# mandanasmi/lane-slam

Hardware: AMD Instinct MI355X
Metric: frames/sec (640x480) detect->descript->project->sanity->associate (higher is better)
Workload: dtype u8/f64 (FP4 e2m1 MFMA with exact f32 accumulation for association)

## Files before the change

### include/lanefront.h

```cpp
#ifndef LANEFRONT_H
#define LANEFRONT_H

#include <stddef.h>
#include <stdint.h>

#define LF_API __attribute__((visibility("default")))

#ifdef __cplusplus
extern "C" {
#endif

#define LF_ABI_VERSION 5

typedef enum lf_status {
    LF_OK = 0,
    LF_ERR_BAD_ARG = -1,
    LF_ERR_CAPACITY = -2,
    LF_ERR_HIP = -3,
    LF_ERR_NOT_INITIALISED = -4,
    LF_ERR_UNSUPPORTED = -5,
    LF_ERR_DECODE = -6
} lf_status;

#define LF_WHITE 0
// ... 427 lines not shown
LF_API int lf_deserialize_segments(lf_handle* h, const uint8_t* bodies, int bodies_on_device, const int64_t* frame_byte_offset,
                            int n_frames, lf_segments* out, int out_on_device, int* n_segments);

LF_API int lf_draw_lines(lf_handle* h, int n_frames, const lf_segments* seg, int seg_on_device, uint8_t* out_bgr, int out_on_device);
LF_API int lf_draw_lines_image(lf_handle* h, const uint8_t* bgr, int n_frames, int rows, int cols, const lf_segments* seg, int seg_on_device,
                               uint8_t* out_bgr, int images_on_device);

#define LF_JPEG_ENCODE_STAGES 8
LF_API size_t lf_jpeg_encode_bound(int rows, int cols);
LF_API int lf_jpeg_encode_batch(lf_handle* h, const uint8_t* bgr, int bgr_on_device, int n_frames, int rows, int cols, int quality, uint8_t* out,
                                size_t out_stride, uint32_t* out_size, int out_on_device);
LF_API int lf_jpeg_encode_timing(lf_handle* h, double* ms_per_stage, int n);
LF_API const char* lf_jpeg_encode_stage_name(int stage);

#define LF_RECTIFY_STAGES 1
LF_API int lf_set_camera(lf_handle* h, const double* K, const double* D, const double* R, const double* P, int cam_w, int cam_h);
LF_API int lf_set_rectified_input(lf_handle* h, int flag);
LF_API int lf_get_rectified_input(lf_handle* h, int* flag);
LF_API int lf_rectify_map(lf_handle* h, float* mapx, float* mapy);
LF_API int lf_rectify_batch(lf_handle* h, const uint8_t* src, int src_on_device, int n_frames, int rows, int cols, int channels, uint8_t* dst,
                            int dst_on_device);
LF_API int lf_rectify_timing(lf_handle* h, double* ms_per_stage, int n);
LF_API const char* lf_rectify_stage_name(int stage);

typedef enum lf_buffer_id {
    LF_BUF_BGR = 0,
    LF_BUF_MASKS = 1,
    LF_BUF_EDGES = 2,
    LF_BUF_LSD_ANGLE = 3,
    LF_BUF_LSD_MODGRAD = 4,
    LF_BUF_LSD_ORDER = 5,
    LF_BUF_LSD_NORDER = 6,
    LF_BUF_LBD_DX = 7,
    LF_BUF_LBD_DY = 8,
    LF_BUF_LSD_COUNTS = 9,
    LF_BUF_LSD_SCRATCH = 10,
    LF_BUF_LSD_NLOW = 11
} lf_buffer_id;
LF_API int lf_debug_fetch(lf_handle* h, int buffer_id, void* dst, size_t bytes);
LF_API int lf_debug_detmath(lf_handle* h, int which, const double* a, const double* b_or_null, double* y, int n);
enum { LF_WAVE_INT = 0, LF_WAVE_UINT = 1, LF_WAVE_FLOAT = 2, LF_WAVE_DOUBLE = 3, LF_WAVE_LONG = 4, LF_WAVE_ULONG = 5 };
enum {
    LF_WAVE_READLANE = 0, LF_WAVE_DPP = 1, LF_WAVE_SUM = 2, LF_WAVE_MAX = 3, LF_WAVE_MIN = 4, LF_WAVE_INCL_SCAN_DPP = 5,
    LF_WAVE_INCL_MIN_DPP = 6, LF_WAVE_SUM_BCAST = 7, LF_WAVE_MIN_BCAST = 8, LF_WAVE_INCL_SCAN = 9, LF_WAVE_REDUCE = 10,
    LF_WAVE_BALLOT = 11, LF_WAVE_LANE_MASK_LT = 12, LF_WAVE_LANES_BELOW = 13, LF_WAVE_BALLOT_BRANCH = 14, LF_WAVE_UNI = 15,
    LF_WAVE_WG_EXCL_SCAN = 16, LF_WAVE_WG_SCAN_TURNS = 17
};
LF_API int lf_debug_wave(lf_handle* h, int op, int type, int arg, int diverge, const uint64_t* in, uint64_t* out, int n_threads, int block);
LF_API int lf_debug_probe(lf_handle* h, int width, int write, size_t bytes, int reps);
LF_API int lf_debug_lsd_binary(lf_handle* h, const uint8_t* img, int rows, int cols, float* lines4, int cap, int* n_out);
LF_API int lf_debug_segments(lf_handle* h, int mode, int n_frames, const int32_t* counts, const float* lines4, const uint8_t* masks,
                             lf_segments* out, int* n_segments);
LF_API int lf_debug_std_sort(lf_handle* h, const int32_t* keys, int n, int32_t* order);
LF_API int lf_lsd_size(const lf_handle* h, int* rows, int* cols);
LF_API int lf_suggested_depth(const lf_handle* h);

LF_API int lf_lsd_list_capacity(const lf_handle* h, int* entries, int* grown);
LF_API int lf_lsd_scratch_stride(const lf_handle* h);

#define LF_N_STAGES 16
LF_API int lf_set_profiling(lf_handle* h, int enabled);
LF_API int lf_get_timing(lf_handle* h, double* ms_per_stage, int32_t* launches_per_stage, int n);
LF_API int lf_reset_timing(lf_handle* h);
LF_API const char* lf_stage_name(int stage);

#ifdef __cplusplus
}
#endif
#endif
```

### lane_slam_amd/_lib.py

```python
import ctypes
import os

from .config import LfConfig

_HERE = os.path.dirname(os.path.abspath(__file__))
SO_PATH = os.environ.get("LANEFRONT_LIBRARY") or os.path.join(_HERE, "liblanefront.so")

LF_N_STAGES = 16
LF_MAP_N_STAGES = 4
LF_MSG_DETECTOR, LF_MSG_GROUND, LF_MSG_FILTERED = 0, 1, 2
(LF_BUF_BGR, LF_BUF_MASKS, LF_BUF_EDGES, LF_BUF_LSD_ANGLE, LF_BUF_LSD_MODGRAD, LF_BUF_LSD_ORDER,
 LF_BUF_LSD_NORDER, LF_BUF_LBD_DX, LF_BUF_LBD_DY, LF_BUF_LSD_COUNTS, LF_BUF_LSD_SCRATCH, LF_BUF_LSD_NLOW) = range(12)

EXPORTS = (
    "lf_abi_version", "lf_create", "lf_destroy", "lf_last_error", "lf_synchronize", "lf_get_stream",
    "lf_set_image", "lf_detect_lines", "lf_process_batch", "lf_process_batch_async", "lf_wait", "lf_associate", "lf_associate_float", "lf_kmeans",
    "lf_jpeg_decode_batch", "lf_jpeg_info", "lf_frames_buffer", "lf_serialize_segments", "lf_deserialize_segments",
    "lf_debug_fetch", "lf_debug_detmath", "lf_debug_wave", "lf_debug_probe", "lf_debug_lsd_binary", "lf_debug_segments", "lf_lsd_size", "lf_set_profiling", "lf_get_timing", "lf_reset_timing", "lf_stage_name",
    "lf_map_create", "lf_map_destroy", "lf_map_last_error", "lf_map_get_stream", "lf_map_synchronize", "lf_map_seed", "lf_map_size",
    "lf_map_associate", "lf_map_pack_block", "lf_map_update", "lf_map_step", "lf_map_step_host", "lf_map_fetch",
    "lf_map_set_profiling", "lf_map_get_timing", "lf_map_stage_name",
    "lf_descriptor_default_params", "lf_set_descriptor_params", "lf_get_descriptor_params",
    "lf_edlines_default_params", "lf_keylines_batch", "lf_describe_keylines", "lf_keylines_debug_fetch", "lf_set_image_edlines", "lf_knn_match", "lf_radius_match", "lf_jpeg_decode_batch_gpu", "lf_jpeg_decode_batch_gpu_async", "lf_jpeg_status", "lf_jpeg_decode_for_detect_async",
    "lf_set_tie_rule", "lf_map_set_tie_rule", "lf_debug_std_sort", "lf_suggested_depth", "lf_lsd_list_capacity", "lf_lsd_scratch_stride", "lf_set_detector", "lf_detector_failures", "lf_keylines_batch_async", "lf_keylines_frame_status", "lf_lsd_keylines_batch", "lf_select_queries",
    "lf_lsd_default_options", "lf_lsd_keylines_batch_ex", "lf_keylines_batch_masked",
    "lf_matcher_add", "lf_matcher_clear", "lf_matcher_size", "lf_matcher_match", "lf_matcher_knn_match", "lf_matcher_radius_match",
    "lf_lane_filter_default_config", "lf_lane_filter_create", "lf_lane_filter_destroy", "lf_lane_filter_last_error", "lf_lane_filter_grid",
    "lf_lane_filter_set_tables", "lf_lane_filter_reset", "lf_lane_filter_step", "lf_lane_filter_get_poses", "lf_lane_filter_get_belief",
    "lf_lane_filter_synchronize", "lf_lane_filter_set_profiling", "lf_lane_filter_get_timing", "lf_lane_filter_stage_name",
    "lf_hough_default_params", "lf_set_hough_params", "lf_get_hough_params",
    "lf_dense_default_params", "lf_set_dense_params", "lf_get_dense_params",
    "lf_ai_transform_batch", "lf_set_ai_transform", "lf_get_ai_transform",
    "lf_draw_lines", "lf_draw_lines_image",
    "lf_jpeg_encode_bound", "lf_jpeg_encode_batch", "lf_jpeg_encode_timing", "lf_jpeg_encode_stage_name",
    "lf_set_camera", "lf_set_rectified_input", "lf_get_rectified_input", "lf_rectify_map", "lf_rectify_batch", "lf_rectify_timing",
    "lf_rectify_stage_name",
    "lf_map_default_view", "lf_map_bounds", "lf_map_render", "lf_map_render_counts", "lf_map_render_timing", "lf_map_render_stage_name",
    "lf_sizeof_camera_view", "lf_map_camera_view", "lf_map_render_camera", "lf_map_render_camera_timing",
    "lf_sizeof_align_config", "lf_sizeof_align_result", "lf_map_align_default_config", "lf_map_align", "lf_map_step_aligned",
    "lf_map_step_aligned_host", "lf_map_align_timing",
    "lf_sizeof_smooth_config", "lf_map_smooth_default_config", "lf_map_smooth", "lf_map_step_smoothed", "lf_map_step_smoothed_host",
    "lf_map_smooth_timing",
    "lf_sizeof_localize_config", "lf_sizeof_localize_result", "lf_map_localize_default_config", "lf_map_localize", "lf_map_localize_timing",
    "lf_sizeof_prune_config", "lf_sizeof_prune_result", "lf_map_prune_default_config", "lf_map_prune", "lf_map_prune_timing",
    "lf_sizeof_near_config", "lf_map_near_default_config", "lf_map_associate_near", "lf_map_set_near", "lf_map_get_near", "lf_map_near_timing",
)
LF_ALIGN_OK, LF_ALIGN_FEW, LF_ALIGN_DEGENERATE, LF_ALIGN_REJECTED = 0, 1, 2, 3
ALIGN_STATUS = ("ok", "few", "degenerate", "rejected")
LF_MAP_RENDER_STAGES = 4
LF_JPEG_ENCODE_STAGES = 8
LF_RECTIFY_STAGES = 1
LF_LANE_FILTER_PREDICT, LF_LANE_FILTER_UPDATE = 1, 2
LF_LANE_FILTER_MAX_CELLS = 4096
LF_LANE_FILTER_N_STAGES = 2
LANE_FILTER_PARAMS = ("mean_d_0", "mean_phi_0", "sigma_d_0", "sigma_phi_0", "delta_d", "delta_phi", "d_max", "d_min", "phi_max",
                      "phi_min", "cov_v", "linewidth_white", "linewidth_yellow", "lanewidth", "min_max", "sigma_d_mask", "sigma_phi_mask")
DETECTORS = {"lsd": 0, "edlines": 1, "hough": 2, "dense": 3}
HOUGH_KEYS = ("hough_threshold", "hough_min_line_length", "hough_max_line_gap")
DENSE_KEYS = ("sobel_threshold",)
TIE_RULES = {"lowest": 0, "mihasher": 1}
LF_MAX_OCTAVES = 5


class LfSegments(ctypes.Structure):
    _fields_ = [
        ("capacity", ctypes.c_int32),
        ("frame_offset", ctypes.c_void_p),
        ("lines", ctypes.c_void_p), ("normals", ctypes.c_void_p), ("color", ctypes.c_void_p),
        ("pixels_normalized", ctypes.c_void_p), ("ground", ctypes.c_void_p), ("keep", ctypes.c_void_p),
        ("desc", ctypes.c_void_p), ("code", ctypes.c_void_p),
    ]


class LfEdlinesParams(ctypes.Structure):
    _fields_ = [("gradient_threshold", ctypes.c_int32), ("anchor_threshold", ctypes.c_int32), ("scan_intervals", ctypes.c_int32),
                ("min_line_len", ctypes.c_int32), ("line_fit_err_threshold", ctypes.c_double), ("ksize", ctypes.c_int32)]

# ... 307 lines not shown
    lib.lf_keylines_batch_masked.argtypes = [vp, vp, ci, ci, ci, ci, ctypes.POINTER(LfEdlinesParams), vp, ci, ctypes.POINTER(LfKeylines), ci, ci,
                                             ctypes.POINTER(ci), vp]
    lib.lf_keylines_batch_masked.restype = ci
    lib.lf_describe_keylines.argtypes = [vp, vp, ci, vp, vp, vp, vp, vp, ci, vp, vp, ci]
    lib.lf_describe_keylines.restype = ci
    lib.lf_keylines_debug_fetch.argtypes = [vp, ci, ci, vp, ctypes.c_size_t, vp]
    lib.lf_keylines_debug_fetch.restype = ci
    lib.lf_set_image_edlines.argtypes = [vp, vp, ci, ci, ci, ctypes.POINTER(LfEdlinesParams)]
    lib.lf_set_image_edlines.restype = ci
    lib.lf_keylines_batch_async.argtypes = [vp, vp, ci, ci, ci, ctypes.POINTER(LfEdlinesParams), ctypes.POINTER(LfKeylines), ci]
    lib.lf_keylines_batch_async.restype = ci
    lib.lf_select_queries.argtypes = [vp, vp, ci, vp, vp, vp, ctypes.POINTER(ci), ci]
    lib.lf_select_queries.restype = ci
    lib.lf_matcher_add.argtypes = [vp, vp, ci, ci]
    lib.lf_matcher_clear.argtypes = [vp]
    lib.lf_matcher_size.argtypes = [vp, ctypes.POINTER(ci), ctypes.POINTER(ci)]
    lib.lf_matcher_match.argtypes = [vp, vp, ci, vp, vp, ctypes.POINTER(ci)]
    lib.lf_matcher_knn_match.argtypes = [vp, vp, ci, ci, vp, ci, vp, vp, ctypes.POINTER(ci)]
    lib.lf_matcher_radius_match.argtypes = [vp, vp, ci, ctypes.c_float, vp, ci, vp, vp, ci, ctypes.POINTER(ci), ctypes.POINTER(ci)]
    for fn in (lib.lf_matcher_add, lib.lf_matcher_clear, lib.lf_matcher_size, lib.lf_matcher_match, lib.lf_matcher_knn_match, lib.lf_matcher_radius_match):
        fn.restype = ci
    lib.lf_lsd_keylines_batch.argtypes = [vp, vp, ci, ci, ci, ci, ctypes.POINTER(LfKeylines), ci, ci, ctypes.POINTER(ci)]
    lib.lf_lsd_keylines_batch.restype = ci
    lib.lf_lsd_keylines_batch_ex.argtypes = [vp, vp, ci, ci, ci, ci, ctypes.POINTER(LfLsdOptions), vp, ci, ctypes.POINTER(LfKeylines), ci, ci, ctypes.POINTER(ci)]
    lib.lf_lsd_keylines_batch_ex.restype = ci
    lib.lf_lsd_default_options.argtypes = [ctypes.POINTER(LfLsdOptions)]
    lib.lf_lsd_default_options.restype = None
    lib.lf_keylines_frame_status.argtypes = [vp, vp, ci]
    lib.lf_keylines_frame_status.restype = ci
    lib.lf_set_detector.argtypes = [vp, ci, ctypes.POINTER(LfEdlinesParams)]
    lib.lf_set_detector.restype = ci
    lib.lf_detector_failures.argtypes = [vp]
    lib.lf_detector_failures.restype = ci
    lib.lf_hough_default_params.argtypes = [ctypes.POINTER(LfHoughParams)]
    lib.lf_hough_default_params.restype = None
    lib.lf_set_hough_params.argtypes = [vp, ctypes.POINTER(LfHoughParams)]
    lib.lf_set_hough_params.restype = ci
    lib.lf_get_hough_params.argtypes = [vp, ctypes.POINTER(LfHoughParams)]
    lib.lf_get_hough_params.restype = ci
    lib.lf_dense_default_params.argtypes = [ctypes.POINTER(LfDenseParams)]
    lib.lf_dense_default_params.restype = None
    lib.lf_set_dense_params.argtypes = [vp, ctypes.POINTER(LfDenseParams)]
    lib.lf_set_dense_params.restype = ci
    lib.lf_get_dense_params.argtypes = [vp, ctypes.POINTER(LfDenseParams)]
    lib.lf_get_dense_params.restype = ci
    lib.lf_suggested_depth.argtypes = [vp]
    lib.lf_lsd_list_capacity.argtypes = [vp, ctypes.POINTER(ci), ctypes.POINTER(ci)]
    lib.lf_lsd_list_capacity.restype = ci
    lib.lf_lsd_scratch_stride.argtypes = [vp]
    lib.lf_lsd_scratch_stride.restype = ci
    lib.lf_suggested_depth.restype = ci
    lib.lf_debug_std_sort.argtypes = [vp, vp, ci, vp]
    lib.lf_debug_std_sort.restype = ci
    lib.lf_set_tie_rule.argtypes = [vp, ci]
    lib.lf_set_tie_rule.restype = ci
    lib.lf_map_set_tie_rule.argtypes = [vp, ci]
    lib.lf_map_set_tie_rule.restype = ci
    lib.lf_knn_match.argtypes = [vp, vp, ci, vp, ci, ci, vp, vp, ci]
    lib.lf_knn_match.restype = ci
    lib.lf_radius_match.argtypes = [vp, vp, ci, vp, ci, ctypes.c_float, vp, vp, vp, ci, ctypes.POINTER(ci), ci]
    lib.lf_radius_match.restype = ci
    lib.lf_lane_filter_default_config.argtypes = [ctypes.POINTER(LfLaneFilterConfig)]
    lib.lf_lane_filter_default_config.restype = None
    lib.lf_lane_filter_create.argtypes = [ci, ctypes.POINTER(LfLaneFilterConfig), ci, ci, ctypes.POINTER(vp)]
    lib.lf_lane_filter_destroy.argtypes = [vp]
    lib.lf_lane_filter_destroy.restype = None
    lib.lf_lane_filter_last_error.argtypes = [vp]
    lib.lf_lane_filter_last_error.restype = ctypes.c_char_p
    lib.lf_lane_filter_grid.argtypes = [vp, ctypes.POINTER(ci), ctypes.POINTER(ci)]
    lib.lf_lane_filter_set_tables.argtypes = [vp, vp, vp, vp, vp]
    lib.lf_lane_filter_reset.argtypes = [vp, ci, vp]
    lib.lf_lane_filter_step.argtypes = [vp, vp, ctypes.POINTER(LfSegments), ci, ci, vp, vp, ci, vp, vp, vp]
    lib.lf_lane_filter_get_poses.argtypes = [vp, vp, ci]
    lib.lf_lane_filter_get_belief.argtypes = [vp, ci, vp]
    lib.lf_lane_filter_synchronize.argtypes = [vp]
    lib.lf_lane_filter_set_profiling.argtypes = [vp, ci]
    lib.lf_lane_filter_get_timing.argtypes = [vp, vp, vp, ci]
    lib.lf_lane_filter_stage_name.argtypes = [ci]
    lib.lf_lane_filter_stage_name.restype = ctypes.c_char_p
    for f in ("lf_lane_filter_create", "lf_lane_filter_grid", "lf_lane_filter_set_tables", "lf_lane_filter_reset", "lf_lane_filter_step",
              "lf_lane_filter_get_poses", "lf_lane_filter_get_belief", "lf_lane_filter_synchronize",
              "lf_lane_filter_set_profiling", "lf_lane_filter_get_timing"):
        getattr(lib, f).restype = ci
    for f in ("lf_map_create", "lf_map_get_stream", "lf_map_synchronize", "lf_map_seed", "lf_map_size", "lf_map_associate",
              "lf_map_pack_block", "lf_map_update", "lf_map_step", "lf_map_fetch"):
        getattr(lib, f).restype = ci
    for f in ("lf_synchronize", "lf_set_image", "lf_detect_lines", "lf_process_batch", "lf_process_batch_async", "lf_wait", "lf_associate",
              "lf_associate_float", "lf_kmeans", "lf_ai_transform_batch", "lf_set_ai_transform", "lf_get_ai_transform", "lf_draw_lines", "lf_draw_lines_image", "lf_jpeg_decode_batch", "lf_jpeg_info", "lf_frames_buffer", "lf_serialize_segments", "lf_deserialize_segments",
    "lf_debug_fetch", "lf_debug_detmath", "lf_debug_lsd_binary", "lf_debug_segments", "lf_lsd_size", "lf_set_profiling", "lf_get_timing",
              "lf_reset_timing"):
        getattr(lib, f).restype = ci
    _lib = lib
    return lib
```

### lane_slam_amd/csrc/common.h

```cpp
#pragma once
#include <hip/hip_runtime.h>
#include <stdint.h>
#include <stddef.h>
#include "../../include/lanefront.h"
#include "detmath.h"

namespace lf {

constexpr int kMaxKsize = 9;
constexpr int kMaxGaussTaps = 15;
constexpr float kNotDef = -1024.0f;
#ifndef LF_LABEL_ITEMS
#define LF_LABEL_ITEMS 8192
#endif
constexpr int kLabelItems = LF_LABEL_ITEMS;
#ifndef LF_LABEL_LDS
#define LF_LABEL_LDS 6144
#endif
constexpr int kLabelLds = LF_LABEL_LDS;
constexpr int kCompCap = 1024;

enum Stage {
    ST_PRE = 0, ST_CANNY, ST_HYST, ST_LSD_GRAD, ST_LSD_ORDER, ST_LSD_GROW, ST_SEGMENTS,
    ST_LBD_GRAD, ST_LBD, ST_ASSOC_PACK, ST_ASSOC, ST_MISC, ST_JPEG, ST_LSD_LABEL, ST_HOUGH, ST_DENSE, ST_COUNT
// ... 75 lines not shown
    int32_t lines_overflow;
    int32_t over_small, over_medium;
    int32_t max_defined;
    int32_t detector_failures;
    int32_t rec_need;
    int32_t reserved;
    int32_t total;
};
static_assert(sizeof(BatchStatus) == 32, "BatchStatus is eight words");

struct ResizeTables {
    const int* xofs;
    const float* xa;
    const int* y0;
    const int* y1;
    const float* yb;
    int xmax;
};

}

#ifdef __HIPCC__
__device__ __forceinline__ void lf_xcd_tile(int& bx, int& by, int& bz)
{
    const unsigned nx = gridDim.x, ny = gridDim.y, total = nx * ny * gridDim.z;
    unsigned b = blockIdx.x + nx * (blockIdx.y + ny * blockIdx.z);
    const unsigned group = 8u * nx;
    if (b < total / group * group) {
        const unsigned g = b / group, r = b - g * group;
        b = g * group + (r & 7u) * nx + (r >> 3);
    }
    bx = (int)(b % nx);
    const unsigned q = b / nx;
    by = (int)(q % ny);
    bz = (int)(q / ny);
}
#endif

extern "C" void lf_set_error(lf_handle* h, int code, const char* fmt, ...);

namespace lf {
void launch_pre_gray(const PreParams& p, const uint8_t* frames, int n_frames, uint8_t* gray, hipStream_t s);
void launch_pre(const PreParams& p, const uint8_t* frames, int n_frames, uint32_t* bgr, uint8_t* gray,
                uint32_t* maskbits, const int* sdiv, const int* hdiv, hipStream_t s, uint32_t* bwbits = nullptr);
void launch_canny(const CannyParams& p, const uint32_t* bgr, int n_frames, uint32_t* strong, uint32_t* weak,
                  hipStream_t s);
int launch_hysteresis(const CannyParams& p, int n_frames, uint32_t* strong, const uint32_t* weak, hipStream_t s);
void launch_bgrx_to_bgr(int n_pix, const uint32_t* bgrx, uint8_t* bgr, hipStream_t s);
void launch_edges_u8(const CannyParams& p, int n_frames, const uint32_t* bits, uint8_t* edges, hipStream_t s);
void launch_lsd_grad(const LsdParams& p, const ResizeTables& rt, const LsdRecords& r, int n_frames, const uint32_t* edge_bits,
                     const uint32_t* mask_bits, int* rec_need, bool counters_zeroed, hipStream_t s);
void launch_lsd_grad_gray(const LsdParams& p, const ResizeTables& rt, const LsdRecords& r, int n_frames, const uint8_t* gray, hipStream_t s);
bool lsd_seed32_supported(const LsdParams& p);
void launch_lsd_seed32(const LsdParams& p, const LsdRecords& r, const LsdCompact& c, int n_frames, int* rec_need, int big, hipStream_t s);
size_t std_sort_debug_words(int n);
void launch_std_sort_debug(const uint32_t* E, uint32_t* work, int n, int* count, hipStream_t s);
void launch_lsd_order(const LsdParams& p, const LsdRecords& r, const LsdCompact& c, int n_frames, hipStream_t s);
void launch_lsd_dense_debug(const LsdParams& p, const LsdCompact& c, int n_frames, float* ang, double* mod, hipStream_t s);
void launch_lsd_rank(const LsdComponents& m, int n_prob, hipStream_t s);
void launch_lsd_label(const LsdParams& p, const LsdCompact& c, const LsdComponents& m, int n_frames, hipStream_t s);
size_t lsd_grow_reg_stride(const LsdParams& p);
void launch_lsd_grow(const LsdParams& p, const LsdCompact& c, const LsdComponents& m, int n_frames, float* lines, int* counts,
                     int lds_kb, bool mixed, int bitmap, hipStream_t s);
int lsd_grow_def_lds(const LsdParams& p, int lds_kb);
constexpr int kGrowLdsKb[3] = { 13, 28, 40 };
void launch_seg_offsets(int n_frames, int cap_lines, const int* counts, int* seg_offset, int* frame_offset,
                        BatchStatus* status, const int* norder, int cap_small, int cap_medium, hipStream_t s);
void launch_dense(int Hc, int W, int Ww, int cap_lines, float thr, int n_problems, const uint32_t* strong, const uint32_t* maskbits,
                  const uint32_t* bwbits, float* slot_lines, float* rec, int* counts, hipStream_t s);
enum SegMode { SEG_FLOAT = 0, SEG_HOUGH = 1, SEG_DENSE = 2 };
void launch_segments(const SegParams& p, int n_frames, const float* slot_lines, const int* counts,
                     const int* seg_offset, const uint32_t* side, int Ww, lf_segments out, int* seg_frame,
                     double* normals64, float* centers, hipStream_t s, SegMode mode = SEG_FLOAT);
void launch_lbd_grad(int Hc, int W, int n_frames, const uint8_t* gray, uint32_t* dxy, hipStream_t s);
struct LbdPlanes { const uint32_t* base[LF_MAX_OCTAVES]; int W[LF_MAX_OCTAVES], H[LF_MAX_OCTAVES]; };
void launch_lbd_keylines(const LbdPlanes& planes, int n_cap, int n_frames, const int* n_lines, const float* in_octave4, const float* angle, const int* npx,
                         const int* octave, const int* frame, const float* gauss_g, const float* gauss_l, float* desc, uint8_t* code,
                         hipStream_t s, int wband = 7);
void launch_lbd_split_debug(size_t n, const uint32_t* dxy, int16_t* dx, int16_t* dy, hipStream_t s);
void launch_lbd(int Hc, int W, int n_seg_cap, const int* n_seg, const float* lines, const int* seg_frame,
                const uint32_t* dxy, const float* gauss_g, const float* gauss_l,
                float* desc, uint8_t* code, hipStream_t s, int wband = 7);
int lbd_max_width_of_band();
size_t assoc_rows_padded_m(int nm);
__host__ __device__ inline size_t assoc_map_offset_fp4(size_t row, int byte)
{
    return (row >> 6) * 8192 + (size_t)(byte >> 4) * 1024 + (row & 63) * 16 + (size_t)(byte & 15);
}
__host__ __device__ inline uint32_t assoc_fp4_expand(uint32_t byte)
{
    uint32_t t = (byte | (byte << 12)) & 0x000f000fu;
    t = (t | (t << 6)) & 0x03030303u;
    t = (t | (t << 3)) & 0x11111111u;
    return (t << 3) | 0x22222222u;
}
#ifdef __HIPCC__
__device__ __forceinline__ void assoc_map_write_row(int8_t* mx, int8_t* mcx, size_t pos, int b, uint32_t byte, const uint8_t* colour_byte)
{
    *reinterpret_cast<uint32_t*>(mx + assoc_map_offset_fp4(pos, 4 * b)) = assoc_fp4_expand(byte);
    if (b < 8) {
        const int colour = *colour_byte;
        uint32_t w = 0;
        if (b == 0 && colour < 3)
            for (int g = 0; g < 3; ++g) if (g != colour) w |= 0xFu << (4 * g);
        *reinterpret_cast<uint32_t*>(mcx + pos * 32 + 4 * b) = w;
    }
}
__device__ __forceinline__ void assoc_map_zero_row(int8_t* mx, int8_t* mcx, size_t pos, int b)
{
    *reinterpret_cast<uint32_t*>(mx + assoc_map_offset_fp4(pos, 4 * b)) = 0u;
    if (b < 8) *reinterpret_cast<uint32_t*>(mcx + pos * 32 + 4 * b) = 0u;
}
#endif
// ... 110 lines not shown
```

### lane_slam_amd/csrc/k_lsd_order.hip

```cpp
#include <cstdlib>
#include <algorithm>
#include "common.h"
#include <type_traits>
#include "lsd_bitplane.h"
#include "scan.h"
#include "wave.h"

namespace lf {
using std::max;
using std::min;

#ifndef LF_ORDER_THREADS
#define LF_ORDER_THREADS 512
#endif
#ifndef LF_ORDER_BM_THREADS
#define LF_ORDER_BM_THREADS 256
#endif
#ifndef LF_LABEL_THREADS
#define LF_LABEL_THREADS 256
#endif
constexpr int OT = LF_ORDER_THREADS;
constexpr int OBT = LF_ORDER_BM_THREADS;
constexpr int NB = 16;
constexpr int LDS_ITEMS = 8192;

template <typename T, int NB = 16, int NT = OT>
__device__ __forceinline__ void radix_pass(const T* __restrict__ src, T* __restrict__ dst, int n, int shift,
                           uint32_t* cnt , int* tot , int* base )
{
    static_assert(NB % (NT / 64) == 0, "every wave scans NB / waves bucket rows");
    const int t = threadIdx.x, lane = t & 63, wave = t >> 6;
    const int seg = (n + NT - 1) / NT;
    const int i0 = min(n, t * seg), i1 = min(n, i0 + seg);
    for (int b = 0; b < NB; ++b) cnt[b * NT + t] = 0;
    for (int i = i0; i < i1; ++i) cnt[(int)((src[i] >> shift) & (NB - 1)) * NT + t]++;
    __syncthreads();
    for (int bb = 0; bb < NB / (NT / 64); ++bb) {
        const int b = wave * (NB / (NT / 64)) + bb;
        int carry = 0;
        for (int c = 0; c < NT / 64; ++c) {
            int v = (int)cnt[b * NT + c * 64 + lane];
            int inc = wave_incl_scan(v, lane);
            cnt[b * NT + c * 64 + lane] = (uint32_t)(carry + inc - v);
            carry += __shfl(inc, 63);
        }
        if (lane == 0) tot[b] = carry;
    }
    __syncthreads();
    if (wave == 0) {
        int v = lane < NB ? tot[lane] : 0;
        int inc = wave_incl_scan(v, lane);
        if (lane < NB) base[lane] = inc - v;
    }
    __syncthreads();
    for (int i = i0; i < i1; ++i) {
        const T it = src[i];
        int b = (int)((it >> shift) & (NB - 1));
        uint32_t pos = (uint32_t)base[b] + cnt[b * NT + t]++;
        dst[pos] = it;
    }
    __syncthreads();
}

template <typename Dst>
__device__ __forceinline__ void stable_pass5(const uint32_t* src, Dst* dst, int n, int shift,
                                             uint32_t* wrun , uint32_t* wbase )
{
    constexpr int W = OT / 64, MAXSTEP = LDS_ITEMS / OT;
    const int t = threadIdx.x, lane = t & 63, w = t >> 6;
    const int C = ((n + W - 1) / W + 63) & ~63;
    const int start = w * C, end = min(n, start + C);
    if (lane < 32) wrun[w * 32 + lane] = 0;
// ... 273 lines not shown
                if (place) A[run + (uint32_t)__popcll(mask & lt)] = it;
                if ((mask >> lane) >> 1 == 0ull) mine[d] = (uint16_t)(run + (uint32_t)__popcll(mask));
            }
            __builtin_amdgcn_fence(__ATOMIC_ACQ_REL, "wavefront");
            __builtin_amdgcn_wave_barrier();
        }
    };
    walk(false);
    __syncthreads();
    for (int d = t; d < OB_BINS; d += OBT) {
        uint32_t s_ = 0;
        for (int k = 0; k < OBT / 64; ++k) s_ += wcnt[k * OB_BINS + d];
        bin_base[d] = s_;
    }
    __syncthreads();
    if (w == 0) {
        uint32_t carry = 0;
        for (int d0 = 0; d0 < OB_BINS; d0 += 64) {
            const uint32_t v = bin_base[d0 + lane];
            const uint32_t inc = (uint32_t)wave_incl_scan((int)v, lane);
            bin_base[d0 + lane] = carry + inc - v;
            carry += (uint32_t)__shfl((int)inc, 63);
        }
    }
    __syncthreads();
    for (int d = t; d < OB_BINS; d += OBT) {
        uint32_t run = bin_base[d];
        for (int k = 0; k < OBT / 64; ++k) { const uint32_t c_ = wcnt[k * OB_BINS + d]; wcnt[k * OB_BINS + d] = (uint16_t)run; run += c_; }
    }
    __syncthreads();
    walk(true);
}

void launch_lsd_order(const LsdParams& p, const LsdRecords& r, const LsdCompact& c, int n_frames, hipStream_t s)
{
    static const bool old_form = getenv("LF_ORDER_SORT") != nullptr;
    static const int force_hbm = getenv("LF_ORDER_HBM") ? 1 : 0;
    const size_t Ps = (size_t)p.Hs * p.Ws;
    size_t blds = bitplane_lds_words(Ps) * 4;
    if (blds < (size_t)(OBT / 64) * OB_BINS * 2) blds = (size_t)(OBT / 64) * OB_BINS * 2;
    if (blds < (size_t)8 * OBT * 4) blds = (size_t)8 * OBT * 4;
    if (!old_form && p.n_bins <= OB_BINS && blds <= 40 * 1024 && Ps < ((size_t)1 << 20)) {
        hipLaunchKernelGGL(k_lsd_order_bm, dim3(n_frames * 3), dim3(OBT), blds, s, p, r.r_addr, r.r_deg, r.r_mod, r.r_cs, r.r_sn, r.n_rec,
                           r.maxgrad, c.sort_a, c.sort_b, c.order_a, c.order_b, c.norder, c.c_xy, c.c_deg, c.c_mod, c.c_cs, c.c_sn, c.row_start, force_hbm);
        return;
    }
    const size_t lds = ((size_t)2 * LDS_ITEMS + 2 * (size_t)(p.Hs + 2) + 2 * (OT / 64) * 32) * sizeof(uint32_t);
    if (lds > 48 * 1024)
        (void)hipFuncSetAttribute(reinterpret_cast<const void*>(k_lsd_order), hipFuncAttributeMaxDynamicSharedMemorySize, (int)lds);
    hipLaunchKernelGGL(k_lsd_order, dim3(n_frames * 3), dim3(OT), lds, s, p, r.r_addr, r.r_deg, r.r_mod, r.r_cs, r.r_sn, r.n_rec, r.maxgrad,
                       c.sort_a, c.sort_b, c.order_a, c.order_b, c.norder, c.c_xy, c.c_deg, c.c_mod, c.c_cs, c.c_sn, c.row_start);
}

struct UfLds {
    volatile lds_u32* P;
    __device__ __forceinline__ uint32_t get(uint32_t i) const { return P[i]; }
    __device__ __forceinline__ void set(uint32_t i, uint32_t v) const { P[i] = v; }
    __device__ __forceinline__ void add(uint32_t i, uint32_t v) const { (void)__hip_atomic_fetch_add((lds_u32*)&P[i], v, __ATOMIC_RELAXED, __HIP_MEMORY_SCOPE_WORKGROUP); }
};
struct UfLds16 {
    volatile lds_u16* P;
    __device__ __forceinline__ uint32_t get(uint32_t i) const { return P[i]; }
    __device__ __forceinline__ void set(uint32_t i, uint32_t v) const { P[i] = (uint16_t)v; }
    __device__ __forceinline__ uint32_t min(uint32_t i, uint32_t v) const
    {
        lds_u32* w = (lds_u32*)P + (i >> 1);
        const uint32_t sh = (i & 1u) * 16u;
        uint32_t cur = *(volatile lds_u32*)w;
        for (;;) {
            const uint32_t old = (cur >> sh) & 0xffffu;
            if (v >= old) return old;
            uint32_t expect = cur;
            if (__hip_atomic_compare_exchange_strong(w, &expect, (cur & ~(0xffffu << sh)) | (v << sh), __ATOMIC_RELAXED, __ATOMIC_RELAXED, __HIP_MEMORY_SCOPE_WORKGROUP)) return old;
            cur = expect;
        }
    }
};
struct UfGlb {
    uint32_t* P;
    __device__ __forceinline__ uint32_t get(uint32_t i) const { return __hip_atomic_load(P + i, __ATOMIC_RELAXED, __HIP_MEMORY_SCOPE_AGENT); }
    __device__ __forceinline__ void set(uint32_t i, uint32_t v) const { __hip_atomic_store(P + i, v, __ATOMIC_RELAXED, __HIP_MEMORY_SCOPE_AGENT); }
    __device__ __forceinline__ uint32_t min(uint32_t i, uint32_t v) const { return __hip_atomic_fetch_min(P + i, v, __ATOMIC_RELAXED, __HIP_MEMORY_SCOPE_AGENT); }
    __device__ __forceinline__ void add(uint32_t i, uint32_t v) const { (void)__hip_atomic_fetch_add(P + i, v, __ATOMIC_RELAXED, __HIP_MEMORY_SCOPE_AGENT); }
};
template <class UF>
__device__ __forceinline__ uint32_t uf_find(const UF& P, uint32_t x)
{
    uint32_t p = P.get(x);
    while (p != x) {
        const uint32_t g = P.get(p);
        if (g != p) (void)P.min(x, g);
        x = p;
        p = g;
    }
    return x;
}

template <class UF>
__device__ __forceinline__ void uf_unite(const UF& P, uint32_t a, uint32_t b)
{
    for (;;) {
        a = uf_find(P, a);
        b = uf_find(P, b);
        if (a == b) return;
        if (a < b) { const uint32_t t = a; a = b; b = t; }
        const uint32_t old = P.min(a, b);
        if (old == a) return;
        a = old;
    }
}

constexpr int LT = LF_LABEL_THREADS;
#ifndef LF_COMP_TOP
#define LF_COMP_TOP 8
#endif
constexpr int kCompTop = LF_COMP_TOP;

template <bool GLB>
__device__ __forceinline__ void lsd_label_problem(const LsdParams& p, const int* __restrict__ norder, const uint32_t* __restrict__ c_xy,
                                                  const int* __restrict__ row_start, uint16_t* __restrict__ c_label,
                                                  uint16_t* __restrict__ comp_list, int* __restrict__ comp_count, int* __restrict__ comp_key, int comp_cap,
                                                  uint32_t* __restrict__ scratch, size_t scratch_stride)
{
    extern __shared__ __attribute__((aligned(16))) uint32_t dyn_lds[];
    const int LS = p.label_lds;
    __shared__ uint16_t roots[kCompCap];
    __shared__ int n_roots, rest_total;
    const int pc = blockIdx.x, t = threadIdx.x;
    const size_t Ps = (size_t)p.Hs * p.Ws, o = (size_t)pc * p.rec_cap;
    const int n = norder[pc];
    uint16_t* lab = c_label + o;
    uint16_t* list = comp_list + (size_t)pc * kCompCap;
    if (n == 0) { if (t == 0) { comp_count[pc] = 0; comp_key[pc] = 0; } return; }
    if (n > p.label_items) {
        for (int e = t; e < n; e += LT) lab[e] = 0;
        if (t == 0) { list[0] = 0; comp_count[pc] = 1; comp_key[pc] = n; }
        return;
    }
    const uint16_t* xs_lds = reinterpret_cast<const uint16_t*>(dyn_lds + LS / 2);
    uint32_t* gtab = scratch + (size_t)pc * scratch_stride;
    typename std::conditional<GLB, UfGlb, UfLds16>::type parent;
    typename std::conditional<GLB, UfGlb, UfLds>::type csize2;
    if constexpr (GLB) { parent.P = gtab; csize2.P = gtab + ((n + 1) & ~1); }
    else { parent.P = (volatile lds_u16*)dyn_lds; csize2.P = (volatile lds_u32*)(dyn_lds + LS / 2); }
    auto xs = [&](int k) -> int { if constexpr (GLB) return (int)(c_xy[o + k] & 0xffffu); else return (int)xs_lds[k]; };
    const int* rs = row_start + (size_t)pc * (p.Hs + 1);
    if (t == 0) { n_roots = 0; rest_total = 0; }
    if constexpr (GLB) {
        __shared__ int wave_tot[LT / 64];
        bitplane_build<LT>(dyn_lds, c_xy + o, n, p.Ws, Ps, wave_tot);
        __syncthreads();
        const unsigned long long* bits64 = reinterpret_cast<const unsigned long long*>(dyn_lds);
        const uint16_t* pref = reinterpret_cast<const uint16_t*>(dyn_lds + 2 * bitplane_words(Ps));
        auto bit = [&](int pos) -> bool { return (bits64[pos >> 6] >> (pos & 63)) & 1ull; };
        auto rank = [&](int pos) -> uint32_t {
            const int w = pos >> 6;
            const unsigned long long lo = bits64[w & ~1], cur = bits64[w];
            return (uint32_t)pref[w >> 1] + ((w & 1) ? (uint32_t)__builtin_popcountll(lo) : 0u) + (uint32_t)__builtin_popcountll(cur & ((1ull << (pos & 63)) - 1ull));
        };
        for (int e = t; e < n; e += LT) {
            const uint32_t xy = c_xy[o + e];
            const int x = (int)(xy & 0xffffu), y = (int)(xy >> 16), pos = y * p.Ws + x;
            int back = 0;
            while (back < x && bit(pos - back - 1)) ++back;
            parent.set((uint32_t)e, (uint32_t)(e - back));
        }
        __syncthreads();
        for (int e = t; e < n; e += LT) {
            const uint32_t xy = c_xy[o + e];
            const int x = (int)(xy & 0xffffu), y = (int)(xy >> 16);
            if (y == 0) continue;
            const int up = (y - 1) * p.Ws + x;
            const bool head = x == 0 || !bit(up + p.Ws - 1);
            const bool uL = x > 0 && bit(up - 1), uC = bit(up), uR = x + 1 < p.Ws && bit(up + 1);
            if (head) {
                if (uL) uf_unite(parent, (uint32_t)e, rank(up - 1));
                else if (uC) uf_unite(parent, (uint32_t)e, rank(up));
                if (uR && !uC) uf_unite(parent, (uint32_t)e, rank(up + 1));
            } else if (uR && !uC) uf_unite(parent, (uint32_t)e, rank(up + 1));
        }
        __syncthreads();
    } else {
        for (int e = t; e < n; e += LT) reinterpret_cast<uint16_t*>(dyn_lds + LS / 2)[e] = (uint16_t)(c_xy[o + e] & 0xffffu);
        __syncthreads();
    for (int e = t; e < n; e += LT) {
        const int y = (int)(c_xy[o + e] >> 16);
        const int first = rs[y];
        int h = e;
        int xh = xs(h);
        while (h > first) { const int xp = xs(h - 1); if (xp + 1 != xh) break; --h; xh = xp; }
        parent.set((uint32_t)e, (uint32_t)h);
    }
    __syncthreads();
    for (int e = t; e < n; e += LT) {
        const uint32_t xy = c_xy[o + e];
        const int x = (int)(xy & 0xffffu), y = (int)(xy >> 16);
        if (y > 0) {
            int lo = rs[y - 1];
            const int end = rs[y];
            int hi = end;
            while (lo < hi) { const int mid = (lo + hi) >> 1; if (xs(mid) < x - 1) lo = mid + 1; else hi = mid; }
            for (int k = lo; k < end && k < lo + 3 && xs(k) <= x + 1; ++k) uf_unite(parent, (uint32_t)e, (uint32_t)k);
        }
    }
    __syncthreads();
    }
    for (int i = t; i < (n + 1) / 2; i += LT) csize2.set((uint32_t)i, 0u);
    __syncthreads();
    for (int e = t; e < n; e += LT) {
        const uint32_t r = uf_find(parent, (uint32_t)e);
        lab[e] = (uint16_t)r;
        csize2.add(r >> 1, 1u << (16 * (r & 1u)));
    }
    __syncthreads();
    auto csize = [&](uint32_t r) -> uint32_t { return (csize2.get(r >> 1) >> (16 * (r & 1u))) & 0xffffu; };
    const uint32_t minsz = p.min_reg_size > 1 ? (uint32_t)p.min_reg_size : 1u;
    for (int e = t; e < n; e += LT)
        if (csize((uint32_t)e) >= minsz) {
            const int k = atomicAdd(&n_roots, 1);
            if (k < comp_cap) roots[k] = (uint16_t)e;
        }
    __syncthreads();
    const int C = n_roots;
    if (C > comp_cap) {
        for (int e = t; e < n; e += LT) lab[e] = 0;
        if (t == 0) { list[0] = 0; comp_count[pc] = 1; comp_key[pc] = n; }
        return;
    }
    for (int i = t; i < C; i += LT) {
        const uint32_t ri = roots[i], si = csize(ri);
        int rank = 0;
        for (int j = 0; j < C; ++j) {
            const uint32_t rj = roots[j], sj = csize(rj);
            rank += (sj > si || (sj == si && rj < ri)) ? 1 : 0;
        }
        list[rank] = (uint16_t)ri;
        parent.set(ri, (uint32_t)rank);
        if (rank == 0) comp_key[pc] = (int)si;
        if (rank >= kCompTop) atomicAdd(&rest_total, (int)si);
    }
    __syncthreads();
    if (C <= kCompTop) {
        if (t == 0) { comp_count[pc] = C; if (C == 0) comp_key[pc] = 0; }
        return;
    }
    __threadfence_block();
    const uint16_t rest_root = list[kCompTop];
    for (int e = t; e < n; e += LT) {
        const uint32_t r = lab[e];
        if (csize(r) >= minsz && parent.get(r) >= (uint32_t)kCompTop) lab[e] = rest_root;
    }
    if (t == 0) {
        const int rest = rest_total;
        const int top0 = (int)csize((uint32_t)list[0]);
        if (rest > top0) {
            for (int k = kCompTop; k > 0; --k) list[k] = list[k - 1];
            list[0] = rest_root;
            comp_key[pc] = rest;
        }
        comp_count[pc] = kCompTop + 1;
    }
}

__global__ __launch_bounds__(256) void k_lsd_rank(int n_prob, const int* __restrict__ norder, int* __restrict__ perm)
{
    __shared__ int nd[1024];
    if (n_prob > 1024) {
        for (int i = threadIdx.x; i < n_prob; i += 256) perm[i] = i;
        return;
    }
    for (int i = threadIdx.x; i < n_prob; i += 256) nd[i] = norder[i];
    __syncthreads();
    for (int i = threadIdx.x; i < n_prob; i += 256) {
        const int mine = nd[i];
        int rank = 0;
        for (int j = 0; j < n_prob; ++j) rank += (nd[j] > mine || (nd[j] == mine && j < i)) ? 1 : 0;
        perm[rank] = i;
    }
}

void launch_lsd_rank(const LsdComponents& m, int n_prob, hipStream_t s)
{
    hipLaunchKernelGGL(k_lsd_rank, dim3(1), dim3(256), 0, s, n_prob, m.comp_key, m.perm);
}

__global__ __launch_bounds__(LT) void k_lsd_label(LsdParams p, const int* __restrict__ norder, const uint32_t* __restrict__ c_xy,
                                                  const int* __restrict__ row_start, uint16_t* __restrict__ c_label,
                                                  uint16_t* __restrict__ comp_list, int* __restrict__ comp_count, int* __restrict__ comp_key, int comp_cap,
                                                  uint32_t* __restrict__ scratch, size_t scratch_stride, int plane_fits)
{
    const int n = norder[blockIdx.x];
    if (n <= p.label_lds)
        lsd_label_problem<false>(p, norder, c_xy, row_start, c_label, comp_list, comp_count, comp_key, comp_cap, scratch, scratch_stride);
    else if (plane_fits)
        lsd_label_problem<true>(p, norder, c_xy, row_start, c_label, comp_list, comp_count, comp_key, comp_cap, scratch, scratch_stride);
    else {
        const size_t o = (size_t)blockIdx.x * p.rec_cap;
        for (int e = threadIdx.x; e < n; e += LT) c_label[o + e] = 0;
        if (threadIdx.x == 0) { comp_list[(size_t)blockIdx.x * kCompCap] = 0; comp_count[blockIdx.x] = 1; comp_key[blockIdx.x] = n; }
    }
}

void launch_lsd_label(const LsdParams& p, const LsdCompact& c, const LsdComponents& m, int n_frames, hipStream_t s)
{
    size_t lds = (size_t)p.label_lds * (2 + 2);
    const size_t plane = bitplane_lds_words((size_t)p.Hs * p.Ws) * 4;
    const int plane_fits = plane <= 150 * 1024 ? 1 : 0;
    if (plane_fits && plane > lds) lds = plane;
    if (lds > 48 * 1024)
        (void)hipFuncSetAttribute(reinterpret_cast<const void*>(k_lsd_label), hipFuncAttributeMaxDynamicSharedMemorySize, (int)lds);
    static const int comp_cap = getenv("LF_DIAG_COMP_CAP") ? max(1, min(kCompCap, atoi(getenv("LF_DIAG_COMP_CAP")))) : kCompCap;
    const size_t stride = lsd_grow_reg_stride(p);
    hipLaunchKernelGGL(k_lsd_label, dim3(n_frames * 3), dim3(LT), lds, s, p, c.norder, c.c_xy, c.row_start, m.c_label, m.comp_list, m.comp_count,
                       m.comp_key, comp_cap, m.reg, stride, plane_fits);
}

__global__ void k_lsd_dense_debug(LsdParams p, const int* __restrict__ norder, const uint32_t* __restrict__ c_xy,
                                  const float* __restrict__ c_deg, const double* __restrict__ c_mod,
                                  float* __restrict__ ang, double* __restrict__ mod)
{
    const int pc = blockIdx.x;
    const size_t Ps = (size_t)p.Hs * p.Ws, o = (size_t)pc * Ps, oc = (size_t)pc * p.rec_cap;
    for (size_t i = threadIdx.x; i < Ps; i += blockDim.x) { ang[o + i] = kNotDef; mod[o + i] = 0.0; }
    __syncthreads();
    const int n = norder[pc];
    for (int e = threadIdx.x; e < n; e += blockDim.x) {
        const uint32_t xy = c_xy[oc + e];
        const size_t a = (size_t)(xy >> 16) * p.Ws + (xy & 0xffffu);
        ang[o + a] = c_deg[oc + e];
        mod[o + a] = c_mod[oc + e];
    }
}

void launch_lsd_dense_debug(const LsdParams& p, const LsdCompact& c, int n_frames, float* ang, double* mod, hipStream_t s)
{
    hipLaunchKernelGGL(k_lsd_dense_debug, dim3(n_frames * 3), dim3(1024), 0, s, p, c.norder, c.c_xy, c.c_deg, c.c_mod, ang, mod);
}

}
```

### lane_slam_amd/csrc/k_lsd_seed32.hip

```cpp
#include <cstdlib>
#include <cstring>
#include "common.h"
#include "lsd_bitplane.h"
#include "scan.h"

namespace lf {

#ifdef LF_SEED_STAMPS
#define SEED_T(v) const long long v = (long long)wall_clock64()
#else
#define SEED_T(v) do { } while (0)
#define FST(k) do { } while (0)
#define FST0 do { } while (0)
#endif

#ifndef LF_SEED_THREADS
#define LF_SEED_THREADS 256
#endif
#ifndef LF_SEED_WAVES2
#define LF_SEED_WAVES2 4
#endif
#ifndef LF_SEED_BLOCK
#define LF_SEED_BLOCK 4096
#endif
#ifndef LF_SEED_EPT
#define LF_SEED_EPT 32
#endif
#ifndef LF_SEED_OCC
#define LF_SEED_OCC 3
#endif
constexpr int ST = LF_SEED_THREADS;
constexpr int SW = ST / 64;
constexpr int DT = 256;
constexpr int kDenseOcc = 4;
constexpr int kBlock = LF_SEED_BLOCK;
constexpr int SW2 = LF_SEED_WAVES2;
constexpr int kSmall = 1024;
constexpr int kWaveWords = kSmall + kSmall / 2 + 2 * 18 * 2 + 18 + 20 + 8 + 128;
constexpr int kBlkWaveWords = kSmall / 2 + 2 * 18 * 2 + 18 + 20 + 8 + 128;
constexpr int kBlkX = SW2 * kBlkWaveWords > kBlock / 2 ? SW2 * kBlkWaveWords : kBlock / 2;
constexpr int kBlkRows = kBlock / 64 + 2;
constexpr int kBlkWords = kBlock + kBlkX + (kBlkRows * 6 + 8) + 2 * (kBlock / 16);

constexpr int kSortThreshold = 16;
constexpr int kMaxLdsBytes = 150 * 1024;
constexpr int SNB = 16;
constexpr int kU = 8;
constexpr int kEPT = LF_SEED_EPT;
constexpr int kListLds = kEPT * ST;
constexpr int kChainDense = 1024;
constexpr int kMaxRanges = 48;
constexpr int kRowsLds = 512;

__device__ __forceinline__ uint32_t key_of(uint32_t v) { return v >> 20; }
__device__ __forceinline__ bool comp(uint32_t a, uint32_t b) { return key_of(a) > key_of(b); }

__device__ __forceinline__ void lds_add(lds_i32* p, int v) { (void)__hip_atomic_fetch_add(p, v, __ATOMIC_RELAXED, __HIP_MEMORY_SCOPE_WORKGROUP); }
__device__ __forceinline__ void lds_min(lds_i32* p, int v) { (void)__hip_atomic_fetch_min(p, v, __ATOMIC_RELAXED, __HIP_MEMORY_SCOPE_WORKGROUP); }
__device__ __forceinline__ void lds_or(lds_i32* p, int v) { (void)__hip_atomic_fetch_or(p, v, __ATOMIC_RELAXED, __HIP_MEMORY_SCOPE_WORKGROUP); }
__device__ __forceinline__ void tab_add(lds_i32* p, int v) { lds_add(p, v); }
__device__ __forceinline__ void tab_min(lds_i32* p, int v) { lds_min(p, v); }


__device__ __forceinline__ void median_to_first(uint32_t* E, int f, int l)
{
    const int ia = f + 1, ib = f + (l - f) / 2, ic = l - 1;
    const uint32_t a = E[ia], b = E[ib], c = E[ic];
// ... 92 lines not shown
        }
        if (lane == 0) SX[R] = 0;
    }
    team_sync<COOP>();
    int wK = 0, wFirstL = 0x7fffffff, wFirstStay = 0x7fffffff;
    for (int r = w; r < R; r += nw) {
        const int i = lo + r * 64 + lane;
        const unsigned long long bl = BL[r], br = BR[r];
        const bool isL = (bl >> lane) & 1ull, isR = (br >> lane) & 1ull;
        const int kl = PL[r] + __popcll(bl & le), r_right = SX[r + 1] + __popcll(br & ~le);
        const int kr = SX[r + 1] + __popcll(br >> lane), l_left = PL[r] + __popcll(bl & lt);
        const bool swl = isL && r_right >= kl, swr = isR && l_left >= kr;
        if (swl) Lpos[kl - 1] = i - org;
        if (swr) Rpos[kr - 1] = i - org;
        const unsigned long long bs = __ballot(swl);
        const unsigned long long un = bl & ~bs;
        wK += __popcll(bs);
        if (bl) wFirstL = min(wFirstL, lo + r * 64 + __ffsll((long long)bl) - 1);
        if (un) wFirstStay = min(wFirstStay, lo + r * 64 + __ffsll((long long)un) - 1);
    }
    if (lane == 0) {
        if (wK) lds_add(&acc[0], wK);
        if (wFirstL != 0x7fffffff) lds_min(&acc[1], wFirstL);
        if (wFirstStay != 0x7fffffff) lds_min(&acc[2], wFirstStay);
    }
    team_sync<COOP>();
    const int K = acc[0];
    for (int k0 = tid; k0 < K; k0 += nthreads * kU) {
        int pi[kU], pj[kU];
        uint32_t a[kU], b[kU];
#pragma unroll
        for (int u = 0; u < kU; ++u) {
            const int k = k0 + u * nthreads;
            pi[u] = k < K ? org + (int)Lpos[k] : -1;
            pj[u] = k < K ? org + (int)Rpos[k] : -1;
        }
#pragma unroll
        for (int u = 0; u < kU; ++u) if (pi[u] >= 0) { a[u] = E[pi[u]]; b[u] = E[pj[u]]; }
#pragma unroll
        for (int u = 0; u < kU; ++u) if (pi[u] >= 0) { E[pi[u]] = b[u]; E[pj[u]] = a[u]; }
    }
    const int cut = K == 0 ? acc[1] : min(acc[2], org + (int)Rpos[K - 1]);
    team_sync<COOP>();
    return cut;
}

template <int NT, typename T64, typename T32>
__device__ __forceinline__ int partition_global(uint32_t* E, int f, int l, T64 BL, T64 BR, T32 PL, T32 SX,
                                                lds_i32* acc, uint32_t* Lpos, uint32_t* Rpos, int w, int lane)
{
    const int lo = f + 1, hi = l;
    const int R = (hi - lo + 63) >> 6;
    const uint32_t pivot = E[f];
    if (threadIdx.x == 0) { acc[0] = 0; acc[1] = 0x7fffffff; acc[2] = 0x7fffffff; acc[3] = (pivot & 0xfffffu) != 0u; }
    __syncthreads();
    for (int r0 = w * kU; r0 < R; r0 += (NT / 64) * kU) {
        uint32_t v[kU];
#pragma unroll
        for (int u = 0; u < kU; ++u) { const int i = lo + (r0 + u) * 64 + lane; v[u] = i < hi ? E[i] : 0xffffffffu; }
        int seeds = 0;
#pragma unroll
        for (int u = 0; u < kU; ++u) {
            const int r = r0 + u;
            if (r < R) {
                const bool valid = lo + r * 64 + lane < hi;
                const unsigned long long bl = __ballot(valid && !comp(v[u], pivot));
                const unsigned long long br = __ballot(valid && !comp(pivot, v[u]));
                seeds += __popcll(__ballot(valid && (v[u] & 0xfffffu) != 0u));
                if (lane == 0) { BL[r] = bl; BR[r] = br; PL[r] = __popcll(bl); SX[r] = __popcll(br); }
            }
        }
        if (lane == 0 && seeds) lds_add(&acc[3], seeds);
    }
    __syncthreads();
    if (acc[3] == 0) { __syncthreads(); return -1; }
    return partition_tail<true>(E, 0, lo, hi, BL, BR, PL, SX, acc, Lpos, Rpos, w, NT / 64, lane, (int)threadIdx.x, NT);
}

#ifdef LF_SEED_STAMPS
__device__ int g_dbg_big[8], g_dbg_small[8], g_dbg_chain[8][4];
__device__ long long g_dbg_b[8][6];
__device__ long long g_dbg_w[8][8];
__device__ long long g_dbg_f[8][12];
#define FST(k) do { const long long n_ = (long long)wall_clock64(); if (threadIdx.x == 0) g_dbg_f[blockIdx.x % 8][k] += n_ - fs_; fs_ = n_; } while (0)
#define FST0 long long fs_ = (long long)wall_clock64()
__device__ long long g_dbg_t[8][4];
#endif

struct SeedRange { int off, len, depth; };

__device__ __forceinline__ int partition_lds(lds_u32* D, int f, int l, lds_u64* BL, lds_u64* BR, lds_i32* PL, lds_i32* SX,
                                             lds_i32* acc, lds_u16* Lpos, lds_u16* Rpos, int lane)
{
    const int lo = f + 1, hi = l;
    const int R = (hi - lo + 63) >> 6;
    const uint32_t pivot = D[f];
    if (lane == 0) { acc[0] = 0; acc[1] = 0x7fffffff; acc[2] = 0x7fffffff; }
    int seeds = (pivot & 0xfffffu) != 0u;
    for (int r = 0; r < R; ++r) {
        const int i = lo + r * 64 + lane;
        const bool valid = i < hi;
        const uint32_t v = valid ? D[i] : 0u;
        const unsigned long long bl = __ballot(valid && !comp(v, pivot));
        const unsigned long long br = __ballot(valid && !comp(pivot, v));
        seeds += __popcll(__ballot(valid && (v & 0xfffffu) != 0u));
        if (lane == 0) { BL[r] = bl; BR[r] = br; PL[r] = __popcll(bl); SX[r] = __popcll(br); }
    }
    team_sync<false>();
    if (seeds == 0) return -1;
    return partition_tail<false>(D, 0, lo, hi, BL, BR, PL, SX, acc, Lpos, Rpos, 0, 1, lane, lane, 64);
}

__device__ __forceinline__ void median_to_first_lds(lds_u32* E, int f, int l)
{
    const int ia = f + 1, ib = f + (l - f) / 2, ic = l - 1;
    const uint32_t a = E[ia], b = E[ib], c = E[ic];
    int pick;
    if (comp(a, b)) pick = comp(b, c) ? ib : (comp(a, c) ? ic : ia);
    else pick = comp(a, c) ? ia : (comp(b, c) ? ic : ib);
    const uint32_t r = E[f], p = E[pick];
    E[f] = p;
    E[pick] = r;
}

__device__ __forceinline__ int partition_lds_coop(lds_u32* D, int f, int l, lds_u64* BL, lds_u64* BR, lds_i32* PL, lds_i32* SX,
                                                  lds_i32* acc, lds_u16* Lpos, lds_u16* Rpos, int w, int lane)
{
    const int lo = f + 1, hi = l;
    const int R = (hi - lo + 63) >> 6;
    const uint32_t pivot = D[f];
    if (threadIdx.x == 0) { acc[0] = 0; acc[1] = 0x7fffffff; acc[2] = 0x7fffffff; acc[3] = (pivot & 0xfffffu) != 0u; }
    __syncthreads();
    int seeds = 0;
    for (int r = w; r < R; r += SW2) {
        const int i = lo + r * 64 + lane;
        const bool valid = i < hi;
        const uint32_t v = valid ? D[i] : 0u;
        const unsigned long long bl = __ballot(valid && !comp(v, pivot));
        const unsigned long long br = __ballot(valid && !comp(pivot, v));
        seeds += __popcll(__ballot(valid && (v & 0xfffffu) != 0u));
        if (lane == 0) { BL[r] = bl; BR[r] = br; PL[r] = __popcll(bl); SX[r] = __popcll(br); }
    }
    if (lane == 0 && seeds) lds_add(&acc[3], seeds);
    __syncthreads();
    if (acc[3] == 0) { __syncthreads(); return -1; }
    return partition_tail<true>(D, 0, lo, hi, BL, BR, PL, SX, acc, Lpos, Rpos, w, SW2, lane, (int)threadIdx.x, 64 * SW2);
}


__device__ __forceinline__ void wave_window(lds_u32* D, uint32_t* D_generic, int w0, int n, int depth, lds_u32* xch, int lane)
{
    const bool in = lane < n;
    uint32_t v = in ? D[w0 + lane] : 0u;
    int f = 0, l = n, d = depth;
    bool done = false;
    const unsigned long long le = lane == 63 ? ~0ull : ((2ull << lane) - 1ull);
    const unsigned long long lt = lane_mask_lt(lane);
    for (;;) {
        const unsigned long long segm = (l >= 64 ? ~0ull : ((1ull << l) - 1ull)) & ~((1ull << f) - 1ull);
        const unsigned long long sb = __ballot(in && (v & 0xfffffu) != 0u);
        const bool active = in && !done && (l - f) > kSortThreshold && (sb & segm) != 0ull;
        if (__ballot(active) == 0ull) break;
        if (__ballot(active && d == 0) != 0ull) {
            if (in) D[w0 + lane] = v;
            team_sync<false>();
            if (active && d == 0 && lane == f) heap_sort_range(D_generic, w0 + f, w0 + l);
            team_sync<false>();
            if (in) v = D[w0 + lane];
            if (active && d == 0) done = true;
            continue;
        }
        const int ia = f + 1, ib = f + ((l - f) >> 1), ic = l - 1;
        const uint32_t va = __shfl(v, ia), vb = __shfl(v, ib), vc = __shfl(v, ic), vf = __shfl(v, f);
        int pick;
        if (comp(va, vb)) pick = comp(vb, vc) ? ib : (comp(va, vc) ? ic : ia);
        else pick = comp(va, vc) ? ia : (comp(vb, vc) ? ic : ib);
        const uint32_t pv = pick == ia ? va : (pick == ib ? vb : vc);
        if (active) { if (lane == f) v = pv; else if (lane == pick) v = vf; }
        const bool part = active && lane > f;
        const uint32_t kp = key_of(pv), kv = key_of(v);
        const bool isL = part && kv <= kp, isR = part && kv >= kp;
        const unsigned long long bl = __ballot(isL) & segm, br = __ballot(isR) & segm;
        const int kl = __popcll(bl & le), r_right = __popcll(br & ~le);
        const int kr = __popcll(br >> lane), l_left = __popcll(bl & lt);
        const bool swl = isL && r_right >= kl, swr = isR && l_left >= kr;
        if (swl) xch[f + kl] = v;
        if (swr) xch[64 + f + kr] = v;
        team_sync<false>();
        if (swl) v = xch[64 + f + kl];
        if (swr) v = xch[f + kr];
        team_sync<false>();
        const unsigned long long bs = __ballot(swl) & segm, bsr = __ballot(swr) & segm;
        const int K = __popcll(bs);
        const unsigned long long un = bl & ~bs;
        const int firstL = bl ? __ffsll((long long)bl) - 1 : 64, firstStay = un ? __ffsll((long long)un) - 1 : 64;
        const int RK = bsr ? __ffsll((long long)bsr) - 1 : 64;
        const int cut = K == 0 ? firstL : min(firstStay, RK);
        if (active) { if (lane < cut) l = cut; else f = cut; --d; }
    }
// ... 27 lines not shown
            const int r = r0 + u;
            const bool valid = lo + r * 64 + lane < hi;
            const unsigned long long bl = __ballot(valid && key_of(v[u]) <= kp);
            const unsigned long long br = __ballot(valid && key_of(v[u]) >= kp);
            seeds |= __ballot(valid && (v[u] & 0xfffffu) != 0u);
            if (lane == r) { myBL = bl; myBR = br; }
        }
    }
    if (seeds == 0ull) return -1;
    const int cl = __popcll(myBL), cr = __popcll(myBR);
    const int myPL = wave_incl_scan_dpp(cl) - cl;
    const int incr = wave_incl_scan_dpp(cr);
    const int mySX = readlane(incr, 63) - incr;
    int K = 0, firstL = 0x7fffffff, firstStay = 0x7fffffff, RK = 0x7fffffff;
    for (int r = 0; r < R; ++r) {
        const unsigned long long bl = readlane(myBL, r), br = readlane(myBR, r);
        const int pl = readlane(myPL, r), sx = readlane(mySX, r);
        const int i = lo + r * 64 + lane;
        const bool isL = (bl >> lane) & 1ull, isR = (br >> lane) & 1ull;
        const int kl = pl + __popcll(bl & le), r_right = sx + __popcll(br & ~le);
        const int kr = sx + __popcll(br >> lane), l_left = pl + __popcll(bl & lt);
        const bool swl = isL && r_right >= kl, swr = isR && l_left >= kr;
        if (swl) Lpos[kl - 1] = (uint16_t)i;
        if (swr) Rpos[kr - 1] = (uint16_t)i;
        const unsigned long long bs = __ballot(swl), bsr = __ballot(swr);
        const unsigned long long un = bl & ~bs;
        K += __popcll(bs);
        if (firstL == 0x7fffffff && bl) firstL = lo + r * 64 + __ffsll((long long)bl) - 1;
        if (firstStay == 0x7fffffff && un) firstStay = lo + r * 64 + __ffsll((long long)un) - 1;
        if (RK == 0x7fffffff && bsr) RK = lo + r * 64 + __ffsll((long long)bsr) - 1;
    }
    team_sync<false>();
    for (int k0 = lane; k0 < K; k0 += 64 * 4) {
        int pi[4], pj[4];
        uint32_t a[4], b[4];
#pragma unroll
        for (int u = 0; u < 4; ++u) { const int k = k0 + u * 64; pi[u] = k < K ? (int)Lpos[k] : -1; pj[u] = k < K ? (int)Rpos[k] : -1; }
#pragma unroll
        for (int u = 0; u < 4; ++u) if (pi[u] >= 0) { a[u] = D[pi[u]]; b[u] = D[pj[u]]; }
#pragma unroll
        for (int u = 0; u < 4; ++u) if (pi[u] >= 0) { D[pi[u]] = b[u]; D[pj[u]] = a[u]; }
    }
    team_sync<false>();
    return K == 0 ? firstL : min(firstStay, RK);
}

__device__ __forceinline__ void wave_subtree(lds_u32* D, uint32_t* D_generic, int f, int l, int depth, lds_u64* wBL, lds_u64* wBR,
                                             lds_i32* wPL, lds_i32* wSX, lds_i32* wacc, lds_u16* Lp, lds_u16* Rp, lds_i32* stack, int lane)
{
    int sp = 0;
    for (;;) {
        while (l - f > kSortThreshold) {
#ifdef LF_SEED_STAMPS
            if (l - f <= 64) { const long long c0 = clock64(); wave_window(D, D_generic, f, l - f, depth, (lds_u32*)Lp, lane); if (lane == 0 && (threadIdx.x >> 6) == 0) { g_dbg_w[blockIdx.x % 8][0] += 1; g_dbg_w[blockIdx.x % 8][1] += clock64() - c0; } break; }
#else
            if (l - f <= 64) { wave_window(D, D_generic, f, l - f, depth, (lds_u32*)Lp, lane); break; }
#endif
            if (depth == 0) {
                if (lane == 0) heap_sort_range(D_generic, f, l);
                team_sync<false>();
                break;
            }
            --depth;
#ifdef LF_SEED_STAMPS
            const long long c0 = clock64();
#endif
            const int cut = wave_partition(D, f, l, Lp, Rp, lane);
#ifdef LF_SEED_STAMPS
            if (lane == 0 && (threadIdx.x >> 6) == 0) { g_dbg_w[blockIdx.x % 8][2] += 1; g_dbg_w[blockIdx.x % 8][3] += clock64() - c0; g_dbg_w[blockIdx.x % 8][4] += (l - f + 62) >> 6; }
#endif
            if (cut < 0) break;
            if (l - cut > kSortThreshold) {
                if (lane == 0) { stack[2 * sp] = cut; stack[2 * sp + 1] = l | (depth << 24); }
                ++sp;
            }
            l = cut;
        }
        if (sp == 0) break;
        --sp;
        team_sync<false>();
        f = stack[2 * sp];
        l = stack[2 * sp + 1] & 0xffffff;
        depth = stack[2 * sp + 1] >> 24;
    }
    team_sync<false>();
}



template <int NT>
__device__ __forceinline__ void introsort_loop_waves(uint32_t* E, int n, const SeedRange* ranges, int n_ranges, unsigned long long* scratch,
                                                  uint32_t* lds, int rows_cap, uint32_t* gtab)
{
    lds_u64* BL = as_lds<lds_u64>(lds);
    lds_u64* BR = BL + rows_cap;
    lds_i32* PL = (lds_i32*)(BR + rows_cap);
    lds_i32* SX = PL + rows_cap;
    unsigned long long* small_list = scratch;
    unsigned long long* block_list = scratch + (n / 16 + 64);
    uint32_t* Lpos = reinterpret_cast<uint32_t*>(block_list + (n / kSmall + 64));
    uint32_t* Rpos = Lpos + (n / 2 + 8);
    __shared__ int acc_[4];
    lds_i32* acc = as_lds<lds_i32>(acc_);
    __shared__ int big_stack[3 * (72 + kMaxRanges)];
    __shared__ int n_big, n_small, n_block, next_small, n_blk_small;
    __shared__ int cur[4];
    const int t = threadIdx.x, lane = t & 63, w = t >> 6;
    auto pack = [](int f, int l, int depth) { return (unsigned long long)f | ((unsigned long long)l << 24) | ((unsigned long long)depth << 48); };
    if (t == 0) {
        n_big = 0; n_small = 0; n_block = 0; next_small = 0;
        for (int i = 0; i < n_ranges; ++i) {
            const int f = ranges[i].off, l = f + ranges[i].len, d = ranges[i].depth, sz = ranges[i].len;
            if (sz > kBlock) { big_stack[3 * n_big] = f; big_stack[3 * n_big + 1] = l; big_stack[3 * n_big + 2] = d; ++n_big; }
            else if (sz > kSmall) block_list[n_block++] = pack(f, l, d);
            else if (sz > kSortThreshold) small_list[n_small++] = pack(f, l, d);
        }
    }
    __syncthreads();
    SEED_T(ta);
    for (;;) {
        if (t == 0) {
            if (n_big > 0) { --n_big; cur[0] = big_stack[3 * n_big]; cur[1] = big_stack[3 * n_big + 1]; cur[2] = big_stack[3 * n_big + 2]; cur[3] = 1; }
            else cur[3] = 0;
        }
        __syncthreads();
        if (!cur[3]) break;
        int f = cur[0], l = cur[1], depth = cur[2];
        __syncthreads();
        while (l - f > kBlock) {
            if (depth == 0) {
                if (t == 0) heap_sort_range(E, f, l);
                __syncthreads();
                l = f;
                break;
            }
            --depth;
            if (t == 0) median_to_first(E, f, l);
            __syncthreads();
            int cut;
            if (((l - f - 1 + 63) >> 6) <= rows_cap - 1) cut = partition_global<NT>(E, f, l, BL, BR, PL, SX, acc, Lpos, Rpos, w, lane);
            else {
                const int rc = ((l - f) >> 6) + 2;
                unsigned long long* gBL = reinterpret_cast<unsigned long long*>(gtab);
                unsigned long long* gBR = gBL + rc;
                int* gPL = reinterpret_cast<int*>(gBR + rc);
                int* gSX = gPL + rc;
                cut = partition_global<NT>(E, f, l, gBL, gBR, gPL, gSX, acc, Lpos, Rpos, w, lane);
            }
#ifdef LF_SEED_STAMPS
            if (t == 0) atomicAdd(&g_dbg_big[blockIdx.x % 8], 1);
#endif
            if (cut < 0) { l = f; break; }
            if (t == 0) {
                const int rs = l - cut;
                if (rs > kBlock) { big_stack[3 * n_big] = cut; big_stack[3 * n_big + 1] = l; big_stack[3 * n_big + 2] = depth; ++n_big; }
                else if (rs > kSmall) block_list[n_block++] = pack(cut, l, depth);
                else if (rs > kSortThreshold) small_list[n_small++] = pack(cut, l, depth);
            }
            l = cut;
            __syncthreads();
// ... 150 lines not shown
#ifdef LF_SEED_STAMPS
    { const long long td = (long long)wall_clock64(); if (t == 0) { g_dbg_t[blockIdx.x % 8][0] = tb - ta; g_dbg_t[blockIdx.x % 8][1] = tc - tb; g_dbg_t[blockIdx.x % 8][2] = td - tc; } }
#endif
}


struct SeedWork {
    uint32_t* E;
    uint32_t* V0; uint32_t* V1;
    uint32_t* P0; uint32_t* P1;
    uint32_t* PP;
    uint32_t* T;
    uint32_t* RT;
    unsigned long long* dscratch;
    uint32_t* out;
    int cap;
};

struct ChainState {
    int f, l, depth, a, b, seeds, cur, e_used, n_ranges, stop;
    int md_idx[4];
    uint32_t md_val[4];
    int K, eK, cut, nP, nG, minR, lseeds, nright, wtot[SW];
    SeedRange ranges[kMaxRanges];
};

template <typename PT>
__device__ __forceinline__ int list_lower_bound(PT P, int a, int b, int q)
{
    while (a < b) {
        const int mid = (a + b) >> 1;
        if ((int)P[mid] < q) a = mid + 1; else b = mid;
    }
    return a;
}

template <typename CT>
__device__ __forceinline__ int wave_scan_rows(CT cnt, int R, int lane)
{
    int carry = 0;
    for (int r0 = 0; r0 < R; r0 += 64) {
        const int r = r0 + lane;
        const int c = r < R ? (int)cnt[r] : 0;
        const int inc = wave_incl_scan_dpp(c);
        if (r < R) cnt[r] = carry + inc - c;
        carry += readlane(inc, 63);
    }
    return carry;
}

template <typename PT>
__device__ __forceinline__ void chain_materialize(uint32_t* E, int off, int f, int l, PT P, const uint32_t* V, int a, int b)
{
    const int t = threadIdx.x;
    for (int i = t; i < l - f; i += ST) E[off + i] = 0u;
    __syncthreads();
    for (int i = a + t; i < b; i += ST) { const uint32_t v = V[i]; if (v) E[off + (int)P[i] - f] = v; }
    __syncthreads();
}

struct Plane { lds_u64* bits; lds_u16* pref; lds_u16* stab; int pairs; };
__host__ __device__ inline int plane_words_for(int len) { const int words = ((len >> 6) + 2) & ~1, pairs = words >> 1; return 2 * words + ((pairs + 1) >> 1) + ((pairs + 3) >> 1); }
__device__ __forceinline__ Plane plane_at(lds_u32* base, int len)
{
    Plane pl;
    const int words = ((len >> 6) + 2) & ~1;
    pl.bits = (lds_u64*)base;
    pl.pairs = words >> 1;
    pl.pref = (lds_u16*)(base + 2 * words);
    pl.stab = (lds_u16*)(base + 2 * words + ((pl.pairs + 1) >> 1));
    return pl;
}
__device__ __forceinline__ int plane_rank(const Plane& pl, int q)
{
    const int w = q >> 6;
    const unsigned long long lo = pl.bits[w & ~1], cur = pl.bits[w];
    return (int)pl.pref[w >> 1] + ((w & 1) ? __popcll(lo) : 0) + __popcll(cur & ((1ull << (q & 63)) - 1ull));
}
__device__ __forceinline__ int word_select(unsigned long long wd, int kk)
{
    int p = 0;
#pragma unroll
    for (int s = 32; s >= 1; s >>= 1) {
        if (__popcll(wd & ((1ull << (p + s)) - 1ull)) < kk) p += s;
    }
    return p;
}
template <int N>
__device__ __forceinline__ void plane_select0_n(const Plane& pl, const int (&k)[N], int (&out)[N])
{
    int x[N];
#pragma unroll
    for (int u = 0; u < N; ++u) x[u] = (int)pl.stab[(k[u] - 1) >> 7];
    for (;;) {
        int nx[N];
        bool any = false;
#pragma unroll
        for (int u = 0; u < N; ++u) { const int c = x[u] + 1; nx[u] = c < pl.pairs ? 128 * c - (int)pl.pref[c] : 0x7fffffff; }
#pragma unroll
        for (int u = 0; u < N; ++u) if (nx[u] < k[u]) { ++x[u]; any = true; }
        if (!any) break;
    }
    unsigned long long w0[N], w1[N];
    int p0[N];
#pragma unroll
    for (int u = 0; u < N; ++u) { w0[u] = pl.bits[2 * x[u]]; w1[u] = pl.bits[2 * x[u] + 1]; p0[u] = (int)pl.pref[x[u]]; }
#pragma unroll
    for (int u = 0; u < N; ++u) {
        int kk = k[u] - (128 * x[u] - p0[u]);
        unsigned long long wd = ~w0[u];
        int base = 128 * x[u];
        const int z0 = __popcll(wd);
        if (kk > z0) { kk -= z0; wd = ~w1[u]; base += 64; }
        out[u] = base + word_select(wd, kk);
    }
}
__device__ __forceinline__ int plane_select0(const Plane& pl, int k)
{
    const int kk[1] = { k };
    int out[1];
    plane_select0_n<1>(pl, kk, out);
    return out[0];
}

__device__ __forceinline__ int plane_counts(const Plane& pl, lds_i32* wave_tot)
{
    const int tid = (int)threadIdx.x, lane = tid & 63, wave = tid >> 6;
    const int per = (pl.pairs + ST - 1) / ST;
    const int w0 = tid * per < pl.pairs ? tid * per : pl.pairs, w1 = w0 + per < pl.pairs ? w0 + per : pl.pairs;
    int mine = 0;
    for (int q = w0; q < w1; ++q) mine += __popcll(pl.bits[2 * q]) + __popcll(pl.bits[2 * q + 1]);
    const int incl = wave_incl_scan_dpp(mine);
    if (lane == 63) wave_tot[wave] = incl;
    __syncthreads();
    int basev = incl - mine, total = 0;
    for (int k = 0; k < SW; ++k) { const int v = wave_tot[k]; if (k < wave) basev += v; total += v; }
    for (int q = w0; q < w1; ++q) {
        const int c = __popcll(pl.bits[2 * q]) + __popcll(pl.bits[2 * q + 1]);
        pl.pref[q] = (uint16_t)basev;
        const int zb0 = 128 * q - basev, zb1 = zb0 + 128 - c;
        for (int j = (zb0 + 127) >> 7; 128 * j < zb1; ++j) pl.stab[j] = (uint16_t)q;
        basev += c;
    }
    __syncthreads();
    return total;
}
__device__ __forceinline__ void plane_set(lds_u32* base, int q) { (void)__hip_atomic_fetch_or(base + (q >> 5), 1u << (q & 31), __ATOMIC_RELAXED, __HIP_MEMORY_SCOPE_WORKGROUP); }


constexpr uint32_t kDeadSlot = 0xffffffffu;
#ifndef LF_SEED_SEL
#define LF_SEED_SEL 4
#endif
constexpr int kSel = LF_SEED_SEL;
__device__ __forceinline__ void chain_step_plane(const SeedWork& W, lds_of<ChainState>* cs, lds_u32* lds,
                                                 uint32_t (&pr)[kEPT], bool& regs_ok)
{
    const int t = threadIdx.x, lane = t & 63;
    const int f = cs->f, l = cs->l, a = cs->a, b = cs->b, depth = cs->depth, cur = cs->cur, seeds = cs->seeds;
    const int len = l - f;
    uint32_t* V = (cur ? W.V1 : W.V0);
    uint32_t* P = (cur ? W.P1 : W.P0);
    uint32_t* V2 = (cur ? W.V0 : W.V1);
    uint32_t* P2 = (cur ? W.P0 : W.P1);
    lds_i32* wtot = (lds_i32*)&cs->wtot[0];
    const bool persist = b - a <= kEPT * ST;
    auto load_tile = [&](int base) {
        uint32_t vv[kEPT];
#pragma unroll
        for (int u = 0; u < kEPT; ++u) { const int i = base + t + u * ST, ic = i < b ? i : b - 1; vv[u] = V[ic]; pr[u] = P[ic]; }
#pragma unroll
        for (int u = 0; u < kEPT; ++u) if (vv[u] == 0u || base + t + u * ST >= b) pr[u] = kDeadSlot;
    };
    FST0;
    const Plane pl = plane_at(lds, len);
    for (int i = t; i < 4 * pl.pairs; i += ST) lds[i] = 0u;
    if (t < 4) { cs->md_idx[t] = -1; cs->md_val[t] = 0u; }
    __syncthreads();
    const int q0 = f, q1 = f + 1, q2 = f + len / 2, q3 = l - 1;
    for (int base = a; base < b; base += kEPT * ST) {
        if (!(persist && regs_ok)) load_tile(base);
#pragma unroll
        for (int u = 0; u < kEPT; ++u) {
            const uint32_t pos = pr[u];
            if (pos != kDeadSlot) {
                plane_set(lds, (int)pos - f);
                if ((int)pos == q0 || (int)pos == q1 || (int)pos == q2 || (int)pos == q3) {
                    const int i = base + t + u * ST;
                    const int which = (int)pos == q0 ? 0 : ((int)pos == q1 ? 1 : ((int)pos == q2 ? 2 : 3));
                    cs->md_idx[which] = i; cs->md_val[which] = V[i];
                }
            }
        }
    }
    if (persist) regs_ok = true;
    __syncthreads();
    FST(0);
    const int total = plane_counts(pl, wtot);
    FST(1);
    const uint32_t vf = cs->md_val[0], va = cs->md_val[1], vb = cs->md_val[2], vc = cs->md_val[3];
    const int xf = cs->md_idx[0];
    int pk;
    if (comp(va, vb)) pk = comp(vb, vc) ? 2 : (comp(va, vc) ? 3 : 1);
    else pk = comp(va, vc) ? 1 : (comp(vb, vc) ? 3 : 2);
    const uint32_t pv = cs->md_val[pk];
    const int xp = cs->md_idx[pk];
    const int pick = pk == 1 ? q1 : (pk == 2 ? q2 : q3);
    __syncthreads();
    if (t == 0) {
        if (xp >= 0) { V[xp] = vf; if (xf >= 0) V[xf] = 0u; }
        else if (xf >= 0) P[xf] = (uint32_t)pick;
// ... 194 lines not shown
        }
        int wemit = 0;
#pragma unroll
        for (int u = 0; u < kST; ++u) {
            const uint32_t v = vv[u];
            const int pos = (int)pp[u];
            bool emit = false, left = false;
            if (v) {
                if (gr[u] <= K) { left = true; emit = tv[u] != 0u; }
                else if ((lmask >> u) & 1u) { }
                else if (pos < cut) { W.E[off + pos - f] = v; left = true; }
                else { emit = true; tv[u] = v; }
            }
            wseeds += __popcll(__ballot(left && (v & 0xfffffu) != 0u));
            wemit += __popcll(__ballot(emit));
            if (emit) emask |= 1u << u;
        }
        if (wemit) {
            int base_ = 0;
            if (lane == 0) base_ = __hip_atomic_fetch_add((lds_i32*)&cs->nright, wemit, __ATOMIC_RELAXED, __HIP_MEMORY_SCOPE_WORKGROUP);
            base_ = a + __builtin_amdgcn_readfirstlane(base_);
#pragma unroll
            for (int u = 0; u < kST; ++u) {
                const bool emit = (emask >> u) & 1u;
                const unsigned long long be = __ballot(emit);
                if (emit) { const int dst = base_ + lanes_below(be, lane); P2[dst] = pp[u]; V2[dst] = tv[u]; }
                base_ += __popcll(be);
            }
        }
    }
    regs_ok = false;
    if (lane == 0 && wseeds) lds_add((lds_i32*)&cs->lseeds, wseeds);
    if (t == 0) W.E[off] = pv;
    __syncthreads();
    FST(10);
    if (t == 0) {
        const int k = cs->n_ranges;
        cs->ranges[k].off = off; cs->ranges[k].len = cut - f; cs->ranges[k].depth = depth - 1;
        cs->n_ranges = k + 1;
        cs->e_used = off + (cut - f);
        cs->seeds = seeds - cs->lseeds;
        cs->f = cut; cs->depth = depth - 1; cs->b = a + cs->nright; cs->cur = cur ^ 1;
    }
    __syncthreads();
#ifdef LF_SEED_STAMPS
    if (t == 0) atomicAdd(&g_dbg_chain[blockIdx.x % 8][1], 1);
#endif
}

template <bool PL>
__device__ __forceinline__ void sparse_chain(const SeedWork& W, lds_u32* Pl, lds_u32* tab, ChainState* cs_generic, int n, int m0, int nseeds, lds_u32* plane_lds, int plane_lds_words)
{
    lds_of<ChainState>* cs = as_lds<lds_of<ChainState>>(cs_generic);
    const int t = threadIdx.x, lane = t & 63, w = t >> 6;
    if (t == 0) {
        cs->f = 0; cs->l = n; cs->depth = 2 * (31 - __clz(n)); cs->a = 0; cs->b = m0; cs->seeds = nseeds; cs->cur = 0; cs->e_used = 0; cs->n_ranges = 0; cs->stop = 0;
    }
    uint32_t pr[kEPT];
    bool regs_ok = false;
    __syncthreads();
    for (;;) {
        const int f = cs->f, l = cs->l, a = cs->a, b = cs->b, depth = cs->depth, cur = cs->cur, seeds = cs->seeds;
        const int len = l - f, m = b - a;
        uint32_t* V = (cur ? W.V1 : W.V0);
        uint32_t* V2 = (cur ? W.V0 : W.V1);
        uint32_t* Pg = (cur ? W.P1 : W.P0);
        uint32_t* Pg2 = (cur ? W.P0 : W.P1);
        __syncthreads();
        if (seeds == 0) break;
        if (len <= kChainDense || (len - m) * 4 <= len || depth == 0 || cs->n_ranges >= kMaxRanges - 1) {
            const int off = cs->e_used;
            if (off + len > W.cap) {
                if (t == 0) cs->stop = off + len;
                __syncthreads();
                break;
            }
            if (PL) chain_materialize(W.E, off, f, l, Pl, V, a, b); else chain_materialize(W.E, off, f, l, Pg, V, a, b);
            if (t == 0) { const int k = cs->n_ranges; cs->ranges[k].off = off; cs->ranges[k].len = len; cs->ranges[k].depth = depth; cs->n_ranges = k + 1; cs->e_used = off + len; }
            __syncthreads();
            break;
        }
        if (!PL && 2 * ((plane_words_for(len) + 1) & ~1) <= plane_lds_words && m <= 65535) {
#ifdef LF_SEED_STAMPS
            const long long c0 = (long long)wall_clock64(); const int nr0 = cs->n_ranges;
#endif
            chain_step_plane(W, cs, plane_lds, pr, regs_ok);
#ifdef LF_SEED_STAMPS
            if (t == 0) { const int sp = cs->n_ranges != nr0; g_dbg_chain[blockIdx.x % 8][2 + sp] += (int)((long long)wall_clock64() - c0); }
#endif
            continue;
        }
        if (t < 4) {
            const int q = t == 0 ? f : (t == 1 ? f + 1 : (t == 2 ? f + len / 2 : l - 1));
            const int i = PL ? list_lower_bound(Pl, a, b, q) : list_lower_bound(Pg, a, b, q);
            const bool hit = i < b && (int)(PL ? Pl[i] : Pg[i]) == q;
            cs->md_idx[t] = hit ? i : -1;
            cs->md_val[t] = hit ? V[i] : 0u;
        }
        __syncthreads();
        const uint32_t vf = cs->md_val[0], va = cs->md_val[1], vb = cs->md_val[2], vc = cs->md_val[3];
        const int xf = cs->md_idx[0];
        int pk;
        if (comp(va, vb)) pk = comp(vb, vc) ? 2 : (comp(va, vc) ? 3 : 1);
        else pk = comp(va, vc) ? 1 : (comp(vb, vc) ? 3 : 2);
        const uint32_t pv = cs->md_val[pk];
        const int xp = cs->md_idx[pk];
        const int pick = pk == 1 ? f + 1 : (pk == 2 ? f + len / 2 : l - 1);
// ... 192 lines not shown
                wseeds += __popcll(__ballot(left && (v & 0xfffffu) != 0u));
                const unsigned long long be = __ballot(emit);
                __builtin_amdgcn_wave_barrier();
                if (lane == 0) { if (PL) { lBA[r] = be; lCA[r] = __popcll(be); } else { gBA[r] = be; gCA[r] = __popcll(be); } }
            }
            if (lane == 0 && wseeds) lds_add((lds_i32*)&cs->lseeds, wseeds);
            if (t == 0) W.E[off] = pv;
            __syncthreads();
            if (w == 0) { const int tot = PL ? wave_scan_rows(lCA, R, lane) : wave_scan_rows(gCA, R, lane); if (lane == 0) cs->nright = tot; }
            __syncthreads();
            uint32_t* Pn = PL ? W.P0 : Pg2;
            for (int r = w; r < R; r += SW) {
                const int i = a1 + r * 64 + lane;
                const unsigned long long be = TBA(r);
                if ((be >> lane) & 1ull) {
                    const uint32_t v = V[i];
                    const unsigned long long bg = TBG(r);
                    const int grank = key_of(v) >= kp ? nG - (TCG(r) + __popcll(bg & ltm)) : 0x7fffffff;
                    const int dst = a1 + TCA(r) + __popcll(be & ltm);
                    Pn[dst] = PL ? Pl[i] : Pg[i];
                    V2[dst] = grank <= K ? V[W.T[grank]] : v;
                }
            }
            __syncthreads();
            const int nright = cs->nright;
            if (PL) {
                for (int i = a1 + t; i < a1 + nright; i += ST) Pl[i] = W.P0[i];
            }
            if (t == 0) {
                const int k = cs->n_ranges;
                cs->ranges[k].off = off; cs->ranges[k].len = cut - f; cs->ranges[k].depth = depth - 1;
                cs->n_ranges = k + 1;
                cs->e_used = off + (cut - f);
                cs->seeds = seeds - cs->lseeds;
                cs->f = cut; cs->depth = depth - 1; cs->a = a1; cs->b = a1 + nright; cs->cur = cur ^ 1;
            }
            __syncthreads();
#undef TBA
#undef TBG
#undef TCA
#undef TCG
#ifdef LF_SEED_STAMPS
            if (t == 0) atomicAdd(&g_dbg_chain[blockIdx.x % 8][1], 1);
#endif
        }
    }
    __syncthreads();
}

template <int NT>
__device__ __forceinline__ void seed_radix_pass(const uint32_t* __restrict__ src, uint32_t* __restrict__ dst, int n, int shift,
                                                uint32_t* cnt , int* tot, int* base)
{
    const int t = threadIdx.x, lane = t & 63, wave = t >> 6;
    const int seg = (n + NT - 1) / NT;
    const int i0 = min(n, t * seg), i1 = min(n, i0 + seg);
    for (int b = 0; b < SNB; ++b) cnt[b * NT + t] = 0;
    for (int i = i0; i < i1; ++i) cnt[(int)((src[i] >> shift) & (SNB - 1)) * NT + t]++;
    __syncthreads();
    for (int bb = 0; bb < SNB / (NT / 64); ++bb) {
        const int b = wave * (SNB / (NT / 64)) + bb;
        int carry = 0;
        for (int c = 0; c < NT / 64; ++c) {
            const int v = (int)cnt[b * NT + c * 64 + lane];
            const int inc = wave_incl_scan_dpp(v);
            cnt[b * NT + c * 64 + lane] = (uint32_t)(carry + inc - v);
            carry += readlane(inc, 63);
        }
        if (lane == 0) tot[b] = carry;
    }
    __syncthreads();
    if (wave == 0) {
        const int v = lane < SNB ? tot[lane] : 0;
        const int inc = wave_incl_scan_dpp(v);
        if (lane < SNB) base[lane] = inc - v;
    }
    __syncthreads();
    for (int i = i0; i < i1; ++i) {
        const uint32_t it = src[i];
        const int b = (int)((it >> shift) & (SNB - 1));
        dst[(uint32_t)base[b] + cnt[b * NT + t]++] = it;
    }
    __syncthreads();
}


__device__ __forceinline__ int seed32_chain(const SeedWork& W, int n, int m, int n_seeds, uint32_t* lds, int lds_words)
{
    __shared__ ChainState cstate;
    const int t = threadIdx.x;
    SEED_T(t0);
    sparse_chain<false>(W, nullptr, nullptr, &cstate, n, m, n_seeds, as_lds<lds_u32>(lds), lds_words);
    int* state = reinterpret_cast<int*>(W.RT);
    if (cstate.stop) return cstate.stop;
    if (t == 0) { state[0] = cstate.e_used; state[1] = cstate.n_ranges; }
    for (int i = t; i < cstate.n_ranges; i += ST) { state[2 + 3 * i] = cstate.ranges[i].off; state[3 + 3 * i] = cstate.ranges[i].len; state[4 + 3 * i] = cstate.ranges[i].depth; }
#ifdef LF_SEED_STAMPS
    { const long long t1 = (long long)wall_clock64(); if (t == 0 && blockIdx.x < 6) printf("[seed32] problem %d: n %d list %d seeds %d | chain %lld (%d folds %d, %d splits %d -> %d dense in %d ranges) (x10 ns) | fold: passA %lld counts %lld median %lld K %lld passB %lld state %lld | split: build %lld counts %lld K %lld TV %lld out %lld\n", (int)blockIdx.x, n, m, n_seeds, t1 - t0, g_dbg_chain[blockIdx.x % 8][0], g_dbg_chain[blockIdx.x % 8][2], g_dbg_chain[blockIdx.x % 8][1], g_dbg_chain[blockIdx.x % 8][3], cstate.e_used, cstate.n_ranges, g_dbg_f[blockIdx.x % 8][0], g_dbg_f[blockIdx.x % 8][1], g_dbg_f[blockIdx.x % 8][2], g_dbg_f[blockIdx.x % 8][3], g_dbg_f[blockIdx.x % 8][4], g_dbg_f[blockIdx.x % 8][5], g_dbg_f[blockIdx.x % 8][6], g_dbg_f[blockIdx.x % 8][7], g_dbg_f[blockIdx.x % 8][8], g_dbg_f[blockIdx.x % 8][9], g_dbg_f[blockIdx.x % 8][10]); }
#endif
    return 0;
}

template <int NT>
__device__ __forceinline__ void seed32_dense(const SeedWork& W, int n_seeds, int n_bins, uint32_t* lds, int rows_cap, int* tot, int* base)
{
    __shared__ SeedRange ranges[kMaxRanges];
    __shared__ int hdr[2];
    const int t = threadIdx.x, lane = t & 63, w = t >> 6;
    const int* state = reinterpret_cast<const int*>(W.RT);
    if (t < 2) hdr[t] = state[t];
    __syncthreads();
    const int M = hdr[0], n_ranges = hdr[1];
    for (int i = t; i < n_ranges; i += NT) { ranges[i].off = state[2 + 3 * i]; ranges[i].len = state[3 + 3 * i]; ranges[i].depth = state[4 + 3 * i]; }
    __syncthreads();
    SEED_T(t1);
    static_assert(NT == 64 * SW2, "the wave form's workgroup");
    introsort_loop_waves<NT>(W.E, M, ranges, n_ranges, W.dscratch, lds, rows_cap, W.PP);
    SEED_T(t2);
    uint32_t* A = W.out;
    uint32_t* B = W.PP;
    int* rowc = reinterpret_cast<int*>(W.T);
    const int R = (M + 63) >> 6;
    for (int r = w; r < R; r += NT / 64) {
        const int i = r * 64 + lane;
        const uint32_t v = i < M ? W.E[i] : 0u;
        const unsigned long long bb = __ballot((v & 0xfffffu) != 0u);
        if (lane == 0) rowc[r] = __popcll(bb);
    }
    __syncthreads();
    if (w == 0) (void)wave_scan_rows(rowc, R, lane);
    __syncthreads();
    for (int r = w; r < R; r += NT / 64) {
        const int i = r * 64 + lane;
        const uint32_t v = i < M ? W.E[i] : 0u;
        const bool seed = (v & 0xfffffu) != 0u;
        const unsigned long long bb = __ballot(seed);
        if (seed) B[rowc[r] + lanes_below(bb, lane)] = ((uint32_t)((n_bins - 1) - (int)key_of(v)) << 20) | ((v & 0xfffffu) - 1u);
    }
    __syncthreads();
    uint32_t* cnt = lds;
    seed_radix_pass<NT>(B, A, n_seeds, 20, cnt, tot, base);
    seed_radix_pass<NT>(A, B, n_seeds, 24, cnt, tot, base);
    seed_radix_pass<NT>(B, A, n_seeds, 28, cnt, tot, base);
#ifdef LF_SEED_STAMPS
    { const long long t3 = (long long)wall_clock64(); if (t == 0 && blockIdx.x < 6) printf("[seed32 dense] problem %d: %d elements in %d ranges, seeds %d | loop %lld (%d big partitions, %d listed ranges; global %lld  blocks %lld)  final %lld (x10 ns) | %lld levels: a %lld b %lld d %lld e+f %lld\n", (int)blockIdx.x, M, n_ranges, n_seeds, t2 - t1, g_dbg_big[blockIdx.x % 8], g_dbg_small[blockIdx.x % 8], g_dbg_t[blockIdx.x % 8][0], g_dbg_t[blockIdx.x % 8][1], t3 - t2, g_dbg_w[blockIdx.x % 8][0], g_dbg_w[blockIdx.x % 8][1], g_dbg_w[blockIdx.x % 8][2], g_dbg_w[blockIdx.x % 8][3], g_dbg_w[blockIdx.x % 8][4]); }
#endif
}

__device__ __forceinline__ void plane_scan(uint32_t* lds, int words, int* wave_tot)
{
    const int tid = (int)threadIdx.x, lane = tid & 63, wave = tid >> 6;
    unsigned long long* bits64 = reinterpret_cast<unsigned long long*>(lds);
    uint16_t* pref = reinterpret_cast<uint16_t*>(lds + 2 * words);
    const int pairs = words >> 1;
    const int per = (pairs + ST - 1) / ST;
    const int w0 = tid * per < pairs ? tid * per : pairs, w1 = w0 + per < pairs ? w0 + per : pairs;
    int mine = 0;
    for (int q = w0; q < w1; ++q) mine += __builtin_popcountll(bits64[2 * q]) + __builtin_popcountll(bits64[2 * q + 1]);
    const int incl = wave_incl_scan_dpp(mine);
    if (lane == 63) wave_tot[wave] = incl;
    __syncthreads();
    int basev = incl - mine;
    for (int k = 0; k < wave; ++k) basev += wave_tot[k];
    for (int q = w0; q < w1; ++q) { pref[q] = (uint16_t)basev; basev += __builtin_popcountll(bits64[2 * q]) + __builtin_popcountll(bits64[2 * q + 1]); }
    __syncthreads();
}

__device__ __forceinline__ SeedWork seed_work(uint32_t* sa, uint32_t* sb, uint32_t* oa, uint32_t* ob, uint32_t* tt, size_t cap)
{
    SeedWork W;
    W.E = sa; W.V0 = sa + cap;
    W.V1 = sb; W.P0 = sb + cap;
    W.P1 = oa; W.PP = ob;
    W.T = tt; W.RT = tt + ((cap + 1) & ~(size_t)1);
    W.dscratch = reinterpret_cast<unsigned long long*>(sb);
    W.out = oa;
    W.cap = (int)cap;
    return W;
}

__global__ __launch_bounds__(ST, LF_SEED_OCC) void k_lsd_seed32(LsdParams p, int* __restrict__ n_rec, int* __restrict__ norder, int* __restrict__ rec_need,
                                                   const unsigned long long* __restrict__ maxgrad,
                                                   const uint32_t* __restrict__ c_xy, const double* __restrict__ c_mod,
                                                   const uint32_t* __restrict__ l_addr, double* l_mod, const int* __restrict__ n_low,
                                                   unsigned long long* __restrict__ sort_a, unsigned long long* __restrict__ sort_b,
                                                   uint32_t* __restrict__ order_a, uint32_t* __restrict__ order_b, int plane_ok, int lds_words)
{
    extern __shared__ __attribute__((aligned(16))) uint32_t seed_lds[];
    __shared__ int tot[SNB];
    __shared__ int base[SNB];
    __shared__ int wave_tot[SW];
    __shared__ int n_list;
    const int pc = blockIdx.x, t = threadIdx.x, lane = t & 63;
    const size_t Ps = (size_t)p.rec_cap;
    const size_t o = (size_t)pc * Ps;
    const int nd = n_rec[pc];
    if (nd == 0) return;
    const SeedWork W = seed_work(reinterpret_cast<uint32_t*>(sort_a + o), reinterpret_cast<uint32_t*>(sort_b + o), order_a + o, order_b + o,
                                 reinterpret_cast<uint32_t*>(l_mod + o), Ps);
    const int Wg = p.Ws - 1, Hg = p.Hs - 1;
    const int n = Wg * Hg;
    const double max_grad = __longlong_as_double((long long)maxgrad[pc]);
    const double bin_coef = (max_grad > 0) ? (double)(p.n_bins - 1) / max_grad : 0;
    const int nl = n_low[pc];
    if (nl > p.rec_cap || nd + nl > p.rec_cap) {
        if (t == 0) { atomicMax(rec_need, nd + nl); n_rec[pc] = 0; norder[pc] = 0; }
        return;
    }
    if (plane_ok && nd + nl <= 65535) {
        const int words = bitplane_words((size_t)n);
        for (int i = t; i < 2 * words; i += ST) seed_lds[i] = 0u;
        if (t == 0) n_list = 0;
        __syncthreads();
        for (int e = t; e < nd; e += ST) {
            const uint32_t xy = c_xy[o + e];
            const int pos = (int)(xy >> 16) * Wg + (int)(xy & 0xffffu);
            atomicOr(seed_lds + (pos >> 5), 1u << (pos & 31));
        }
        for (int j = t; j < nl; j += ST) {
            const uint32_t a = l_addr[o + j];
            if ((int)(l_mod[o + j] * bin_coef) > 0) {
                const int y = (int)(a / (uint32_t)p.Ws), x = (int)(a - (uint32_t)y * (uint32_t)p.Ws);
                const int pos = y * Wg + x;
                atomicOr(seed_lds + (pos >> 5), 1u << (pos & 31));
            }
        }
        __syncthreads();
        plane_scan(seed_lds, words, wave_tot);
        int mine = 0;
        for (int e = t; e < nd; e += ST) {
            const uint32_t xy = c_xy[o + e];
            const int pos = (int)(xy >> 16) * Wg + (int)(xy & 0xffffu);
            const uint32_t idx = bitplane_rank(seed_lds, (size_t)n, pos);
            W.P0[idx] = (uint32_t)pos;
            W.V0[idx] = ((uint32_t)(int)(c_mod[o + e] * bin_coef) << 20) | (uint32_t)(e + 1);
        }
        for (int j = t; j < nl; j += ST) {
            const uint32_t a = l_addr[o + j];
            const int bin = (int)(l_mod[o + j] * bin_coef);
            if (bin > 0) {
                const int y = (int)(a / (uint32_t)p.Ws), x = (int)(a - (uint32_t)y * (uint32_t)p.Ws);
                const int pos = y * Wg + x;
                const uint32_t idx = bitplane_rank(seed_lds, (size_t)n, pos);
                W.P0[idx] = (uint32_t)pos;
                W.V0[idx] = (uint32_t)bin << 20;
                ++mine;
// ... 7 lines not shown
        uint32_t* LB = W.P1;
        if (t == 0) n_list = 0;
        __syncthreads();
        for (int j0 = 0; j0 < nl; j0 += ST) {
            const int j = j0 + t;
            uint32_t item = 0;
            bool on = false;
            if (j < nl) {
                const uint32_t a = l_addr[o + j];
                const int bin = (int)(l_mod[o + j] * bin_coef);
                const int y = (int)(a / (uint32_t)p.Ws), x = (int)(a - (uint32_t)y * (uint32_t)p.Ws);
                on = bin > 0;
                item = ((uint32_t)(y * Wg + x) << 10) | (uint32_t)bin;
            }
            const unsigned long long bo = __ballot(on);
            int wbase = 0;
            if (lane == 0 && bo) wbase = atomicAdd(&n_list, __popcll(bo));
            wbase = __builtin_amdgcn_readfirstlane(wbase);
            if (on) LA[wbase + lanes_below(bo, lane)] = item;
        }
        __syncthreads();
        const int nlz = n_list;
        __syncthreads();
        uint32_t* src = LA;
        uint32_t* dst = LB;
        for (int shift = 10; shift < 32; shift += 4) {
            seed_radix_pass<ST>(src, dst, nlz, shift, seed_lds, tot, base);
            uint32_t* x = src; src = dst; dst = x;
        }
        for (int e = t; e < nd; e += ST) {
            const uint32_t xy = c_xy[o + e];
            const int pos = (int)(xy >> 16) * Wg + (int)(xy & 0xffffu);
            int x = 0, y = nlz;
            while (x < y) { const int mid = (x + y) >> 1; if ((int)(src[mid] >> 10) < pos) x = mid + 1; else y = mid; }
            W.P0[e + x] = (uint32_t)pos;
            W.V0[e + x] = ((uint32_t)(int)(c_mod[o + e] * bin_coef) << 20) | (uint32_t)(e + 1);
        }
        for (int j = t; j < nlz; j += ST) {
            const uint32_t it = src[j];
            const int pos = (int)(it >> 10);
            int x = 0, y = nd;
            while (x < y) { const int mid = (x + y) >> 1; const uint32_t xy = c_xy[o + mid]; if ((int)(xy >> 16) * Wg + (int)(xy & 0xffffu) < pos) x = mid + 1; else y = mid; }
            W.P0[j + x] = (uint32_t)pos;
            W.V0[j + x] = (it & 1023u) << 20;
        }
        __syncthreads();
    }
    const int m = nd + n_list;
    __syncthreads();
    const int need = seed32_chain(W, n, m, nd, seed_lds, lds_words);
    if (need && t == 0) { atomicMax(rec_need, need); n_rec[pc] = 0; norder[pc] = 0; }
}

__global__ __launch_bounds__(DT, kDenseOcc) void k_lsd_seed32_dense(LsdParams p, const int* __restrict__ n_rec, double* l_mod,
                                                            unsigned long long* __restrict__ sort_a, unsigned long long* __restrict__ sort_b,
                                                            uint32_t* __restrict__ order_a, uint32_t* __restrict__ order_b, int rows_cap)
{
    extern __shared__ __attribute__((aligned(16))) uint32_t seed_lds[];
    __shared__ int tot[SNB];
    __shared__ int base[SNB];
    const int pc = blockIdx.x;
    const size_t Ps = (size_t)p.rec_cap;
    const size_t o = (size_t)pc * Ps;
    const int nd = n_rec[pc];
    if (nd == 0) return;
    const SeedWork W = seed_work(reinterpret_cast<uint32_t*>(sort_a + o), reinterpret_cast<uint32_t*>(sort_b + o), order_a + o, order_b + o,
                                 reinterpret_cast<uint32_t*>(l_mod + o), Ps);
    seed32_dense<DT>(W, nd, p.n_bins, seed_lds, rows_cap, tot, base);
}

__global__ __launch_bounds__(ST, LF_SEED_OCC) void k_std_sort_debug(const uint32_t* __restrict__ E, uint32_t* __restrict__ work, int n, int cap, int* __restrict__ count, int lds_words)
{
    extern __shared__ __attribute__((aligned(16))) uint32_t seed_lds[];
    const int t = threadIdx.x, lane = t & 63, w = t >> 6;
    const SeedWork W = seed_work(work, work + 2 * (size_t)cap, work + 4 * (size_t)cap, work + 5 * (size_t)cap, work + 6 * (size_t)cap, (size_t)cap);
    int* rowc = reinterpret_cast<int*>(W.RT);
    const int R = (n + 63) >> 6;
    for (int r = w; r < R; r += SW) {
        const int i = r * 64 + lane;
        const uint32_t v = i < n ? E[i] : 0u;
        const unsigned long long bb = __ballot(key_of(v) != 0u);
        if (lane == 0) rowc[r] = __popcll(bb);
    }
    __syncthreads();
    __shared__ int m_sh;
    if (w == 0) { const int total = wave_scan_rows(rowc, R, lane); if (lane == 0) m_sh = total; }
    __syncthreads();
    for (int r = w; r < R; r += SW) {
        const int i = r * 64 + lane;
        const uint32_t v = i < n ? E[i] : 0u;
        const bool on = key_of(v) != 0u;
        const unsigned long long bb = __ballot(on);
        if (on) { const int idx = rowc[r] + lanes_below(bb, lane); W.P0[idx] = (uint32_t)i; W.V0[idx] = v; }
    }
    __syncthreads();
    const int m = m_sh;
    if (t == 0) *count = m;
    if (m == 0) return;
    if (seed32_chain(W, n, m, m, seed_lds, lds_words) && t == 0) *count = 0;
}

__global__ __launch_bounds__(DT, kDenseOcc) void k_std_sort_debug_dense(uint32_t* __restrict__ work, int cap, int rows_cap, const int* __restrict__ count)
{
    extern __shared__ __attribute__((aligned(16))) uint32_t seed_lds[];
    __shared__ int tot[SNB];
    __shared__ int base[SNB];
    const int m = *count;
    if (m == 0) return;
    const SeedWork W = seed_work(work, work + 2 * (size_t)cap, work + 4 * (size_t)cap, work + 5 * (size_t)cap, work + 6 * (size_t)cap, (size_t)cap);
    seed32_dense<DT>(W, m, 1024, seed_lds, rows_cap, tot, base);
}

constexpr size_t kPlaneLdsBytes = 56 * 1024;
static size_t seed_lds_bytes(long long n)
{
    size_t words = (size_t)SNB * ST;
    bool planes = false;
    if (n < (1ll << 30)) {
        const size_t two = 2 * (((size_t)plane_words_for((int)n) + 1) & ~(size_t)1);
        planes = two * 4 <= kPlaneLdsBytes;
        if (planes && words < two) words = two;
    }
    if (!planes && words < 8192) words = 8192;
    return words * sizeof(uint32_t);
}
static size_t seed_dense_lds_bytes(int rows_cap)
{
    size_t words = (size_t)rows_cap * 6 + 128;
    if (words < (size_t)SW2 * kWaveWords) words = (size_t)SW2 * kWaveWords;
    if (words < (size_t)kBlkWords) words = (size_t)kBlkWords;
    if (words < (size_t)SNB * DT) words = (size_t)SNB * DT;
    return words * sizeof(uint32_t);
}

bool lsd_seed32_supported(const LsdParams& p)
{
    const long long n = (long long)(p.Hs - 1) * (p.Ws - 1);
    return p.n_bins <= 4096 && (long long)p.Hs * p.Ws < (1 << 21) && n >= 1 && (double)(p.n_bins - 1) * p.rho / 360.7 >= 1.0;
}

void launch_lsd_seed32(const LsdParams& p, const LsdRecords& r, const LsdCompact& c, int n_frames, int* rec_need, int big, hipStream_t s)
{
    const long long n = (long long)(p.Hs - 1) * (p.Ws - 1);
    int rows_cap = kRowsLds;
    if (big) {
        const long long full = ((n + 63) / 64 + 1 + 63) / 64 * 64;
        if ((size_t)full * 24 + 512 <= (size_t)kMaxLdsBytes) rows_cap = (int)full;
    }
    const size_t lds = seed_lds_bytes(n), lds2 = seed_dense_lds_bytes(rows_cap);
    const int plane_ok = bitplane_lds_words((size_t)n) * 4 <= lds;
    if (lds > 48 * 1024)
        (void)hipFuncSetAttribute(reinterpret_cast<const void*>(k_lsd_seed32), hipFuncAttributeMaxDynamicSharedMemorySize, (int)lds);
    if (lds2 > 48 * 1024)
        (void)hipFuncSetAttribute(reinterpret_cast<const void*>(k_lsd_seed32_dense), hipFuncAttributeMaxDynamicSharedMemorySize, (int)lds2);
    static const char* diag_skip = getenv("LF_DIAG_SKIP");
    if (!(diag_skip && strstr(diag_skip, "seedchain")))
    hipLaunchKernelGGL(k_lsd_seed32, dim3(n_frames * 3), dim3(ST), lds, s, p, r.n_rec, c.norder, rec_need, r.maxgrad, c.c_xy, c.c_mod, r.l_addr, r.l_mod,
                       r.n_low, c.sort_a, c.sort_b, c.order_a, c.order_b, plane_ok, (int)(lds / 4));
    if (!(diag_skip && (strstr(diag_skip, "seeddense") || strstr(diag_skip, "seedchain"))))
    hipLaunchKernelGGL(k_lsd_seed32_dense, dim3(n_frames * 3), dim3(DT), lds2, s, p, r.n_rec, r.l_mod, c.sort_a, c.sort_b, c.order_a, c.order_b, rows_cap);
}

size_t std_sort_debug_words(int n) { const size_t cap = ((size_t)(n < 1024 ? 1024 : n) + 63) / 64 * 64; return 12 * cap; }

void launch_std_sort_debug(const uint32_t* E, uint32_t* work, int n, int* count, hipStream_t s)
{
    const size_t cap = ((size_t)(n < 1024 ? 1024 : n) + 63) / 64 * 64;
    const int rows_cap = kRowsLds;
    const size_t lds = seed_lds_bytes(n), lds2 = seed_dense_lds_bytes(rows_cap);
    if (lds > 48 * 1024)
        (void)hipFuncSetAttribute(reinterpret_cast<const void*>(k_std_sort_debug), hipFuncAttributeMaxDynamicSharedMemorySize, (int)lds);
    if (lds2 > 48 * 1024)
        (void)hipFuncSetAttribute(reinterpret_cast<const void*>(k_std_sort_debug_dense), hipFuncAttributeMaxDynamicSharedMemorySize, (int)lds2);
    hipLaunchKernelGGL(k_std_sort_debug, dim3(1), dim3(ST), lds, s, E, work, n, (int)cap, count, (int)(lds / 4));
    hipLaunchKernelGGL(k_std_sort_debug_dense, dim3(1), dim3(DT), lds2, s, work, (int)cap, rows_cap, static_cast<const int*>(count));
}

}
```

### lane_slam_amd/csrc/lanefront_debug.hip

```cpp
#include <string.h>
#include <vector>
#include "lanefront_handle.h"

using namespace lf;

extern "C" int lf_debug_std_sort(lf_handle* h, const int32_t* keys, int n, int32_t* order)
{
    if (!h) return LF_ERR_NOT_INITIALISED;
    if (!keys || !order || n < 1 || n >= (1 << 20)) { lf_set_error(h, LF_ERR_BAD_ARG, "lf_debug_std_sort: bad argument (1 <= n < 2^20)"); return LF_ERR_BAD_ARG; }
    LF_HIP_CHECK(h, hipSetDevice(h->device));
    hipStream_t s = h->stream;
    std::vector<uint32_t> e((size_t)n);
    for (int i = 0; i < n; ++i) {
        if (keys[i] < 0 || keys[i] > 1023) { lf_set_error(h, LF_ERR_BAD_ARG, "lf_debug_std_sort: keys must be in [0, 1023]"); return LF_ERR_BAD_ARG; }
        e[i] = ((uint32_t)keys[i] << 20) | (uint32_t)(i + 1);
    }
    int rc;
    const size_t words = std_sort_debug_words(n);
    Staging st(h);
    const uint32_t* d_e = st.in(0, e.data(), (size_t)n * 4, h->a_q);
    if ((rc = scratch(h, h->a_m, words * 4)) || (rc = scratch(h, h->a_best, 64)) || (rc = st.upload())) return rc;
    launch_std_sort_debug(d_e, static_cast<uint32_t*>(h->a_m.p), n, static_cast<int*>(h->a_best.p), s);
    LF_HIP_CHECK(h, hipGetLastError());
    int cnt = 0;
    if ((rc = fetch(h, { { &cnt, h->a_best.p, sizeof(int) } })) != LF_OK) return rc;
    const size_t cap = words / 12;
    if (cnt > 0 && (rc = fetch(h, { { e.data(), static_cast<uint32_t*>(h->a_m.p) + 4 * cap, (size_t)cnt * 4 } })) != LF_OK) return rc;
    for (int i = 0; i < cnt; ++i) order[i] = (int32_t)(e[i] & 0xfffffu);
    {
        int k = cnt;
        for (int i = 0; i < n; ++i) if (keys[i] == 0) order[k++] = i;
    }
    return LF_OK;
}

extern "C" int lf_debug_lsd_binary(lf_handle* h, const uint8_t* img, int rows, int cols, float* lines4, int cap, int* n_out)
{
    if (!h) return LF_ERR_NOT_INITIALISED;
    if (!img || !lines4 || !n_out || rows != h->Hc || cols != h->W) { lf_set_error(h, LF_ERR_BAD_ARG, "lf_debug_lsd_binary: bad argument (image must be %dx%d)", h->Hc, h->W); return LF_ERR_BAD_ARG; }
    LF_HIP_CHECK(h, hipSetDevice(h->device));
    hipStream_t s = h->stream;
    if ((size_t)h->lsd.params.rec_cap < h->lsd.Ps) {
        LF_HIP_CHECK(h, hipStreamSynchronize(s));
        const int rc = h->lsd.grow_lists(h, (int)h->lsd.Ps);
        if (rc != LF_OK) return rc;
    }
    const size_t nw = (size_t)h->Hc * h->Ww;
    std::vector<uint32_t> bits(nw, 0u), ones(nw * 3, 0xffffffffu);
    for (int y = 0; y < rows; ++y)
        for (int x = 0; x < cols; ++x)
            if (img[(size_t)y * cols + x]) bits[(size_t)y * h->Ww + (x >> 5)] |= 1u << (x & 31);
    LF_HIP_CHECK(h, hipMemcpyAsync(h->d_strong, bits.data(), nw * 4, hipMemcpyHostToDevice, s));
    LF_HIP_CHECK(h, hipMemcpyAsync(h->d_maskbits, ones.data(), nw * 12, hipMemcpyHostToDevice, s));
    LF_HIP_CHECK(h, hipMemsetAsync(h->lsd.d_maxgrad, 0, 3 * sizeof(unsigned long long), s));
    h->lsd.grad(1, h->d_strong, h->d_maskbits, false, s);
    h->lsd.order(1, 0, s);
    h->lsd.label(1, false, s);
    h->lsd.grow(1, h->d_slot_lines, h->d_counts, kGrowLdsKb[h->lsd.grow_lds_level], true, false, s);
    LF_HIP_CHECK(h, hipGetLastError());
    int n = 0;
    if (const int rc = fetch(h, { { &n, h->d_counts.p, sizeof(int) } })) return rc;
    h->last_frames = 1;
    h->plugin_ready = false;
    *n_out = n;
    if (n > h->cap_lines) { lf_set_error(h, LF_ERR_CAPACITY, "LSD found %d lines, max_lines_per_color is %d", n, h->cap_lines); return LF_ERR_CAPACITY; }
    if (n > cap) { lf_set_error(h, LF_ERR_CAPACITY, "%d lines exceed caller capacity %d", n, cap); return LF_ERR_CAPACITY; }
    return fetch(h, { { lines4, h->d_slot_lines.p, (size_t)n * 4 * sizeof(float) } });
}

extern "C" int lf_debug_segments(lf_handle* h, int mode, int n_frames, const int32_t* counts, const float* lines4, const uint8_t* masks,
                                 lf_segments* out, int* n_segments)
{
    if (!h) return LF_ERR_NOT_INITIALISED;
    if (h->flight.kind != InFlight::NONE) { lf_set_error(h, LF_ERR_BAD_ARG, "lf_debug_segments: a batch is in flight on this handle: call lf_wait first"); return LF_ERR_BAD_ARG; }
    if (!counts || !lines4 || !out || n_frames < 1 || n_frames > h->max_frames || (mode != 0 && mode != 1)) {
        lf_set_error(h, LF_ERR_BAD_ARG, "lf_debug_segments: bad argument (1 <= n_frames <= %d, mode 0 or 1, counts, lines4 and out not null)", h->max_frames);
        return LF_ERR_BAD_ARG;
    }
    const size_t nprob = (size_t)n_frames * 3;
    for (size_t i = 0; i < nprob; ++i)
        if (counts[i] < 0) { lf_set_error(h, LF_ERR_BAD_ARG, "lf_debug_segments: counts[%zu] = %d is negative", i, counts[i]); return LF_ERR_BAD_ARG; }
    LF_HIP_CHECK(h, hipSetDevice(h->device));
    hipStream_t s = h->stream;
    LF_HIP_CHECK(h, hipMemcpyAsync(h->d_counts, counts, nprob * sizeof(int32_t), hipMemcpyHostToDevice, s));
    LF_HIP_CHECK(h, hipMemcpyAsync(h->d_slot_lines, lines4, nprob * h->cap_lines * 4 * sizeof(float), hipMemcpyHostToDevice, s));
    std::vector<uint32_t> bits;
    if (masks) {
        const size_t nw = (size_t)h->Hc * h->Ww;
        bits.assign(nprob * nw, 0u);
        for (size_t pc = 0; pc < nprob; ++pc)
            for (int y = 0; y < h->Hc; ++y)
                for (int x = 0; x < h->W; ++x)
                    if (masks[(pc * h->Hc + y) * h->W + x]) bits[pc * nw + (size_t)y * h->Ww + (x >> 5)] |= 1u << (x & 31);
        LF_HIP_CHECK(h, hipMemcpyAsync(h->d_maskbits, bits.data(), bits.size() * 4, hipMemcpyHostToDevice, s));
    }
    lf_segments dev = h->d_out;
    dev.capacity = out->capacity < h->out_capacity ? out->capacity : h->out_capacity;
    if (dev.capacity < 0) dev.capacity = 0;
    if (!out->lines) dev.lines = nullptr;
    if (!out->normals) dev.normals = nullptr;
    if (!out->color) dev.color = nullptr;
    if (!out->pixels_normalized) dev.pixels_normalized = nullptr;
    if (!out->ground) dev.ground = nullptr;
    if (!out->keep) dev.keep = nullptr;
    dev.desc = nullptr; dev.code = nullptr;
    dev.frame_offset = h->d_frame_offset;
    h->slot_mode = mode == 1 ? SEG_HOUGH : SEG_FLOAT;
// ... 83 lines not shown
```

### lane_slam_amd/csrc/lanefront_handle.h

```cpp
#pragma once
#include <stdio.h>
#include <stdlib.h>
#include <string.h>
#include <memory>
#include <utility>
#include <vector>
#include "lanefront_core.h"
#include "jpeg_entropy.h"
#include "k_edlines_types.h"
#include "k_hough.h"
#include "k_jenc.h"
#include "k_rectify.h"

namespace lf {

struct JpegState {
    lf::jpeg::WorkerPool pool;
    std::vector<lf::jpeg::FrameCoefs> frames;
    int rows = 0, cols = 0, max_frames = 0;
    DevBuf planes, entries, block_end, hdrs, out;
    DevBuf gh_clean, gh_sub, gh_seg, gh_info, gh_coef;
    std::vector<int> h_status;
    HostArray<void> h_stage;
    hipEvent_t staged = nullptr;
// ... 39 lines not shown
    KlArrays staged;
    HostArray<KlTotals> h_pinned;
    int32_t* h_frame_status() const { return reinterpret_cast<int32_t*>(h_pinned.p + 1); }
    int alloc(lf_handle* h);
    int images(lf_handle* h, const uint8_t* images, int n, int input_kind, int on_device, const uint8_t** d);
    int upload(lf_handle* h, DevBuf& buf, const uint8_t* planes, int n, const uint8_t** d);
    int keylines(lf_handle* h, const char* who, const lf_keylines& out, int on_device, int describe, lf_keylines* dev);
};

int kl_batch_check(lf_handle* h, const char* who, const uint8_t* images, const lf_keylines* out, int n_frames, int n_octaves, int input_kind);
KlOut kl_out(const lf_keylines& k, int32_t* frame);

struct KlOctave {
    int W = 0, H = 0, cap = 0, max_edges = 0, max_lines = 0;
    bool marks_in_lds = false;
    bool aflags_on = false;
    DevBuf src, blur, dxy, g, anchors, part, chain, sid, gmarks, counts, l_ep, l_c, l_dir, l_npx, l_sal, tl, rs_tab, ework;
    DevBuf aflags;
};

struct KlState {
    int n_octaves = 0;
    KlOctave oct[LF_MAX_OCTAVES];
    KlBatch batch;
    DevBuf status, big;
    DevBuf m_fo, m_totals, m_erased, m_kept;
    KlArrays unmasked;
    DevBuf any_tmp, any_blur;
    DevBuf d_frame, d_io, d_angle, d_npx, d_oct, d_desc, d_code, d_n;
    size_t lds_bytes = 0;
    int last_octaves = 0, last_frames = 0;
};

struct LsdState {
    LsdParams params;
    ResizeTables rt{};
    int seed_order = LF_LSD_SEED_OPENCV30, max_frames = 0;
    size_t Ps = 0;
    int max_nsx = 0, max_nsy = 0;
    int label_items_full = 0;
    DevArray<int> d_xofs, d_y0, d_y1;
    DevArray<float> d_xa, d_yb;
    DevArray<uint32_t> d_raddr, d_order_a, d_order_b, d_cxy, d_reg, d_laddr;
    DevArray<float> d_rdeg, d_cdeg, d_rsd, d_csd;
    DevArray<double> d_rmod, d_rcs, d_rsn, d_cmod, d_ccs, d_lmod;
    DevArray<unsigned long long> d_sort_a, d_sort_b;
    DevArray<uint16_t> d_clabel, d_comp_list;
    DevArray<uint32_t> d_tile_list, d_gused;
    DevArray<int> d_row_start, d_norder, d_comp_count, d_comp_key, d_perm;
    DevArray<float> d_tmp_lines;
    DevArray<int> d_tmp_tags;
    DevArray<uint8_t> d_zero; size_t zero_bytes = 0;
    unsigned long long* d_maxgrad = nullptr;
    int *d_nrec = nullptr, *d_nlow = nullptr, *d_tile_count = nullptr;
    BatchStatus* d_status = nullptr;
    int lists_grown = 0;
    bool lists_lost = false;
    bool grow_mixed = false;
    int grow_lds_level = 0;
    int env_lds_level = -1;
    int env_mixed = -1;
    int env_bitmap = 1;

    int init(lf_handle* h, int Hc, int W, const lf_lsd_options& o, int seed_order, int max_frames, int cap_lines);
    int alloc_lists(lf_handle* h, int rec_cap);
    void free_lists();
    int grow_lists(lf_handle* h, int need);
    void adapt_slice(int over_small, int over_medium, int problems);
    LsdRecords records() const;
    LsdCompact compact() const;
    LsdComponents components(bool use_perm = true) const;
    void grad(int n, const uint32_t* edge_bits, const uint32_t* mask_bits, bool counters_zeroed, hipStream_t s);
    void grad_gray(int n, const uint8_t* gray, hipStream_t s);
    void order(int n, int big, hipStream_t s);
    void label(int n, bool rank, hipStream_t s);
    void grow(int n, float* lines, int* counts, int lds_kb, bool mixed, bool use_perm, hipStream_t s);
};

struct LsdKlLevel {
    LsdState lsd;
    DevArray<float> lines;
    DevArray<int> counts;
    lf_lsd_options opts{};
    bool ready = false;
};

struct LsdKlState {
    LsdKlLevel level[LF_MAX_OCTAVES];
    DevBuf pyr[LF_MAX_OCTAVES];
    KlBatch batch;
};

struct InFlight {
    enum Kind { NONE, SEGMENTS, KEYLINES } kind = NONE;
    const uint8_t* in = nullptr; int n = 0; lf_segments out{}; bool describe = false;
    int problems = 0, capacity = 0;
};

struct MatcherState {
    DevBuf codes;
    std::vector<std::pair<int, int> > index_map;
    int num_images = 0;
    int total = 0;
    DevBuf q, idx, dist, off;
};

// ... 118 lines not shown
```

### lane_slam_amd/csrc/lanefront_lsd.hip

```cpp
#include <string.h>
#include <math.h>
#include <vector>
#include "lanefront_handle.h"
#include "lsd_bitplane.h"
#include "k_lsd_grad.h"

namespace lf {

struct CounterBlock {
    size_t nrec, nlow, tile_count, status, bytes;
    explicit CounterBlock(size_t nprob) : nrec(nprob * 8), nlow(nrec + nprob * 4), tile_count(nlow + nprob * 4), status(tile_count + 16), bytes(status + sizeof(BatchStatus)) {}
};

int LsdState::init(lf_handle* h, int Hc, int W, const lf_lsd_options& o, int seed_order_, int max_frames_, int cap_lines)
{
    seed_order = seed_order_;
    max_frames = max_frames_;
    LsdParams& L = params;
    memset(&L, 0, sizeof(L));
    L.Hc = Hc; L.W = W; L.Ww = (W + 31) / 32;
    L.scaled = o.scale != 1.0;
    L.scale = o.scale;
    if (o.scale <= 0 || o.scale > 1.0) { lf_set_error(h, LF_ERR_UNSUPPORTED, "lsd_scale must be in (0,1]"); return LF_ERR_UNSUPPORTED; }
    if (L.scaled) { L.Ws = dm::round_half_even(W * o.scale); L.Hs = dm::round_half_even(Hc * o.scale); }
    else { L.Ws = W; L.Hs = Hc; }
    const int Hs = L.Hs, Ws = L.Ws;
    Ps = (size_t)Hs * Ws;
    if (Ps >= (1u << 20) || L.Ws > 65535 || L.Hs > 65535) { lf_set_error(h, LF_ERR_UNSUPPORTED, "scaled LSD image too large"); return LF_ERR_UNSUPPORTED; }
    if ((size_t)((L.Hs + 2) & ~1) * 4 + 512 * 4 + 1024 > 64 * 1024) { lf_set_error(h, LF_ERR_UNSUPPORTED, "scaled LSD image has %d rows: the row table exceeds the LDS of one problem", L.Hs); return LF_ERR_UNSUPPORTED; }
    if (o.n_bins < 2 || o.n_bins > 4096) { lf_set_error(h, LF_ERR_UNSUPPORTED, "lsd_n_bins must be in [2,4096] (a seed is its bin above a 20-bit pixel index in one word)"); return LF_ERR_UNSUPPORTED; }
    if (L.scaled) {
        const double sigma = (o.scale < 1) ? (o.sigma_scale / o.scale) : o.sigma_scale;
        const double sprec = 3;
        const unsigned hh = (unsigned)ceil(sigma * sqrt(2 * sprec * dm::dlog(10.0)));
        const int n = 1 + 2 * (int)hh;
        if (n > kMaxGaussTaps) { lf_set_error(h, LF_ERR_UNSUPPORTED, "LSD Gaussian needs %d taps (max %d)", n, kMaxGaussTaps); return LF_ERR_UNSUPPORTED; }
        const double scale2X = -0.5 / (sigma * sigma);
        double sum = 0;
        for (int i = 0; i < n; ++i) { double x = i - (n - 1) * 0.5; double t = dm::dexp(scale2X * x * x); L.k[i] = t; sum += t; }
        sum = 1.0 / sum;
        for (int i = 0; i < n; ++i) L.k[i] *= sum;
        L.ntaps = n; L.half = n / 2;
    } else { L.ntaps = 1; L.half = 0; L.k[0] = 1.0; }
    L.prec = 3.14159265358979323846 * o.ang_th / 180;
    L.p = o.ang_th / 180;
    L.rho = o.quant / dm::dsin(L.prec);
    L.log_nt = 5 * (dm::dlog10((double)L.Ws) + dm::dlog10((double)L.Hs)) / 2 + dm::dlog10(11.0);
    L.min_reg_size = (int)(-L.log_nt / dm::dlog10(L.p));
    L.log_eps = o.log_eps; L.density_th = o.density_th;
    L.n_bins = o.n_bins; L.refine = o.refine; L.cap_lines = cap_lines;
    if (seed_order != LF_LSD_SEED_OPENCV30 && seed_order != LF_LSD_SEED_OPENCV32) { lf_set_error(h, LF_ERR_BAD_ARG, "lsd_seed_order %d: LF_LSD_SEED_OPENCV30 or LF_LSD_SEED_OPENCV32", seed_order); return LF_ERR_BAD_ARG; }
    if (seed_order == LF_LSD_SEED_OPENCV32 && !lsd_seed32_supported(L)) { lf_set_error(h, LF_ERR_UNSUPPORTED, "lsd_seed_order OPENCV32: the %dx%d LSD image exceeds the row tables of the sort emulation, or (n_bins - 1) * quant / sin(ang_th) < 361 (k_lsd_seed32.hip)", L.Ws, L.Hs); return LF_ERR_UNSUPPORTED; }
    L.label_lds = kLabelLds;
    {
        const size_t plane = bitplane_lds_words(Ps) * 4;
        if (plane <= 150 * 1024 && plane / 4 > (size_t)L.label_lds) L.label_lds = (int)((plane / 4 < 65534 ? plane / 4 : 65534) & ~(size_t)1);
    }
    L.label_items = (int)(Ps / 3 / 1024) * 1024;
    if (L.label_items > 64512) L.label_items = 64512;
    if (L.label_items < kLabelItems) L.label_items = kLabelItems;
    L.label_items_max = L.label_items;
    label_items_full = L.label_items;
    L.rec_cap = (int)Ps;
    std::vector<int> xofs(Ws), y0(Hs), y1(Hs);
// ... 1 lines not shown
    int xmax = Ws;
    const double scale_x = 1.0 / L.scale, scale_y = 1.0 / L.scale;
    for (int dx = 0; dx < Ws; ++dx) {
        float fx; int sx;
        if (L.scaled) {
            fx = (float)((dx + 0.5) * scale_x - 0.5);
            sx = dm::ifloor((double)fx);
            fx -= sx;
        } else { fx = 0.f; sx = dx; }
        if (sx < 0) { fx = 0; sx = 0; }
        if (sx + 1 >= W) {
            if (dx < xmax) xmax = dx;
            if (sx >= W - 1) { fx = 0; sx = W - 1; }
        }
        xofs[dx] = sx; xa[2 * dx] = 1.f - fx; xa[2 * dx + 1] = fx;
    }
    for (int dy = 0; dy < Hs; ++dy) {
        float fy; int sy;
        if (L.scaled) {
            fy = (float)((dy + 0.5) * scale_y - 0.5);
            sy = dm::ifloor((double)fy);
            fy -= sy;
        } else { fy = 0.f; sy = dy; }
        yb[2 * dy] = 1.f - fy; yb[2 * dy + 1] = fy;
        y0[dy] = sy < 0 ? 0 : (sy > Hc - 1 ? Hc - 1 : sy);
        y1[dy] = sy + 1 < 0 ? 0 : (sy + 1 > Hc - 1 ? Hc - 1 : sy + 1);
    }
    lsd_grad_footprint(xofs.data(), y0.data(), y1.data(), W, Ws, Hs, &max_nsx, &max_nsy);
    {
        const size_t lds = lsd_grad_carve(L.half, max_nsx, max_nsy).bytes + kLsdGradStaticLds;
        if (lds > kLsdGradMaxLds) { lf_set_error(h, LF_ERR_UNSUPPORTED, "lsd_scale %.3f needs %zu B of LDS per tile (max %zu)", L.scale, lds, kLsdGradMaxLds); return LF_ERR_UNSUPPORTED; }
        if (lsd_tiles_x(Ws) > kLsdMaxTilesPerSide || lsd_tiles_y(Hs) > kLsdMaxTilesPerSide || max_frames * 3 > kLsdMaxTileProblems || L.Ww > kLsdMaxWordCols) {
            lf_set_error(h, LF_ERR_UNSUPPORTED, "LSD image %d x %d of %d frames: more tiles than a tile list entry names", Ws, Hs, max_frames);
            return LF_ERR_UNSUPPORTED;
        }
    }
    if (dalloc(h, &d_xofs, Ws) || dalloc(h, &d_y0, Hs) || dalloc(h, &d_y1, Hs) || dalloc(h, &d_xa, 2 * (size_t)Ws) || dalloc(h, &d_yb, 2 * (size_t)Hs))
        return LF_ERR_HIP;
    LF_HIP_CHECK(h, hipMemcpy(d_xofs, xofs.data(), Ws * sizeof(int), hipMemcpyHostToDevice));
    LF_HIP_CHECK(h, hipMemcpy(d_y0, y0.data(), Hs * sizeof(int), hipMemcpyHostToDevice));
    LF_HIP_CHECK(h, hipMemcpy(d_y1, y1.data(), Hs * sizeof(int), hipMemcpyHostToDevice));
    LF_HIP_CHECK(h, hipMemcpy(d_xa, xa.data(), 2 * (size_t)Ws * sizeof(float), hipMemcpyHostToDevice));
    LF_HIP_CHECK(h, hipMemcpy(d_yb, yb.data(), 2 * (size_t)Hs * sizeof(float), hipMemcpyHostToDevice));
    rt.xofs = d_xofs; rt.xa = d_xa; rt.y0 = d_y0; rt.y1 = d_y1; rt.yb = d_yb; rt.xmax = xmax;
    const size_t nprob = (size_t)max_frames * 3, cap = nprob * (size_t)cap_lines;
    if (dalloc(h, &d_tile_list, nprob * (size_t)(lsd_tiles_x(Ws) * lsd_tiles_y(Hs))) ||
        dalloc(h, &d_gused, nprob * ((Ps + 31) / 32)) || dalloc(h, &d_row_start, nprob * (size_t)(Hs + 1)) ||
        dalloc(h, &d_comp_list, nprob * (size_t)kCompCap) || dalloc(h, &d_comp_count, nprob) || dalloc(h, &d_perm, nprob) || dalloc(h, &d_comp_key, nprob) ||
        dalloc(h, &d_tmp_lines, cap * 4) || dalloc(h, &d_tmp_tags, cap) || dalloc(h, &d_norder, nprob))
        return LF_ERR_HIP;
    const CounterBlock cb(nprob);
    zero_bytes = cb.bytes;
    if (dalloc(h, &d_zero, zero_bytes)) return LF_ERR_HIP;
    d_maxgrad = reinterpret_cast<unsigned long long*>(d_zero.p);
    d_nrec = reinterpret_cast<int*>(d_zero + cb.nrec);
    if (seed_order == LF_LSD_SEED_OPENCV32) d_nlow = reinterpret_cast<int*>(d_zero + cb.nlow);
    d_tile_count = reinterpret_cast<int*>(d_zero + cb.tile_count);
    d_status = reinterpret_cast<BatchStatus*>(d_zero + cb.status);
    LF_HIP_CHECK(h, hipMemset(d_zero, 0, zero_bytes));
    if (const char* ev = getenv("LF_GROW_LDS_LEVEL")) { const int v = atoi(ev); env_lds_level = v < 0 ? 0 : (v > 2 ? 2 : v); }
    if (const char* ev = getenv("LF_GROW_MIXED")) env_mixed = atoi(ev) != 0 ? 1 : 0;
    if (const char* ev = getenv("LF_GROW_BITMAP")) { const int v = atoi(ev); env_bitmap = v < 0 ? 0 : v; }
    return LF_OK;
}

void LsdState::free_lists()
{
    for (auto* b : { &d_raddr, &d_order_a, &d_order_b, &d_cxy, &d_reg, &d_laddr }) b->reset();
    for (auto* b : { &d_rdeg, &d_cdeg, &d_rsd, &d_csd }) b->reset();
    for (auto* b : { &d_rmod, &d_rcs, &d_rsn, &d_cmod, &d_ccs, &d_lmod }) b->reset();
    d_sort_a.reset(); d_sort_b.reset(); d_clabel.reset();
    params.r_sd = nullptr; params.c_sd = nullptr;
}

int LsdState::alloc_lists(lf_handle* h, int rec_cap)
{
    const size_t nprob = (size_t)max_frames * 3, S = (size_t)rec_cap;
    LsdParams& L = params;
    L.rec_cap = rec_cap;
    const int li = rec_cap > kLabelItems ? rec_cap : kLabelItems;
    L.label_items = label_items_full < li ? label_items_full : li;
    L.label_items_max = L.label_items;
    if (dalloc(h, &d_raddr, nprob * S) || dalloc(h, &d_rdeg, nprob * S) || dalloc(h, &d_rmod, nprob * S) ||
        dalloc(h, &d_rcs, nprob * S) || dalloc(h, &d_rsn, nprob * S) || dalloc(h, &d_sort_a, nprob * S) || dalloc(h, &d_sort_b, nprob * S) ||
        dalloc(h, &d_order_a, nprob * S) || dalloc(h, &d_order_b, nprob * S) || dalloc(h, &d_cxy, nprob * S) || dalloc(h, &d_cdeg, nprob * S) ||
        dalloc(h, &d_cmod, nprob * S) || dalloc(h, &d_ccs, nprob * S * 2) || dalloc(h, &d_reg, nprob * lsd_grow_reg_stride(L)) ||
        dalloc(h, &d_clabel, nprob * S))
        return LF_ERR_HIP;
    if (dalloc(h, &d_rsd, nprob * S * 2) || dalloc(h, &d_csd, nprob * S * 2)) return LF_ERR_HIP;
    L.r_sd = d_rsd; L.c_sd = d_csd;
    if (seed_order == LF_LSD_SEED_OPENCV32 && (dalloc(h, &d_laddr, nprob * S) || dalloc(h, &d_lmod, nprob * S)))
        return LF_ERR_HIP;
    return LF_OK;
}

int LsdState::grow_lists(lf_handle* h, int need)
{
    size_t cap = ((size_t)need + (size_t)need / 4 + 4095) / 4096 * 4096;
    if (cap > Ps) cap = Ps;
    if (alloc_trace()) fprintf(stderr, "lanefront: a problem needs %d list entries, the handle holds %d: growing to %zu\n", need, params.rec_cap, cap);
    const int old_cap = params.rec_cap;
    free_lists();
    int rc = alloc_lists(h, (int)cap);
    if (rc == LF_OK) { ++lists_grown; lists_lost = false; return LF_OK; }
    free_lists();
    if (alloc_lists(h, old_cap) != LF_OK) { free_lists(); params.rec_cap = old_cap; lists_lost = true; }
    lf_set_error(h, LF_ERR_HIP, "out of device memory growing the LSD lists from %d to %zu entries per problem%s", old_cap, cap,
                 lists_lost ? "; the lists are gone: the handle refuses detection" : "; the handle keeps its old lists");
    return LF_ERR_HIP;
}

void LsdState::adapt_slice(int over_small, int over_medium, int problems)
{
    grow_lds_level = over_medium * 4 > problems ? 2 : (over_small * 20 > problems ? 1 : 0);
    grow_mixed = (grow_lds_level == 0 ? over_small : over_medium) * 100 > problems;
}

LsdRecords LsdState::records() const
{
    LsdRecords v{};
    v.r_addr = d_raddr; v.r_deg = d_rdeg; v.r_mod = d_rmod; v.r_cs = d_rcs; v.r_sn = d_rsn;
    v.n_rec = d_nrec; v.maxgrad = d_maxgrad;
    v.l_addr = d_laddr; v.l_mod = d_lmod; v.n_low = d_nlow;
    v.list = d_tile_list; v.list_count = d_tile_count;
    v.max_nsx = max_nsx; v.max_nsy = max_nsy;
    return v;
}

LsdCompact LsdState::compact() const
{
    LsdCompact v{};
    v.sort_a = d_sort_a; v.sort_b = d_sort_b; v.order_a = d_order_a; v.order_b = d_order_b;
    v.norder = d_norder;
    v.c_xy = d_cxy; v.c_deg = d_cdeg; v.c_mod = d_cmod;
    v.c_cs = d_ccs; v.c_sn = d_ccs ? d_ccs + 1 : nullptr;
    v.row_start = d_row_start;
    return v;
}

LsdComponents LsdState::components(bool use_perm) const
{
    LsdComponents v{};
    v.c_label = d_clabel;
    v.comp_list = d_comp_list; v.comp_count = d_comp_count; v.comp_key = d_comp_key; v.comp_cap = kCompCap;
    v.perm = use_perm ? d_perm.p : nullptr;
    v.reg = d_reg; v.gused = d_gused;
    v.tmp_lines = d_tmp_lines; v.tmp_tags = d_tmp_tags;
    return v;
}

void LsdState::grad(int n, const uint32_t* edge_bits, const uint32_t* mask_bits, bool counters_zeroed, hipStream_t s)
{
    launch_lsd_grad(params, rt, records(), n, edge_bits, mask_bits, &d_status->rec_need, counters_zeroed, s);
}

void LsdState::grad_gray(int n, const uint8_t* gray, hipStream_t s)
{
    launch_lsd_grad_gray(params, rt, records(), n, gray, s);
}

void LsdState::order(int n, int big, hipStream_t s)
{
    launch_lsd_order(params, records(), compact(), n, s);
    if (seed_order == LF_LSD_SEED_OPENCV32) launch_lsd_seed32(params, records(), compact(), n, &d_status->rec_need, big, s);
}

void LsdState::label(int n, bool rank, hipStream_t s)
{
    launch_lsd_label(params, compact(), components(), n, s);
    if (rank) launch_lsd_rank(components(), n * 3, s);
}

void LsdState::grow(int n, float* lines, int* counts, int lds_kb, bool mixed, bool use_perm, hipStream_t s)
{
    launch_lsd_grow(params, compact(), components(use_perm), n, lines, counts, lds_kb, mixed, env_bitmap, s);
}

}
```

### lane_slam_amd/csrc/lanefront_lsdkl.hip

```cpp

#include <string.h>
#include <algorithm>
#include <string>
#include "lanefront_handle.h"
#include "wave.h"

using namespace lf;


extern "C" void lf_lsd_default_options(lf_lsd_options* o)
{
    if (!o) return;
    o->refine = 1; o->scale = 0.8; o->sigma_scale = 0.6; o->quant = 2.0; o->ang_th = 22.5; o->log_eps = 0.0; o->density_th = 0.7; o->n_bins = 1024;
    o->min_length = 0.0;
}

static bool lsdkl_same_opts(const lf_lsd_options& a, const lf_lsd_options& b)
{
    return a.refine == b.refine && a.scale == b.scale && a.sigma_scale == b.sigma_scale && a.quant == b.quant && a.ang_th == b.ang_th &&
           a.log_eps == b.log_eps && a.density_th == b.density_th && a.n_bins == b.n_bins;
}

static int lsdkl_level(lf_handle* h, LsdKlLevel& lv, int Ho, int Wo, const lf_lsd_options& opts)
{
// ... 57 lines not shown
            total += __popcll(__ballot(keep));
        }
    }
    if (lane == 0) frame_count[f] = total;
}

__global__ __launch_bounds__(64) void k_lsdkl_fill(LsdKlLevels L, int n_octaves, const int* __restrict__ frame_offset, int capacity, KlOut out)
{
    const int f = blockIdx.x, lane = threadIdx.x;
    const int base = frame_offset[f], n = frame_offset[f + 1] - base;
    if (n <= 0 || base + n > capacity) return;
    int cls0 = 0, out0 = 0;
    for (int o = 0; o < n_octaves; ++o) {
        int cnt = L.counts[o][3 * f];
        cnt = cnt < L.cap_lines ? cnt : L.cap_lines;
        const int cols = L.W[o], rows = L.H[o];
        const float octaveScale = (float)(1 << o);
        for (int l0 = 0; l0 < cnt; l0 += 64) {
            const int l = l0 + lane;
            float e[4] = { 0, 0, 0, 0 }, len = 0;
            bool keep_len = false, keep_mask = false;
            if (l < cnt) lsdkl_line(L, o, f, l, e, len, keep_len, keep_mask);
            const unsigned long long bl = __ballot(keep_len), bo = __ballot(keep_len && keep_mask);
            const unsigned long long below = lane_mask_lt(lane);
            if (keep_len && keep_mask) {
                const float e0 = e[0], e1 = e[1], e2 = e[2], e3 = e[3];
                const size_t k = (size_t)base + out0 + __popcll(bo & below);
                const float sx = e0 * octaveScale, sy = e1 * octaveScale, ex = e2 * octaveScale, ey = e3 * octaveScale;
                if (out.start_end) { out.start_end[4 * k] = sx; out.start_end[4 * k + 1] = sy; out.start_end[4 * k + 2] = ex; out.start_end[4 * k + 3] = ey; }
                if (out.in_octave) { out.in_octave[4 * k] = e0; out.in_octave[4 * k + 1] = e1; out.in_octave[4 * k + 2] = e2; out.in_octave[4 * k + 3] = e3; }
                if (out.line_length) out.line_length[k] = len;
                const int ix0 = dm::round_half_even((double)e0), iy0 = dm::round_half_even((double)e1);
                const int ix1 = dm::round_half_even((double)e2), iy1 = dm::round_half_even((double)e3);
                const int adx = ix1 > ix0 ? ix1 - ix0 : ix0 - ix1, ady = iy1 > iy0 ? iy1 - iy0 : iy0 - iy1;
                if (out.num_pixels) out.num_pixels[k] = (adx > ady ? adx : ady) + 1;
                if (out.angle) out.angle[k] = (float)dm::datan2((double)(ey - sy), (double)(ex - sx));
                if (out.class_id) out.class_id[k] = cls0 + __popcll(bl & below);
                if (out.octave) out.octave[k] = o;
                if (out.size) out.size[k] = (ex - sx) * (ey - sy);
                if (out.response) out.response[k] = len / (float)(cols > rows ? cols : rows);
                if (out.pt) { out.pt[2 * k] = (ex + sx) / 2; out.pt[2 * k + 1] = (ey + sy) / 2; }
                if (out.salience) out.salience[k] = 0.f;
                if (out.frame) out.frame[k] = f;
            }
            cls0 += __popcll(bl);
            out0 += __popcll(bo);
        }
    }
}

static int lsdkl_run_level(lf_handle* h, LsdKlLevel& lv, const uint8_t* d_gray, int n)
{
    hipStream_t st = h->stream;
    LF_HIP_CHECK(h, hipMemsetAsync(lv.lsd.d_maxgrad, 0, (size_t)n * 3 * sizeof(unsigned long long), st));
    lv.lsd.grad_gray(n, d_gray, st);
    lv.lsd.order(n, 1, st);
    lv.lsd.label(n, false, st);
    lv.lsd.grow(n, lv.lines, lv.counts, kGrowLdsKb[2], true, false, st);
    LF_HIP_CHECK(h, hipGetLastError());
    return LF_OK;
}

extern "C" int lf_lsd_keylines_batch_ex(lf_handle* h, const uint8_t* images, int n_frames, int input_kind, int images_on_device, int n_octaves,
                                        const lf_lsd_options* opts_in, const uint8_t* masks, int masks_on_device,
                                        lf_keylines* out, int out_on_device, int describe, int* n_keylines);

extern "C" int lf_lsd_keylines_batch(lf_handle* h, const uint8_t* images, int n_frames, int input_kind, int images_on_device, int n_octaves,
                                     lf_keylines* out, int out_on_device, int describe, int* n_keylines)
{
    return lf_lsd_keylines_batch_ex(h, images, n_frames, input_kind, images_on_device, n_octaves, nullptr, nullptr, 0, out, out_on_device, describe, n_keylines);
}

extern "C" int lf_lsd_keylines_batch_ex(lf_handle* h, const uint8_t* images, int n_frames, int input_kind, int images_on_device, int n_octaves,
                                        const lf_lsd_options* opts_in, const uint8_t* masks, int masks_on_device,
                                        lf_keylines* out, int out_on_device, int describe, int* n_keylines)
{
    if (!h) return LF_ERR_NOT_INITIALISED;
    lf_lsd_options opts;
    lf_lsd_default_options(&opts);
    if (opts_in) opts = *opts_in; else opts.min_length = -1.0;
    if (opts.refine < 0 || opts.refine > 2 || opts.n_bins < 2 || opts.n_bins > 4096 || !(opts.scale > 0) || !(opts.sigma_scale > 0) || !(opts.quant >= 0) ||
        !(opts.ang_th > 0 && opts.ang_th < 180) || !(opts.density_th >= 0 && opts.density_th < 1)) {
        lf_set_error(h, LF_ERR_BAD_ARG, "lf_lsd_keylines_batch_ex: options outside cv::createLineSegmentDetector's domain (refine 0..2, n_bins 2..4096, scale > 0, "
                     "sigma_scale > 0, quant >= 0, 0 < ang_th < 180, 0 <= density_th < 1)");
        return LF_ERR_BAD_ARG;
    }
    int rc;
    if ((rc = kl_batch_check(h, "lf_lsd_keylines_batch", images, out, n_frames, n_octaves, input_kind)) != LF_OK) return rc;
    if (out->capacity < 1) { lf_set_error(h, LF_ERR_BAD_ARG, "lf_lsd_keylines_batch: out->capacity < 1"); return LF_ERR_BAD_ARG; }
    if (describe && n_octaves > 1 && h->desc_params.reduction_ratio != 2) {
        lf_set_error(h, LF_ERR_UNSUPPORTED, "lf_lsd_keylines_batch: describe over %d octaves with reductionRatio %d: cv::pyrDown only takes a destination "
                     "within 2 pixels of half the source (the reference raises cv::Exception here)", n_octaves, h->desc_params.reduction_ratio);
        return LF_ERR_UNSUPPORTED;
    }
    LF_HIP_CHECK(h, hipSetDevice(h->device));
    hipStream_t s = h->stream;
    if (!h->lsdkl) { h->lsdkl.reset(new (std::nothrow) LsdKlState()); if (!h->lsdkl) return LF_ERR_HIP; }
    LsdKlState* k = h->lsdkl.get();
    KlBatch& b = k->batch;
    const size_t B = (size_t)h->max_frames;
    const uint8_t* gray0;
    if ((rc = b.images(h, images, n_frames, input_kind, images_on_device, &gray0)) != LF_OK) return rc;
    if (input_kind == 0) {
        launch_pre_gray(h->pre, gray0, n_frames, h->d_gray, s);
        gray0 = h->d_gray;
    }
    int W = h->W, Hh = h->Hc;
// ... 47 lines not shown
```

Before: 120,200.

## Fuse LSD component labeling into seed32 pass and parallelize rank kernel

Moves the union-find labeling routine into a shared header so the seed32 ordering kernel can run labeling itself, using tickets and a CU count. The goal is to cut a separate label launch and its global round-trip. The rank kernel now runs on multiple blocks, one thread per problem, and reads the shared key table in int4 vector loads. The fused path adds complexity and a fallback (launch_lsd_seed32 now returns bool), and much of the wiring is not visible here.

```diff
diff --git a/include/lanefront.h b/include/lanefront.h
--- a/include/lanefront.h
+++ b/include/lanefront.h
@@ -503,6 +503,7 @@
 LF_API int lf_debug_segments(lf_handle* h, int mode, int n_frames, const int32_t* counts, const float* lines4, const uint8_t* masks,
                              lf_segments* out, int* n_segments);
 LF_API int lf_debug_std_sort(lf_handle* h, const int32_t* keys, int n, int32_t* order);
+LF_API int lf_debug_lsd_rank(lf_handle* h, const int32_t* keys, int n, int32_t* perm);
 LF_API int lf_lsd_size(const lf_handle* h, int* rows, int* cols);
 LF_API int lf_suggested_depth(const lf_handle* h);
 
diff --git a/lane_slam_amd/_lib.py b/lane_slam_amd/_lib.py
--- a/lane_slam_amd/_lib.py
+++ b/lane_slam_amd/_lib.py
@@ -22,7 +22,7 @@
     "lf_map_set_profiling", "lf_map_get_timing", "lf_map_stage_name",
     "lf_descriptor_default_params", "lf_set_descriptor_params", "lf_get_descriptor_params",
     "lf_edlines_default_params", "lf_keylines_batch", "lf_describe_keylines", "lf_keylines_debug_fetch", "lf_set_image_edlines", "lf_knn_match", "lf_radius_match", "lf_jpeg_decode_batch_gpu", "lf_jpeg_decode_batch_gpu_async", "lf_jpeg_status", "lf_jpeg_decode_for_detect_async",
-    "lf_set_tie_rule", "lf_map_set_tie_rule", "lf_debug_std_sort", "lf_suggested_depth", "lf_lsd_list_capacity", "lf_lsd_scratch_stride", "lf_set_detector", "lf_detector_failures", "lf_keylines_batch_async", "lf_keylines_frame_status", "lf_lsd_keylines_batch", "lf_select_queries",
+    "lf_set_tie_rule", "lf_map_set_tie_rule", "lf_debug_std_sort", "lf_debug_lsd_rank", "lf_suggested_depth", "lf_lsd_list_capacity", "lf_lsd_scratch_stride", "lf_set_detector", "lf_detector_failures", "lf_keylines_batch_async", "lf_keylines_frame_status", "lf_lsd_keylines_batch", "lf_select_queries",
     "lf_lsd_default_options", "lf_lsd_keylines_batch_ex", "lf_keylines_batch_masked",
     "lf_matcher_add", "lf_matcher_clear", "lf_matcher_size", "lf_matcher_match", "lf_matcher_knn_match", "lf_matcher_radius_match",
     "lf_lane_filter_default_config", "lf_lane_filter_create", "lf_lane_filter_destroy", "lf_lane_filter_last_error", "lf_lane_filter_grid",
@@ -436,6 +436,8 @@
     lib.lf_suggested_depth.restype = ci
     lib.lf_debug_std_sort.argtypes = [vp, vp, ci, vp]
     lib.lf_debug_std_sort.restype = ci
+    lib.lf_debug_lsd_rank.argtypes = [vp, vp, ci, vp]
+    lib.lf_debug_lsd_rank.restype = ci
     lib.lf_set_tie_rule.argtypes = [vp, ci]
     lib.lf_set_tie_rule.restype = ci
     lib.lf_map_set_tie_rule.argtypes = [vp, ci]
diff --git a/lane_slam_amd/csrc/common.h b/lane_slam_amd/csrc/common.h
--- a/lane_slam_amd/csrc/common.h
+++ b/lane_slam_amd/csrc/common.h
@@ -151,13 +151,15 @@
                      const uint32_t* mask_bits, int* rec_need, bool counters_zeroed, hipStream_t s);
 void launch_lsd_grad_gray(const LsdParams& p, const ResizeTables& rt, const LsdRecords& r, int n_frames, const uint8_t* gray, hipStream_t s);
 bool lsd_seed32_supported(const LsdParams& p);
-void launch_lsd_seed32(const LsdParams& p, const LsdRecords& r, const LsdCompact& c, int n_frames, int* rec_need, int big, hipStream_t s);
+bool launch_lsd_seed32(const LsdParams& p, const LsdRecords& r, const LsdCompact& c, int n_frames, int* rec_need, int big, int* tickets, int n_cu,
+                       const LsdComponents* label, hipStream_t s);
 size_t std_sort_debug_words(int n);
 void launch_std_sort_debug(const uint32_t* E, uint32_t* work, int n, int* count, hipStream_t s);
 void launch_lsd_order(const LsdParams& p, const LsdRecords& r, const LsdCompact& c, int n_frames, hipStream_t s);
 void launch_lsd_dense_debug(const LsdParams& p, const LsdCompact& c, int n_frames, float* ang, double* mod, hipStream_t s);
 void launch_lsd_rank(const LsdComponents& m, int n_prob, hipStream_t s);
 void launch_lsd_label(const LsdParams& p, const LsdCompact& c, const LsdComponents& m, int n_frames, hipStream_t s);
+int lsd_label_comp_cap();
 size_t lsd_grow_reg_stride(const LsdParams& p);
 void launch_lsd_grow(const LsdParams& p, const LsdCompact& c, const LsdComponents& m, int n_frames, float* lines, int* counts,
                      int lds_kb, bool mixed, int bitmap, hipStream_t s);
diff --git a/lane_slam_amd/csrc/k_lsd_order.hip b/lane_slam_amd/csrc/k_lsd_order.hip
--- a/lane_slam_amd/csrc/k_lsd_order.hip
+++ b/lane_slam_amd/csrc/k_lsd_order.hip
@@ -1,3 +1,4 @@
+#include <climits>
 #include <cstdlib>
 #include <algorithm>
 #include "common.h"
@@ -5,6 +6,7 @@
 #include "lsd_bitplane.h"
 #include "scan.h"
 #include "wave.h"
+#include "lsd_label.h"
 
 namespace lf {
 using std::max;
@@ -15,9 +17,6 @@
 #endif
 #ifndef LF_ORDER_BM_THREADS
 #define LF_ORDER_BM_THREADS 256
-#endif
-#ifndef LF_LABEL_THREADS
-#define LF_LABEL_THREADS 256
 #endif
 constexpr int OT = LF_ORDER_THREADS;
 constexpr int OBT = LF_ORDER_BM_THREADS;
@@ -397,236 +396,42 @@
                        c.sort_a, c.sort_b, c.order_a, c.order_b, c.norder, c.c_xy, c.c_deg, c.c_mod, c.c_cs, c.c_sn, c.row_start);
 }
 
-struct UfLds {
-    volatile lds_u32* P;
-    __device__ __forceinline__ uint32_t get(uint32_t i) const { return P[i]; }
-    __device__ __forceinline__ void set(uint32_t i, uint32_t v) const { P[i] = v; }
-    __device__ __forceinline__ void add(uint32_t i, uint32_t v) const { (void)__hip_atomic_fetch_add((lds_u32*)&P[i], v, __ATOMIC_RELAXED, __HIP_MEMORY_SCOPE_WORKGROUP); }
-};
-struct UfLds16 {
-    volatile lds_u16* P;
-    __device__ __forceinline__ uint32_t get(uint32_t i) const { return P[i]; }
-    __device__ __forceinline__ void set(uint32_t i, uint32_t v) const { P[i] = (uint16_t)v; }
-    __device__ __forceinline__ uint32_t min(uint32_t i, uint32_t v) const
-    {
-        lds_u32* w = (lds_u32*)P + (i >> 1);
-        const uint32_t sh = (i & 1u) * 16u;
-        uint32_t cur = *(volatile lds_u32*)w;
-        for (;;) {
-            const uint32_t old = (cur >> sh) & 0xffffu;
-            if (v >= old) return old;
-            uint32_t expect = cur;
-            if (__hip_atomic_compare_exchange_strong(w, &expect, (cur & ~(0xffffu << sh)) | (v << sh), __ATOMIC_RELAXED, __ATOMIC_RELAXED, __HIP_MEMORY_SCOPE_WORKGROUP)) return old;
-            cur = expect;
-        }
-    }
-};
-struct UfGlb {
-    uint32_t* P;
-    __device__ __forceinline__ uint32_t get(uint32_t i) const { return __hip_atomic_load(P + i, __ATOMIC_RELAXED, __HIP_MEMORY_SCOPE_AGENT); }
-    __device__ __forceinline__ void set(uint32_t i, uint32_t v) const { __hip_atomic_store(P + i, v, __ATOMIC_RELAXED, __HIP_MEMORY_SCOPE_AGENT); }
-    __device__ __forceinline__ uint32_t min(uint32_t i, uint32_t v) const { return __hip_atomic_fetch_min(P + i, v, __ATOMIC_RELAXED, __HIP_MEMORY_SCOPE_AGENT); }
-    __device__ __forceinline__ void add(uint32_t i, uint32_t v) const { (void)__hip_atomic_fetch_add(P + i, v, __ATOMIC_RELAXED, __HIP_MEMORY_SCOPE_AGENT); }
-};
-template <class UF>
-__device__ __forceinline__ uint32_t uf_find(const UF& P, uint32_t x)
-{
-    uint32_t p = P.get(x);
-    while (p != x) {
-        const uint32_t g = P.get(p);
-        if (g != p) (void)P.min(x, g);
-        x = p;
-        p = g;
-    }
-    return x;
-}
-
-template <class UF>
-__device__ __forceinline__ void uf_unite(const UF& P, uint32_t a, uint32_t b)
-{
-    for (;;) {
-        a = uf_find(P, a);
-        b = uf_find(P, b);
-        if (a == b) return;
-        if (a < b) { const uint32_t t = a; a = b; b = t; }
-        const uint32_t old = P.min(a, b);
-        if (old == a) return;
-        a = old;
-    }
-}
-
-constexpr int LT = LF_LABEL_THREADS;
-#ifndef LF_COMP_TOP
-#define LF_COMP_TOP 8
-#endif
-constexpr int kCompTop = LF_COMP_TOP;
-
-template <bool GLB>
-__device__ __forceinline__ void lsd_label_problem(const LsdParams& p, const int* __restrict__ norder, const uint32_t* __restrict__ c_xy,
-                                                  const int* __restrict__ row_start, uint16_t* __restrict__ c_label,
-                                                  uint16_t* __restrict__ comp_list, int* __restrict__ comp_count, int* __restrict__ comp_key, int comp_cap,
-                                                  uint32_t* __restrict__ scratch, size_t scratch_stride)
-{
-    extern __shared__ __attribute__((aligned(16))) uint32_t dyn_lds[];
-    const int LS = p.label_lds;
-    __shared__ uint16_t roots[kCompCap];
-    __shared__ int n_roots, rest_total;
-    const int pc = blockIdx.x, t = threadIdx.x;
-    const size_t Ps = (size_t)p.Hs * p.Ws, o = (size_t)pc * p.rec_cap;
-    const int n = norder[pc];
-    uint16_t* lab = c_label + o;
-    uint16_t* list = comp_list + (size_t)pc * kCompCap;
-    if (n == 0) { if (t == 0) { comp_count[pc] = 0; comp_key[pc] = 0; } return; }
-    if (n > p.label_items) {
-        for (int e = t; e < n; e += LT) lab[e] = 0;
-        if (t == 0) { list[0] = 0; comp_count[pc] = 1; comp_key[pc] = n; }
-        return;
-    }
-    const uint16_t* xs_lds = reinterpret_cast<const uint16_t*>(dyn_lds + LS / 2);
-    uint32_t* gtab = scratch + (size_t)pc * scratch_stride;
-    typename std::conditional<GLB, UfGlb, UfLds16>::type parent;
-    typename std::conditional<GLB, UfGlb, UfLds>::type csize2;
-    if constexpr (GLB) { parent.P = gtab; csize2.P = gtab + ((n + 1) & ~1); }
-    else { parent.P = (volatile lds_u16*)dyn_lds; csize2.P = (volatile lds_u32*)(dyn_lds + LS / 2); }
-    auto xs = [&](int k) -> int { if constexpr (GLB) return (int)(c_xy[o + k] & 0xffffu); else return (int)xs_lds[k]; };
-    const int* rs = row_start + (size_t)pc * (p.Hs + 1);
-    if (t == 0) { n_roots = 0; rest_total = 0; }
-    if constexpr (GLB) {
-        __shared__ int wave_tot[LT / 64];
-        bitplane_build<LT>(dyn_lds, c_xy + o, n, p.Ws, Ps, wave_tot);
-        __syncthreads();
-        const unsigned long long* bits64 = reinterpret_cast<const unsigned long long*>(dyn_lds);
-        const uint16_t* pref = reinterpret_cast<const uint16_t*>(dyn_lds + 2 * bitplane_words(Ps));
-        auto bit = [&](int pos) -> bool { return (bits64[pos >> 6] >> (pos & 63)) & 1ull; };
-        auto rank = [&](int pos) -> uint32_t {
-            const int w = pos >> 6;
-            const unsigned long long lo = bits64[w & ~1], cur = bits64[w];
-            return (uint32_t)pref[w >> 1] + ((w & 1) ? (uint32_t)__builtin_popcountll(lo) : 0u) + (uint32_t)__builtin_popcountll(cur & ((1ull << (pos & 63)) - 1ull));
-        };
-        for (int e = t; e < n; e += LT) {
-            const uint32_t xy = c_xy[o + e];
-            const int x = (int)(xy & 0xffffu), y = (int)(xy >> 16), pos = y * p.Ws + x;
-            int back = 0;
-            while (back < x && bit(pos - back - 1)) ++back;
-            parent.set((uint32_t)e, (uint32_t)(e - back));
-        }
-        __syncthreads();
-        for (int e = t; e < n; e += LT) {
-            const uint32_t xy = c_xy[o + e];
-            const int x = (int)(xy & 0xffffu), y = (int)(xy >> 16);
-            if (y == 0) continue;
-            const int up = (y - 1) * p.Ws + x;
-            const bool head = x == 0 || !bit(up + p.Ws - 1);
-            const bool uL = x > 0 && bit(up - 1), uC = bit(up), uR = x + 1 < p.Ws && bit(up + 1);
-            if (head) {
-                if (uL) uf_unite(parent, (uint32_t)e, rank(up - 1));
-                else if (uC) uf_unite(parent, (uint32_t)e, rank(up));
-                if (uR && !uC) uf_unite(parent, (uint32_t)e, rank(up + 1));
-            } else if (uR && !uC) uf_unite(parent, (uint32_t)e, rank(up + 1));
-        }
-        __syncthreads();
-    } else {
-        for (int e = t; e < n; e += LT) reinterpret_cast<uint16_t*>(dyn_lds + LS / 2)[e] = (uint16_t)(c_xy[o + e] & 0xffffu);
-        __syncthreads();
-    for (int e = t; e < n; e += LT) {
-        const int y = (int)(c_xy[o + e] >> 16);
-        const int first = rs[y];
-        int h = e;
-        int xh = xs(h);
-        while (h > first) { const int xp = xs(h - 1); if (xp + 1 != xh) break; --h; xh = xp; }
-        parent.set((uint32_t)e, (uint32_t)h);
-    }
-    __syncthreads();
-    for (int e = t; e < n; e += LT) {
-        const uint32_t xy = c_xy[o + e];
-        const int x = (int)(xy & 0xffffu), y = (int)(xy >> 16);
-        if (y > 0) {
-            int lo = rs[y - 1];
-            const int end = rs[y];
-            int hi = end;
-            while (lo < hi) { const int mid = (lo + hi) >> 1; if (xs(mid) < x - 1) lo = mid + 1; else hi = mid; }
-            for (int k = lo; k < end && k < lo + 3 && xs(k) <= x + 1; ++k) uf_unite(parent, (uint32_t)e, (uint32_t)k);
-        }
-    }
-    __syncthreads();
-    }
-    for (int i = t; i < (n + 1) / 2; i += LT) csize2.set((uint32_t)i, 0u);
-    __syncthreads();
-    for (int e = t; e < n; e += LT) {
-        const uint32_t r = uf_find(parent, (uint32_t)e);
-        lab[e] = (uint16_t)r;
-        csize2.add(r >> 1, 1u << (16 * (r & 1u)));
-    }
-    __syncthreads();
-    auto csize = [&](uint32_t r) -> uint32_t { return (csize2.get(r >> 1) >> (16 * (r & 1u))) & 0xffffu; };
-    const uint32_t minsz = p.min_reg_size > 1 ? (uint32_t)p.min_reg_size : 1u;
-    for (int e = t; e < n; e += LT)
-        if (csize((uint32_t)e) >= minsz) {
-            const int k = atomicAdd(&n_roots, 1);
-            if (k < comp_cap) roots[k] = (uint16_t)e;
-        }
-    __syncthreads();
-    const int C = n_roots;
-    if (C > comp_cap) {
-        for (int e = t; e < n; e += LT) lab[e] = 0;
-        if (t == 0) { list[0] = 0; comp_count[pc] = 1; comp_key[pc] = n; }
-        return;
-    }
-    for (int i = t; i < C; i += LT) {
-        const uint32_t ri = roots[i], si = csize(ri);
-        int rank = 0;
-        for (int j = 0; j < C; ++j) {
-            const uint32_t rj = roots[j], sj = csize(rj);
-            rank += (sj > si || (sj == si && rj < ri)) ? 1 : 0;
-        }
-        list[rank] = (uint16_t)ri;
-        parent.set(ri, (uint32_t)rank);
-        if (rank == 0) comp_key[pc] = (int)si;
-        if (rank >= kCompTop) atomicAdd(&rest_total, (int)si);
-    }
-    __syncthreads();
-    if (C <= kCompTop) {
-        if (t == 0) { comp_count[pc] = C; if (C == 0) comp_key[pc] = 0; }
-        return;
-    }
-    __threadfence_block();
-    const uint16_t rest_root = list[kCompTop];
-    for (int e = t; e < n; e += LT) {
-        const uint32_t r = lab[e];
-        if (csize(r) >= minsz && parent.get(r) >= (uint32_t)kCompTop) lab[e] = rest_root;
-    }
-    if (t == 0) {
-        const int rest = rest_total;
-        const int top0 = (int)csize((uint32_t)list[0]);
-        if (rest > top0) {
-            for (int k = kCompTop; k > 0; --k) list[k] = list[k - 1];
-            list[0] = rest_root;
-            comp_key[pc] = rest;
-        }
-        comp_count[pc] = kCompTop + 1;
-    }
-}
-
+
+constexpr int kRankMax = 1024;
 __global__ __launch_bounds__(256) void k_lsd_rank(int n_prob, const int* __restrict__ norder, int* __restrict__ perm)
 {
-    __shared__ int nd[1024];
-    if (n_prob > 1024) {
-        for (int i = threadIdx.x; i < n_prob; i += 256) perm[i] = i;
-        return;
-    }
-    for (int i = threadIdx.x; i < n_prob; i += 256) nd[i] = norder[i];
-    __syncthreads();
-    for (int i = threadIdx.x; i < n_prob; i += 256) {
-        const int mine = nd[i];
-        int rank = 0;
-        for (int j = 0; j < n_prob; ++j) rank += (nd[j] > mine || (nd[j] == mine && j < i)) ? 1 : 0;
-        perm[rank] = i;
-    }
+    __shared__ __attribute__((aligned(16))) int nd[kRankMax];
+    const int i = (int)(blockIdx.x * 256 + threadIdx.x);
+    if (n_prob > kRankMax) {
+        if (i < n_prob) perm[i] = i;
+        return;
+    }
+    const int n4 = (n_prob + 3) & ~3;
+    for (int j = threadIdx.x; j < n4; j += 256) nd[j] = j < n_prob ? norder[j] : INT_MIN;
+    __syncthreads();
+    if (i >= n_prob) return;
+    const int mine = nd[i];
+    const int4* nd4 = reinterpret_cast<const int4*>(nd);
+    int rank = 0;
+    for (int j = 0; j < n4; j += 4) {
+        const int4 k = nd4[j >> 2];
+        rank += (k.x > mine || (k.x == mine && j < i)) ? 1 : 0;
+        rank += (k.y > mine || (k.y == mine && j + 1 < i)) ? 1 : 0;
+        rank += (k.z > mine || (k.z == mine && j + 2 < i)) ? 1 : 0;
+        rank += (k.w > mine || (k.w == mine && j + 3 < i)) ? 1 : 0;
+    }
+    perm[rank] = i;
 }
 
 void launch_lsd_rank(const LsdComponents& m, int n_prob, hipStream_t s)
 {
-    hipLaunchKernelGGL(k_lsd_rank, dim3(1), dim3(256), 0, s, n_prob, m.comp_key, m.perm);
+    hipLaunchKernelGGL(k_lsd_rank, dim3((n_prob + 255) / 256), dim3(256), 0, s, n_prob, m.comp_key, m.perm);
+}
+
+int lsd_label_comp_cap()
+{
+    static const int comp_cap = getenv("LF_DIAG_COMP_CAP") ? max(1, min(kCompCap, atoi(getenv("LF_DIAG_COMP_CAP")))) : kCompCap;
+    return comp_cap;
 }
 
 __global__ __launch_bounds__(LT) void k_lsd_label(LsdParams p, const int* __restrict__ norder, const uint32_t* __restrict__ c_xy,
@@ -634,30 +439,18 @@
                                                   uint16_t* __restrict__ comp_list, int* __restrict__ comp_count, int* __restrict__ comp_key, int comp_cap,
                                                   uint32_t* __restrict__ scratch, size_t scratch_stride, int plane_fits)
 {
-    const int n = norder[blockIdx.x];
-    if (n <= p.label_lds)
-        lsd_label_problem<false>(p, norder, c_xy, row_start, c_label, comp_list, comp_count, comp_key, comp_cap, scratch, scratch_stride);
-    else if (plane_fits)
-        lsd_label_problem<true>(p, norder, c_xy, row_start, c_label, comp_list, comp_count, comp_key, comp_cap, scratch, scratch_stride);
-    else {
-        const size_t o = (size_t)blockIdx.x * p.rec_cap;
-        for (int e = threadIdx.x; e < n; e += LT) c_label[o + e] = 0;
-        if (threadIdx.x == 0) { comp_list[(size_t)blockIdx.x * kCompCap] = 0; comp_count[blockIdx.x] = 1; comp_key[blockIdx.x] = n; }
-    }
+    lsd_label_any(p, (int)blockIdx.x, norder, c_xy, row_start, c_label, comp_list, comp_count, comp_key, comp_cap, scratch, scratch_stride, plane_fits);
 }
 
 void launch_lsd_label(const LsdParams& p, const LsdCompact& c, const LsdComponents& m, int n_frames, hipStream_t s)
 {
-    size_t lds = (size_t)p.label_lds * (2 + 2);
-    const size_t plane = bitplane_lds_words((size_t)p.Hs * p.Ws) * 4;
-    const int plane_fits = plane <= 150 * 1024 ? 1 : 0;
-    if (plane_fits && plane > lds) lds = plane;
+    int plane_fits = 0;
+    const size_t lds = lsd_label_lds_bytes(p, &plane_fits);
     if (lds > 48 * 1024)
         (void)hipFuncSetAttribute(reinterpret_cast<const void*>(k_lsd_label), hipFuncAttributeMaxDynamicSharedMemorySize, (int)lds);
-    static const int comp_cap = getenv("LF_DIAG_COMP_CAP") ? max(1, min(kCompCap, atoi(getenv("LF_DIAG_COMP_CAP")))) : kCompCap;
     const size_t stride = lsd_grow_reg_stride(p);
     hipLaunchKernelGGL(k_lsd_label, dim3(n_frames * 3), dim3(LT), lds, s, p, c.norder, c.c_xy, c.row_start, m.c_label, m.comp_list, m.comp_count,
-                       m.comp_key, comp_cap, m.reg, stride, plane_fits);
+                       m.comp_key, lsd_label_comp_cap(), m.reg, stride, plane_fits);
 }
 
 __global__ void k_lsd_dense_debug(LsdParams p, const int* __restrict__ norder, const uint32_t* __restrict__ c_xy,
diff --git a/lane_slam_amd/csrc/k_lsd_seed32.hip b/lane_slam_amd/csrc/k_lsd_seed32.hip
--- a/lane_slam_amd/csrc/k_lsd_seed32.hip
+++ b/lane_slam_amd/csrc/k_lsd_seed32.hip
@@ -3,6 +3,7 @@
 #include "common.h"
 #include "lsd_bitplane.h"
 #include "scan.h"
+#include "lsd_label.h"
 
 namespace lf {
 
@@ -13,6 +14,13 @@
 #define FST(k) do { } while (0)
 #define FST0 do { } while (0)
 #endif
+
+__device__ __forceinline__ int seed_tid()
+{
+    int t = (int)threadIdx.x;
+    asm volatile("" : "+v"(t));
+    return t;
+}
 
 #ifndef LF_SEED_THREADS
 #define LF_SEED_THREADS 256
@@ -211,7 +219,7 @@
     const int lo = f + 1, hi = l;
     const int R = (hi - lo + 63) >> 6;
     const uint32_t pivot = E[f];
-    if (threadIdx.x == 0) { acc[0] = 0; acc[1] = 0x7fffffff; acc[2] = 0x7fffffff; acc[3] = (pivot & 0xfffffu) != 0u; }
+    if (seed_tid() == 0) { acc[0] = 0; acc[1] = 0x7fffffff; acc[2] = 0x7fffffff; acc[3] = (pivot & 0xfffffu) != 0u; }
     __syncthreads();
     for (int r0 = w * kU; r0 < R; r0 += (NT / 64) * kU) {
         uint32_t v[kU];
@@ -233,7 +241,7 @@
     }
     __syncthreads();
     if (acc[3] == 0) { __syncthreads(); return -1; }
-    return partition_tail<true>(E, 0, lo, hi, BL, BR, PL, SX, acc, Lpos, Rpos, w, NT / 64, lane, (int)threadIdx.x, NT);
+    return partition_tail<true>(E, 0, lo, hi, BL, BR, PL, SX, acc, Lpos, Rpos, w, NT / 64, lane, seed_tid(), NT);
 }
 
 #ifdef LF_SEED_STAMPS
@@ -241,7 +249,7 @@
 __device__ long long g_dbg_b[8][6];
 __device__ long long g_dbg_w[8][8];
 __device__ long long g_dbg_f[8][12];
-#define FST(k) do { const long long n_ = (long long)wall_clock64(); if (threadIdx.x == 0) g_dbg_f[blockIdx.x % 8][k] += n_ - fs_; fs_ = n_; } while (0)
+#define FST(k) do { const long long n_ = (long long)wall_clock64(); if (seed_tid() == 0) g_dbg_f[blockIdx.x % 8][k] += n_ - fs_; fs_ = n_; } while (0)
 #define FST0 long long fs_ = (long long)wall_clock64()
 __device__ long long g_dbg_t[8][4];
 #endif
@@ -288,7 +296,7 @@
     const int lo = f + 1, hi = l;
     const int R = (hi - lo + 63) >> 6;
     const uint32_t pivot = D[f];
-    if (threadIdx.x == 0) { acc[0] = 0; acc[1] = 0x7fffffff; acc[2] = 0x7fffffff; acc[3] = (pivot & 0xfffffu) != 0u; }
+    if (seed_tid() == 0) { acc[0] = 0; acc[1] = 0x7fffffff; acc[2] = 0x7fffffff; acc[3] = (pivot & 0xfffffu) != 0u; }
     __syncthreads();
     int seeds = 0;
     for (int r = w; r < R; r += SW2) {
@@ -303,7 +311,7 @@
     if (lane == 0 && seeds) lds_add(&acc[3], seeds);
     __syncthreads();
     if (acc[3] == 0) { __syncthreads(); return -1; }
-    return partition_tail<true>(D, 0, lo, hi, BL, BR, PL, SX, acc, Lpos, Rpos, w, SW2, lane, (int)threadIdx.x, 64 * SW2);
+    return partition_tail<true>(D, 0, lo, hi, BL, BR, PL, SX, acc, Lpos, Rpos, w, SW2, lane, seed_tid(), 64 * SW2);
 }
 
 
@@ -437,7 +445,7 @@
     for (;;) {
         while (l - f > kSortThreshold) {
 #ifdef LF_SEED_STAMPS
-            if (l - f <= 64) { const long long c0 = clock64(); wave_window(D, D_generic, f, l - f, depth, (lds_u32*)Lp, lane); if (lane == 0 && (threadIdx.x >> 6) == 0) { g_dbg_w[blockIdx.x % 8][0] += 1; g_dbg_w[blockIdx.x % 8][1] += clock64() - c0; } break; }
+            if (l - f <= 64) { const long long c0 = clock64(); wave_window(D, D_generic, f, l - f, depth, (lds_u32*)Lp, lane); if (lane == 0 && (seed_tid() >> 6) == 0) { g_dbg_w[blockIdx.x % 8][0] += 1; g_dbg_w[blockIdx.x % 8][1] += clock64() - c0; } break; }
 #else
             if (l - f <= 64) { wave_window(D, D_generic, f, l - f, depth, (lds_u32*)Lp, lane); break; }
 #endif
@@ -452,7 +460,7 @@
 #endif
             const int cut = wave_partition(D, f, l, Lp, Rp, lane);
 #ifdef LF_SEED_STAMPS
-            if (lane == 0 && (threadIdx.x >> 6) == 0) { g_dbg_w[blockIdx.x % 8][2] += 1; g_dbg_w[blockIdx.x % 8][3] += clock64() - c0; g_dbg_w[blockIdx.x % 8][4] += (l - f + 62) >> 6; }
+            if (lane == 0 && (seed_tid() >> 6) == 0) { g_dbg_w[blockIdx.x % 8][2] += 1; g_dbg_w[blockIdx.x % 8][3] += clock64() - c0; g_dbg_w[blockIdx.x % 8][4] += (l - f + 62) >> 6; }
 #endif
             if (cut < 0) break;
             if (l - cut > kSortThreshold) {
@@ -490,7 +498,7 @@
     __shared__ int big_stack[3 * (72 + kMaxRanges)];
     __shared__ int n_big, n_small, n_block, next_small, n_blk_small;
     __shared__ int cur[4];
-    const int t = threadIdx.x, lane = t & 63, w = t >> 6;
+    const int t = seed_tid(), lane = t & 63, w = t >> 6;
     auto pack = [](int f, int l, int depth) { return (unsigned long long)f | ((unsigned long long)l << 24) | ((unsigned long long)depth << 48); };
     if (t == 0) {
         n_big = 0; n_small = 0; n_block = 0; next_small = 0;
@@ -747,7 +755,7 @@
 template <typename PT>
 __device__ __forceinline__ void chain_materialize(uint32_t* E, int off, int f, int l, PT P, const uint32_t* V, int a, int b)
 {
-    const int t = threadIdx.x;
+    const int t = seed_tid();
     for (int i = t; i < l - f; i += ST) E[off + i] = 0u;
     __syncthreads();
     for (int i = a + t; i < b; i += ST) { const uint32_t v = V[i]; if (v) E[off + (int)P[i] - f] = v; }
@@ -820,7 +828,7 @@
 
 __device__ __forceinline__ int plane_counts(const Plane& pl, lds_i32* wave_tot)
 {
-    const int tid = (int)threadIdx.x, lane = tid & 63, wave = tid >> 6;
+    const int tid = seed_tid(), lane = tid & 63, wave = tid >> 6;
     const int per = (pl.pairs + ST - 1) / ST;
     const int w0 = tid * per < pl.pairs ? tid * per : pl.pairs, w1 = w0 + per < pl.pairs ? w0 + per : pl.pairs;
     int mine = 0;
@@ -851,7 +859,7 @@
 __device__ __forceinline__ void chain_step_plane(const SeedWork& W, lds_of<ChainState>* cs, lds_u32* lds,
                                                  uint32_t (&pr)[kEPT], bool& regs_ok)
 {
-    const int t = threadIdx.x, lane = t & 63;
+    const int t = seed_tid(), lane = t & 63;
     const int f = cs->f, l = cs->l, a = cs->a, b = cs->b, depth = cs->depth, cur = cs->cur, seeds = cs->seeds;
     const int len = l - f;
     uint32_t* V = (cur ? W.V1 : W.V0);
@@ -1152,7 +1160,7 @@
 __device__ __forceinline__ void sparse_chain(const SeedWork& W, lds_u32* Pl, lds_u32* tab, ChainState* cs_generic, int n, int m0, int nseeds, lds_u32* plane_lds, int plane_lds_words)
 {
     lds_of<ChainState>* cs = as_lds<lds_of<ChainState>>(cs_generic);
-    const int t = threadIdx.x, lane = t & 63, w = t >> 6;
+    const int t = seed_tid(), lane = t & 63, w = t >> 6;
     if (t == 0) {
         cs->f = 0; cs->l = n; cs->depth = 2 * (31 - __clz(n)); cs->a = 0; cs->b = m0; cs->seeds = nseeds; cs->cur = 0; cs->e_used = 0; cs->n_ranges = 0; cs->stop = 0;
     }
@@ -1451,7 +1459,7 @@
 __device__ __forceinline__ void seed_radix_pass(const uint32_t* __restrict__ src, uint32_t* __restrict__ dst, int n, int shift,
                                                 uint32_t* cnt , int* tot, int* base)
 {
-    const int t = threadIdx.x, lane = t & 63, wave = t >> 6;
+    const int t = seed_tid(), lane = t & 63, wave = t >> 6;
     const int seg = (n + NT - 1) / NT;
     const int i0 = min(n, t * seg), i1 = min(n, i0 + seg);
     for (int b = 0; b < SNB; ++b) cnt[b * NT + t] = 0;
@@ -1487,7 +1495,7 @@
 __device__ __forceinline__ int seed32_chain(const SeedWork& W, int n, int m, int n_seeds, uint32_t* lds, int lds_words)
 {
     __shared__ ChainState cstate;
-    const int t = threadIdx.x;
+    const int t = seed_tid();
     SEED_T(t0);
     sparse_chain<false>(W, nullptr, nullptr, &cstate, n, m, n_seeds, as_lds<lds_u32>(lds), lds_words);
     int* state = reinterpret_cast<int*>(W.RT);
@@ -1505,7 +1513,7 @@
 {
     __shared__ SeedRange ranges[kMaxRanges];
     __shared__ int hdr[2];
-    const int t = threadIdx.x, lane = t & 63, w = t >> 6;
+    const int t = seed_tid(), lane = t & 63, w = t >> 6;
     const int* state = reinterpret_cast<const int*>(W.RT);
     if (t < 2) hdr[t] = state[t];
     __syncthreads();
@@ -1548,7 +1556,7 @@
 
 __device__ __forceinline__ void plane_scan(uint32_t* lds, int words, int* wave_tot)
 {
-    const int tid = (int)threadIdx.x, lane = tid & 63, wave = tid >> 6;
+    const int tid = seed_tid(), lane = tid & 63, wave = tid >> 6;
     unsigned long long* bits64 = reinterpret_cast<unsigned long long*>(lds);
     uint16_t* pref = reinterpret_cast<uint16_t*>(lds + 2 * words);
     const int pairs = words >> 1;
@@ -1578,8 +1586,24 @@
     return W;
 }
 
-__global__ __launch_bounds__(ST, LF_SEED_OCC) void k_lsd_seed32(LsdParams p, int* __restrict__ n_rec, int* __restrict__ norder, int* __restrict__ rec_need,
-                                                   const unsigned long long* __restrict__ maxgrad,
+__device__ __forceinline__ int seed_next_ticket(int* counter, int* slot)
+{
+    __syncthreads();
+    if (seed_tid() == 0) *slot = atomicAdd(counter, 1);
+    __syncthreads();
+    return __builtin_amdgcn_readfirstlane(*slot);
+}
+
+template <class T>
+__device__ __forceinline__ const T* seed_kernargs()
+{
+    auto k = __builtin_amdgcn_kernarg_segment_ptr();
+    asm volatile("" : "+s"(k));
+    return (const T*)k;
+}
+
+__device__ __forceinline__ void seed32_list_chain_problem(const LsdParams& p, int pc, int* __restrict__ n_rec, int* __restrict__ norder,
+                                                   int* __restrict__ rec_need, const unsigned long long* __restrict__ maxgrad,
                                                    const uint32_t* __restrict__ c_xy, const double* __restrict__ c_mod,
                                                    const uint32_t* __restrict__ l_addr, double* l_mod, const int* __restrict__ n_low,
                                                    unsigned long long* __restrict__ sort_a, unsigned long long* __restrict__ sort_b,
@@ -1590,7 +1614,7 @@
     __shared__ int base[SNB];
     __shared__ int wave_tot[SW];
     __shared__ int n_list;
-    const int pc = blockIdx.x, t = threadIdx.x, lane = t & 63;
+    const int t = seed_tid(), lane = t & 63;
     const size_t Ps = (size_t)p.rec_cap;
     const size_t o = (size_t)pc * Ps;
     const int nd = n_rec[pc];
@@ -1704,14 +1728,32 @@
     if (need && t == 0) { atomicMax(rec_need, need); n_rec[pc] = 0; norder[pc] = 0; }
 }
 
-__global__ __launch_bounds__(DT, kDenseOcc) void k_lsd_seed32_dense(LsdParams p, const int* __restrict__ n_rec, double* l_mod,
-                                                            unsigned long long* __restrict__ sort_a, unsigned long long* __restrict__ sort_b,
-                                                            uint32_t* __restrict__ order_a, uint32_t* __restrict__ order_b, int rows_cap)
+struct SeedChainArgs {
+    LsdParams p; int n_prob; int* ticket;
+    int* n_rec; int* norder; int* rec_need; const unsigned long long* maxgrad; const uint32_t* c_xy; const double* c_mod;
+    const uint32_t* l_addr; double* l_mod; const int* n_low;
+    unsigned long long* sort_a; unsigned long long* sort_b; uint32_t* order_a; uint32_t* order_b; int plane_ok, lds_words;
+};
+
+__global__ __launch_bounds__(ST, LF_SEED_OCC) void k_lsd_seed32(SeedChainArgs)
+{
+    __shared__ int next_pc;
+    for (;;) {
+        const SeedChainArgs* a = seed_kernargs<SeedChainArgs>();
+        const int pc = seed_next_ticket(a->ticket, &next_pc);
+        if (pc >= a->n_prob) break;
+        seed32_list_chain_problem(a->p, pc, a->n_rec, a->norder, a->rec_need, a->maxgrad, a->c_xy, a->c_mod, a->l_addr, a->l_mod, a->n_low,
+                                  a->sort_a, a->sort_b, a->order_a, a->order_b, a->plane_ok, a->lds_words);
+    }
+}
+
+__device__ __forceinline__ void seed32_dense_problem(const LsdParams& p, int pc, const int* __restrict__ n_rec, double* l_mod,
+                                                     unsigned long long* __restrict__ sort_a, unsigned long long* __restrict__ sort_b,
+                                                     uint32_t* __restrict__ order_a, uint32_t* __restrict__ order_b, int rows_cap)
 {
     extern __shared__ __attribute__((aligned(16))) uint32_t seed_lds[];
     __shared__ int tot[SNB];
     __shared__ int base[SNB];
-    const int pc = blockIdx.x;
     const size_t Ps = (size_t)p.rec_cap;
     const size_t o = (size_t)pc * Ps;
     const int nd = n_rec[pc];
@@ -1721,10 +1763,38 @@
     seed32_dense<DT>(W, nd, p.n_bins, seed_lds, rows_cap, tot, base);
 }
 
+struct SeedLabelArgs {
+    const int* norder; const uint32_t* c_xy; const int* row_start;
+    uint16_t* c_label; uint16_t* comp_list; int* comp_count; int* comp_key; int comp_cap;
+    uint32_t* scratch; size_t scratch_stride; int plane_fits;
+};
+
+struct SeedDenseArgs {
+    LsdParams p; int n_prob, n_label; int* ticket;
+    const int* n_rec; double* l_mod; unsigned long long* sort_a; unsigned long long* sort_b; uint32_t* order_a; uint32_t* order_b; int rows_cap;
+    SeedLabelArgs lb;
+};
+
+__global__ __launch_bounds__(DT, kDenseOcc) void k_lsd_seed32_dense(SeedDenseArgs)
+{
+    __shared__ int next_pc;
+    static_assert(DT == LT, "the labelling runs with the dense kernel's workgroup");
+    for (;;) {
+        const SeedDenseArgs* a = seed_kernargs<SeedDenseArgs>();
+        const int pc = seed_next_ticket(a->ticket, &next_pc);
+        const int n_prob = a->n_prob;
+        if (pc >= n_prob + a->n_label) break;
+        const SeedLabelArgs& lb = a->lb;
+        if (pc < n_prob) seed32_dense_problem(a->p, pc, a->n_rec, a->l_mod, a->sort_a, a->sort_b, a->order_a, a->order_b, a->rows_cap);
+        else lsd_label_any(a->p, pc - n_prob, lb.norder, lb.c_xy, lb.row_start, lb.c_label, lb.comp_list, lb.comp_count, lb.comp_key, lb.comp_cap,
+                           lb.scratch, lb.scratch_stride, lb.plane_fits);
+    }
+}
+
 __global__ __launch_bounds__(ST, LF_SEED_OCC) void k_std_sort_debug(const uint32_t* __restrict__ E, uint32_t* __restrict__ work, int n, int cap, int* __restrict__ count, int lds_words)
 {
     extern __shared__ __attribute__((aligned(16))) uint32_t seed_lds[];
-    const int t = threadIdx.x, lane = t & 63, w = t >> 6;
+    const int t = seed_tid(), lane = t & 63, w = t >> 6;
     const SeedWork W = seed_work(work, work + 2 * (size_t)cap, work + 4 * (size_t)cap, work + 5 * (size_t)cap, work + 6 * (size_t)cap, (size_t)cap);
     int* rowc = reinterpret_cast<int*>(W.RT);
     const int R = (n + 63) >> 6;
@@ -1791,7 +1861,16 @@
     return p.n_bins <= 4096 && (long long)p.Hs * p.Ws < (1 << 21) && n >= 1 && (double)(p.n_bins - 1) * p.rho / 360.7 >= 1.0;
 }
 
-void launch_lsd_seed32(const LsdParams& p, const LsdRecords& r, const LsdCompact& c, int n_frames, int* rec_need, int big, hipStream_t s)
+constexpr int kChainPerCu = 3, kDensePerCu = 3;
+static int seed_grid(int tickets, int per_cu, int n_cu)
+{
+    static const int forced = getenv("LF_SEED_GRID") ? atoi(getenv("LF_SEED_GRID")) : 0;
+    const int g = forced > 0 ? forced : per_cu * (n_cu > 0 ? n_cu : 1);
+    return g < tickets ? g : tickets;
+}
+
+bool launch_lsd_seed32(const LsdParams& p, const LsdRecords& r, const LsdCompact& c, int n_frames, int* rec_need, int big, int* tickets, int n_cu,
+                       const LsdComponents* label, hipStream_t s)
 {
     const long long n = (long long)(p.Hs - 1) * (p.Ws - 1);
     int rows_cap = kRowsLds;
@@ -1806,11 +1885,26 @@
     if (lds2 > 48 * 1024)
         (void)hipFuncSetAttribute(reinterpret_cast<const void*>(k_lsd_seed32_dense), hipFuncAttributeMaxDynamicSharedMemorySize, (int)lds2);
     static const char* diag_skip = getenv("LF_DIAG_SKIP");
+    const int n_prob = n_frames * 3;
+    SeedLabelArgs lb{};
+    int plane_fits = 0;
+    const bool with_label = label && !diag_skip && lsd_label_lds_bytes(p, &plane_fits) <= lds2;
+    if (with_label) {
+        lb.norder = c.norder; lb.c_xy = c.c_xy; lb.row_start = c.row_start;
+        lb.c_label = label->c_label; lb.comp_list = label->comp_list; lb.comp_count = label->comp_count; lb.comp_key = label->comp_key;
+        lb.comp_cap = lsd_label_comp_cap();
+        lb.scratch = label->reg; lb.scratch_stride = lsd_grow_reg_stride(p);
+        lb.plane_fits = plane_fits;
+    }
+    const int n_label = with_label ? n_prob : 0;
     if (!(diag_skip && strstr(diag_skip, "seedchain")))
-    hipLaunchKernelGGL(k_lsd_seed32, dim3(n_frames * 3), dim3(ST), lds, s, p, r.n_rec, c.norder, rec_need, r.maxgrad, c.c_xy, c.c_mod, r.l_addr, r.l_mod,
-                       r.n_low, c.sort_a, c.sort_b, c.order_a, c.order_b, plane_ok, (int)(lds / 4));
+    hipLaunchKernelGGL(k_lsd_seed32, dim3(seed_grid(n_prob, kChainPerCu, n_cu)), dim3(ST), lds, s,
+                       SeedChainArgs{ p, n_prob, tickets, r.n_rec, c.norder, rec_need, r.maxgrad, c.c_xy, c.c_mod, r.l_addr, r.l_mod, r.n_low,
+                                      c.sort_a, c.sort_b, c.order_a, c.order_b, plane_ok, (int)(lds / 4) });
     if (!(diag_skip && (strstr(diag_skip, "seeddense") || strstr(diag_skip, "seedchain"))))
-    hipLaunchKernelGGL(k_lsd_seed32_dense, dim3(n_frames * 3), dim3(DT), lds2, s, p, r.n_rec, r.l_mod, c.sort_a, c.sort_b, c.order_a, c.order_b, rows_cap);
+    hipLaunchKernelGGL(k_lsd_seed32_dense, dim3(seed_grid(n_prob + n_label, kDensePerCu, n_cu)), dim3(DT), lds2, s,
+                       SeedDenseArgs{ p, n_prob, n_label, tickets + 1, r.n_rec, r.l_mod, c.sort_a, c.sort_b, c.order_a, c.order_b, rows_cap, lb });
+    return with_label;
 }
 
 size_t std_sort_debug_words(int n) { const size_t cap = ((size_t)(n < 1024 ? 1024 : n) + 63) / 64 * 64; return 12 * cap; }
diff --git a/lane_slam_amd/csrc/lanefront_debug.hip b/lane_slam_amd/csrc/lanefront_debug.hip
--- a/lane_slam_amd/csrc/lanefront_debug.hip
+++ b/lane_slam_amd/csrc/lanefront_debug.hip
@@ -34,6 +34,18 @@
     return LF_OK;
 }
 
+extern "C" int lf_debug_lsd_rank(lf_handle* h, const int32_t* keys, int n, int32_t* perm)
+{
+    if (!h) return LF_ERR_NOT_INITIALISED;
+    if (!keys || !perm || n < 1 || n > h->lsd.max_frames * 3) { lf_set_error(h, LF_ERR_BAD_ARG, "lf_debug_lsd_rank: bad argument (1 <= n <= %d problems)", h->lsd.max_frames * 3); return LF_ERR_BAD_ARG; }
+    LF_HIP_CHECK(h, hipSetDevice(h->device));
+    hipStream_t s = h->stream;
+    LF_HIP_CHECK(h, hipMemcpyAsync(h->lsd.d_comp_key, keys, (size_t)n * sizeof(int), hipMemcpyHostToDevice, s));
+    launch_lsd_rank(h->lsd.components(), n, s);
+    LF_HIP_CHECK(h, hipGetLastError());
+    return fetch(h, { { perm, h->lsd.d_perm.p, (size_t)n * sizeof(int) } });
+}
+
 extern "C" int lf_debug_lsd_binary(lf_handle* h, const uint8_t* img, int rows, int cols, float* lines4, int cap, int* n_out)
 {
     if (!h) return LF_ERR_NOT_INITIALISED;
@@ -52,7 +64,7 @@
             if (img[(size_t)y * cols + x]) bits[(size_t)y * h->Ww + (x >> 5)] |= 1u << (x & 31);
     LF_HIP_CHECK(h, hipMemcpyAsync(h->d_strong, bits.data(), nw * 4, hipMemcpyHostToDevice, s));
     LF_HIP_CHECK(h, hipMemcpyAsync(h->d_maskbits, ones.data(), nw * 12, hipMemcpyHostToDevice, s));
-    LF_HIP_CHECK(h, hipMemsetAsync(h->lsd.d_maxgrad, 0, 3 * sizeof(unsigned long long), s));
+    LF_HIP_CHECK(h, hipMemsetAsync(h->lsd.d_zero, 0, h->lsd.zero_head_bytes(1), s));
     h->lsd.grad(1, h->d_strong, h->d_maskbits, false, s);
     h->lsd.order(1, 0, s);
     h->lsd.label(1, false, s);
diff --git a/lane_slam_amd/csrc/lanefront_handle.h b/lane_slam_amd/csrc/lanefront_handle.h
--- a/lane_slam_amd/csrc/lanefront_handle.h
+++ b/lane_slam_amd/csrc/lanefront_handle.h
@@ -115,6 +115,10 @@
     DevArray<int> d_tmp_tags;
     DevArray<uint8_t> d_zero; size_t zero_bytes = 0;
     unsigned long long* d_maxgrad = nullptr;
+    int* d_seed_tickets = nullptr;
+    size_t zero_head_bytes(int n) const { return (size_t)((uint8_t*)d_maxgrad - d_zero.p) + (size_t)n * 3 * sizeof(unsigned long long); }
+    int n_cu = 0;
+    bool label_done = false;
     int *d_nrec = nullptr, *d_nlow = nullptr, *d_tile_count = nullptr;
     BatchStatus* d_status = nullptr;
     int lists_grown = 0;
diff --git a/lane_slam_amd/csrc/lanefront_lsd.hip b/lane_slam_amd/csrc/lanefront_lsd.hip
--- a/lane_slam_amd/csrc/lanefront_lsd.hip
+++ b/lane_slam_amd/csrc/lanefront_lsd.hip
@@ -8,8 +8,8 @@
 namespace lf {
 
 struct CounterBlock {
-    size_t nrec, nlow, tile_count, status, bytes;
-    explicit CounterBlock(size_t nprob) : nrec(nprob * 8), nlow(nrec + nprob * 4), tile_count(nlow + nprob * 4), status(tile_count + 16), bytes(status + sizeof(BatchStatus)) {}
+    size_t maxgrad, nrec, nlow, tile_count, status, bytes;
+    explicit CounterBlock(size_t nprob) : maxgrad(8), nrec(maxgrad + nprob * 8), nlow(nrec + nprob * 4), tile_count(nlow + nprob * 4), status(tile_count + 16), bytes(status + sizeof(BatchStatus)) {}
 };
 
 int LsdState::init(lf_handle* h, int Hc, int W, const lf_lsd_options& o, int seed_order_, int max_frames_, int cap_lines)
@@ -117,12 +117,14 @@
     const CounterBlock cb(nprob);
     zero_bytes = cb.bytes;
     if (dalloc(h, &d_zero, zero_bytes)) return LF_ERR_HIP;
-    d_maxgrad = reinterpret_cast<unsigned long long*>(d_zero.p);
+    d_seed_tickets = reinterpret_cast<int*>(d_zero.p);
+    d_maxgrad = reinterpret_cast<unsigned long long*>(d_zero + cb.maxgrad);
     d_nrec = reinterpret_cast<int*>(d_zero + cb.nrec);
     if (seed_order == LF_LSD_SEED_OPENCV32) d_nlow = reinterpret_cast<int*>(d_zero + cb.nlow);
     d_tile_count = reinterpret_cast<int*>(d_zero + cb.tile_count);
     d_status = reinterpret_cast<BatchStatus*>(d_zero + cb.status);
     LF_HIP_CHECK(h, hipMemset(d_zero, 0, zero_bytes));
+    LF_HIP_CHECK(h, hipDeviceGetAttribute(&n_cu, hipDeviceAttributeMultiprocessorCount, h->device));
     if (const char* ev = getenv("LF_GROW_LDS_LEVEL")) { const int v = atoi(ev); env_lds_level = v < 0 ? 0 : (v > 2 ? 2 : v); }
     if (const char* ev = getenv("LF_GROW_MIXED")) env_mixed = atoi(ev) != 0 ? 1 : 0;
     if (const char* ev = getenv("LF_GROW_BITMAP")) { const int v = atoi(ev); env_bitmap = v < 0 ? 0 : v; }
@@ -227,12 +229,17 @@
 void LsdState::order(int n, int big, hipStream_t s)
 {
     launch_lsd_order(params, records(), compact(), n, s);
-    if (seed_order == LF_LSD_SEED_OPENCV32) launch_lsd_seed32(params, records(), compact(), n, &d_status->rec_need, big, s);
+    label_done = false;
+    if (seed_order == LF_LSD_SEED_OPENCV32) {
+        const LsdComponents m = components();
+        label_done = launch_lsd_seed32(params, records(), compact(), n, &d_status->rec_need, big, d_seed_tickets, n_cu, &m, s);
+    }
 }
 
 void LsdState::label(int n, bool rank, hipStream_t s)
 {
-    launch_lsd_label(params, compact(), components(), n, s);
+    if (!label_done) launch_lsd_label(params, compact(), components(), n, s);
+    label_done = false;
     if (rank) launch_lsd_rank(components(), n * 3, s);
 }
 
diff --git a/lane_slam_amd/csrc/lanefront_lsdkl.hip b/lane_slam_amd/csrc/lanefront_lsdkl.hip
--- a/lane_slam_amd/csrc/lanefront_lsdkl.hip
+++ b/lane_slam_amd/csrc/lanefront_lsdkl.hip
@@ -133,7 +133,7 @@
 static int lsdkl_run_level(lf_handle* h, LsdKlLevel& lv, const uint8_t* d_gray, int n)
 {
     hipStream_t st = h->stream;
-    LF_HIP_CHECK(h, hipMemsetAsync(lv.lsd.d_maxgrad, 0, (size_t)n * 3 * sizeof(unsigned long long), st));
+    LF_HIP_CHECK(h, hipMemsetAsync(lv.lsd.d_zero, 0, lv.lsd.zero_head_bytes(n), st));
     lv.lsd.grad_gray(n, d_gray, st);
     lv.lsd.order(n, 1, st);
     lv.lsd.label(n, false, st);
diff --git a/lane_slam_amd/csrc/lsd_label.h b/lane_slam_amd/csrc/lsd_label.h
--- /dev/null
+++ b/lane_slam_amd/csrc/lsd_label.h
@@ -0,0 +1,249 @@
+#pragma once
+#include <type_traits>
+#include "common.h"
+#include "lsd_bitplane.h"
+#include "wave.h"
+
+namespace lf {
+
+#ifndef LF_LABEL_THREADS
+#define LF_LABEL_THREADS 256
+#endif
+
+struct UfLds {
+    volatile lds_u32* P;
+    __device__ __forceinline__ uint32_t get(uint32_t i) const { return P[i]; }
+    __device__ __forceinline__ void set(uint32_t i, uint32_t v) const { P[i] = v; }
+    __device__ __forceinline__ void add(uint32_t i, uint32_t v) const { (void)__hip_atomic_fetch_add((lds_u32*)&P[i], v, __ATOMIC_RELAXED, __HIP_MEMORY_SCOPE_WORKGROUP); }
+};
+struct UfLds16 {
+    volatile lds_u16* P;
+    __device__ __forceinline__ uint32_t get(uint32_t i) const { return P[i]; }
+    __device__ __forceinline__ void set(uint32_t i, uint32_t v) const { P[i] = (uint16_t)v; }
+    __device__ __forceinline__ uint32_t min(uint32_t i, uint32_t v) const
+    {
+        lds_u32* w = (lds_u32*)P + (i >> 1);
+        const uint32_t sh = (i & 1u) * 16u;
+        uint32_t cur = *(volatile lds_u32*)w;
+        for (;;) {
+            const uint32_t old = (cur >> sh) & 0xffffu;
+            if (v >= old) return old;
+            uint32_t expect = cur;
+            if (__hip_atomic_compare_exchange_strong(w, &expect, (cur & ~(0xffffu << sh)) | (v << sh), __ATOMIC_RELAXED, __ATOMIC_RELAXED, __HIP_MEMORY_SCOPE_WORKGROUP)) return old;
+            cur = expect;
+        }
+    }
+};
+struct UfGlb {
+    uint32_t* P;
+    __device__ __forceinline__ uint32_t get(uint32_t i) const { return __hip_atomic_load(P + i, __ATOMIC_RELAXED, __HIP_MEMORY_SCOPE_AGENT); }
+    __device__ __forceinline__ void set(uint32_t i, uint32_t v) const { __hip_atomic_store(P + i, v, __ATOMIC_RELAXED, __HIP_MEMORY_SCOPE_AGENT); }
+    __device__ __forceinline__ uint32_t min(uint32_t i, uint32_t v) const { return __hip_atomic_fetch_min(P + i, v, __ATOMIC_RELAXED, __HIP_MEMORY_SCOPE_AGENT); }
+    __device__ __forceinline__ void add(uint32_t i, uint32_t v) const { (void)__hip_atomic_fetch_add(P + i, v, __ATOMIC_RELAXED, __HIP_MEMORY_SCOPE_AGENT); }
+};
+template <class UF>
+__device__ __forceinline__ uint32_t uf_find(const UF& P, uint32_t x)
+{
+    uint32_t p = P.get(x);
+    while (p != x) {
+        const uint32_t g = P.get(p);
+        if (g != p) (void)P.min(x, g);
+        x = p;
+        p = g;
+    }
+    return x;
+}
+
+template <class UF>
+__device__ __forceinline__ void uf_unite(const UF& P, uint32_t a, uint32_t b)
+{
+    for (;;) {
+        a = uf_find(P, a);
+        b = uf_find(P, b);
+        if (a == b) return;
+        if (a < b) { const uint32_t t = a; a = b; b = t; }
+        const uint32_t old = P.min(a, b);
+        if (old == a) return;
+        a = old;
+    }
+}
+
+constexpr int LT = LF_LABEL_THREADS;
+#ifndef LF_COMP_TOP
+#define LF_COMP_TOP 8
+#endif
+constexpr int kCompTop = LF_COMP_TOP;
+
+template <bool GLB>
+__device__ __forceinline__ void lsd_label_problem(const LsdParams& p, int pc, const int* __restrict__ norder, const uint32_t* __restrict__ c_xy,
+                                                  const int* __restrict__ row_start, uint16_t* __restrict__ c_label,
+                                                  uint16_t* __restrict__ comp_list, int* __restrict__ comp_count, int* __restrict__ comp_key, int comp_cap,
+                                                  uint32_t* __restrict__ scratch, size_t scratch_stride)
+{
+    extern __shared__ __attribute__((aligned(16))) uint32_t dyn_lds[];
+    const int LS = p.label_lds;
+    __shared__ uint16_t roots[kCompCap];
+    __shared__ int n_roots, rest_total;
+    const int t = threadIdx.x;
+    const size_t Ps = (size_t)p.Hs * p.Ws, o = (size_t)pc * p.rec_cap;
+    const int n = norder[pc];
+    uint16_t* lab = c_label + o;
+    uint16_t* list = comp_list + (size_t)pc * kCompCap;
+    if (n == 0) { if (t == 0) { comp_count[pc] = 0; comp_key[pc] = 0; } return; }
+    if (n > p.label_items) {
+        for (int e = t; e < n; e += LT) lab[e] = 0;
+        if (t == 0) { list[0] = 0; comp_count[pc] = 1; comp_key[pc] = n; }
+        return;
+    }
+    const uint16_t* xs_lds = reinterpret_cast<const uint16_t*>(dyn_lds + LS / 2);
+    uint32_t* gtab = scratch + (size_t)pc * scratch_stride;
+    typename std::conditional<GLB, UfGlb, UfLds16>::type parent;
+    typename std::conditional<GLB, UfGlb, UfLds>::type csize2;
+    if constexpr (GLB) { parent.P = gtab; csize2.P = gtab + ((n + 1) & ~1); }
+    else { parent.P = (volatile lds_u16*)dyn_lds; csize2.P = (volatile lds_u32*)(dyn_lds + LS / 2); }
+    auto xs = [&](int k) -> int { if constexpr (GLB) return (int)(c_xy[o + k] & 0xffffu); else return (int)xs_lds[k]; };
+    const int* rs = row_start + (size_t)pc * (p.Hs + 1);
+    if (t == 0) { n_roots = 0; rest_total = 0; }
+    if constexpr (GLB) {
+        __shared__ int wave_tot[LT / 64];
+        bitplane_build<LT>(dyn_lds, c_xy + o, n, p.Ws, Ps, wave_tot);
+        __syncthreads();
+        const unsigned long long* bits64 = reinterpret_cast<const unsigned long long*>(dyn_lds);
+        const uint16_t* pref = reinterpret_cast<const uint16_t*>(dyn_lds + 2 * bitplane_words(Ps));
+        auto bit = [&](int pos) -> bool { return (bits64[pos >> 6] >> (pos & 63)) & 1ull; };
+        auto rank = [&](int pos) -> uint32_t {
+            const int w = pos >> 6;
+            const unsigned long long lo = bits64[w & ~1], cur = bits64[w];
+            return (uint32_t)pref[w >> 1] + ((w & 1) ? (uint32_t)__builtin_popcountll(lo) : 0u) + (uint32_t)__builtin_popcountll(cur & ((1ull << (pos & 63)) - 1ull));
+        };
+        for (int e = t; e < n; e += LT) {
+            const uint32_t xy = c_xy[o + e];
+            const int x = (int)(xy & 0xffffu), y = (int)(xy >> 16), pos = y * p.Ws + x;
+            int back = 0;
+            while (back < x && bit(pos - back - 1)) ++back;
+            parent.set((uint32_t)e, (uint32_t)(e - back));
+        }
+        __syncthreads();
+        for (int e = t; e < n; e += LT) {
+            const uint32_t xy = c_xy[o + e];
+            const int x = (int)(xy & 0xffffu), y = (int)(xy >> 16);
+            if (y == 0) continue;
+            const int up = (y - 1) * p.Ws + x;
+            const bool head = x == 0 || !bit(up + p.Ws - 1);
+            const bool uL = x > 0 && bit(up - 1), uC = bit(up), uR = x + 1 < p.Ws && bit(up + 1);
+            if (head) {
+                if (uL) uf_unite(parent, (uint32_t)e, rank(up - 1));
+                else if (uC) uf_unite(parent, (uint32_t)e, rank(up));
+                if (uR && !uC) uf_unite(parent, (uint32_t)e, rank(up + 1));
+            } else if (uR && !uC) uf_unite(parent, (uint32_t)e, rank(up + 1));
+        }
+        __syncthreads();
+    } else {
+        for (int e = t; e < n; e += LT) reinterpret_cast<uint16_t*>(dyn_lds + LS / 2)[e] = (uint16_t)(c_xy[o + e] & 0xffffu);
+        __syncthreads();
+    for (int e = t; e < n; e += LT) {
+        const int y = (int)(c_xy[o + e] >> 16);
+        const int first = rs[y];
+        int h = e;
+        int xh = xs(h);
+        while (h > first) { const int xp = xs(h - 1); if (xp + 1 != xh) break; --h; xh = xp; }
+        parent.set((uint32_t)e, (uint32_t)h);
+    }
+    __syncthreads();
+    for (int e = t; e < n; e += LT) {
+        const uint32_t xy = c_xy[o + e];
+        const int x = (int)(xy & 0xffffu), y = (int)(xy >> 16);
+        if (y > 0) {
+            int lo = rs[y - 1];
+            const int end = rs[y];
+            int hi = end;
+            while (lo < hi) { const int mid = (lo + hi) >> 1; if (xs(mid) < x - 1) lo = mid + 1; else hi = mid; }
+            for (int k = lo; k < end && k < lo + 3 && xs(k) <= x + 1; ++k) uf_unite(parent, (uint32_t)e, (uint32_t)k);
+        }
+    }
+    __syncthreads();
+    }
+    for (int i = t; i < (n + 1) / 2; i += LT) csize2.set((uint32_t)i, 0u);
+    __syncthreads();
+    for (int e = t; e < n; e += LT) {
+        const uint32_t r = uf_find(parent, (uint32_t)e);
+        lab[e] = (uint16_t)r;
+        csize2.add(r >> 1, 1u << (16 * (r & 1u)));
+    }
+    __syncthreads();
+    auto csize = [&](uint32_t r) -> uint32_t { return (csize2.get(r >> 1) >> (16 * (r & 1u))) & 0xffffu; };
+    const uint32_t minsz = p.min_reg_size > 1 ? (uint32_t)p.min_reg_size : 1u;
+    for (int e = t; e < n; e += LT)
+        if (csize((uint32_t)e) >= minsz) {
+            const int k = atomicAdd(&n_roots, 1);
+            if (k < comp_cap) roots[k] = (uint16_t)e;
+        }
+    __syncthreads();
+    const int C = n_roots;
+    if (C > comp_cap) {
+        for (int e = t; e < n; e += LT) lab[e] = 0;
+        if (t == 0) { list[0] = 0; comp_count[pc] = 1; comp_key[pc] = n; }
+        return;
+    }
+    for (int i = t; i < C; i += LT) {
+        const uint32_t ri = roots[i], si = csize(ri);
+        int rank = 0;
+        for (int j = 0; j < C; ++j) {
+            const uint32_t rj = roots[j], sj = csize(rj);
+            rank += (sj > si || (sj == si && rj < ri)) ? 1 : 0;
+        }
+        list[rank] = (uint16_t)ri;
+        parent.set(ri, (uint32_t)rank);
+        if (rank == 0) comp_key[pc] = (int)si;
+        if (rank >= kCompTop) atomicAdd(&rest_total, (int)si);
+    }
+    __syncthreads();
+    if (C <= kCompTop) {
+        if (t == 0) { comp_count[pc] = C; if (C == 0) comp_key[pc] = 0; }
+        return;
+    }
+    __threadfence_block();
+    const uint16_t rest_root = list[kCompTop];
+    for (int e = t; e < n; e += LT) {
+        const uint32_t r = lab[e];
+        if (csize(r) >= minsz && parent.get(r) >= (uint32_t)kCompTop) lab[e] = rest_root;
+    }
+    if (t == 0) {
+        const int rest = rest_total;
+        const int top0 = (int)csize((uint32_t)list[0]);
+        if (rest > top0) {
+            for (int k = kCompTop; k > 0; --k) list[k] = list[k - 1];
+            list[0] = rest_root;
+            comp_key[pc] = rest;
+        }
+        comp_count[pc] = kCompTop + 1;
+    }
+}
+
+__device__ __forceinline__ void lsd_label_any(const LsdParams& p, int pc, const int* __restrict__ norder, const uint32_t* __restrict__ c_xy,
+                                              const int* __restrict__ row_start, uint16_t* __restrict__ c_label,
+                                              uint16_t* __restrict__ comp_list, int* __restrict__ comp_count, int* __restrict__ comp_key, int comp_cap,
+                                              uint32_t* __restrict__ scratch, size_t scratch_stride, int plane_fits)
+{
+    const int n = norder[pc];
+    if (n <= p.label_lds)
+        lsd_label_problem<false>(p, pc, norder, c_xy, row_start, c_label, comp_list, comp_count, comp_key, comp_cap, scratch, scratch_stride);
+    else if (plane_fits)
+        lsd_label_problem<true>(p, pc, norder, c_xy, row_start, c_label, comp_list, comp_count, comp_key, comp_cap, scratch, scratch_stride);
+    else {
+        const size_t o = (size_t)pc * p.rec_cap;
+        for (int e = threadIdx.x; e < n; e += LT) c_label[o + e] = 0;
+        if (threadIdx.x == 0) { comp_list[(size_t)pc * kCompCap] = 0; comp_count[pc] = 1; comp_key[pc] = n; }
+    }
+}
+
+inline size_t lsd_label_lds_bytes(const LsdParams& p, int* plane_fits)
+{
+    size_t lds = (size_t)p.label_lds * (2 + 2);
+    const size_t plane = bitplane_lds_words((size_t)p.Hs * p.Ws) * 4;
+    *plane_fits = plane <= 150 * 1024 ? 1 : 0;
+    if (*plane_fits && plane > lds) lds = plane;
+    return lds;
+}
+
+}
```

Result: slower. 116,900 (-2.8%).
